# sephiroce/srf

Hardware: AMD Instinct MI355X
Metric: acoustic frames/sec through SRF (123-d fbank, 3-iter DR) at 1/2/4/8 MI355X (higher is better)
Workload: dtype fp32; 1 GPU; wsj_c4: SRF L=6 PH=CH=16 DIM=32 LPAD=RPAD=2 DR iter=3, train step (fwd+bwd+allreduce+Adam); utterances_per_gpu=28, frames_per_utterance=800, global_batch=28, parallelism=dp1, launch=hipgraph (fwd+CTC+bwd)

## Files before the change

### include/srf.h

```cpp
#ifndef SRF_H_
#define SRF_H_
#include <stddef.h>

#ifdef __cplusplus
extern "C" {
#endif

int srf_version(void);
const char* srf_last_error(void);

int srf_route_dr_auto_chunks(int B, int T, int N, int din, int lpad, int rpad, int J, int dout);
int srf_route_dr_split_table(int B, int T, int N, int din, int lpad, int rpad, int J, int dout, int n_chunks,
                             int* info, int* table, int capacity);
size_t srf_route_dr_saved_floats(int B, int T, int J, int dout, int iters);
size_t srf_route_dr_fwd_workspace(int B, int T, int N, int din, int lpad, int rpad, int J, int dout, int iters,
                                  int n_chunks);
size_t srf_route_dr_bwd_workspace(int B, int T, int N, int din, int lpad, int rpad, int J, int dout, int iters,
                                  int n_chunks);
int srf_route_dr_fwd(const float* emb, const float* W, const float* bias, int B, int T, int N, int din, int lpad,
                     int rpad, int J, int dout, int iters, int mask_first, int n_chunks, float* v_out,
                     float* saved, void* workspace, size_t workspace_bytes, void* stream);
size_t srf_route_dr_coupling_floats(int B, int T, int N, int din, int lpad, int rpad, int J, int dout, int iters);
#define SRF_DR_LAYOUT_N 17
int srf_route_dr_operand_layout(int B, int T, int N, int din, int lpad, int rpad, int J, int dout, int iters,
                                long long* out);
int srf_route_dr_fwd_ex(const float* emb, const float* W, const float* bias, int B, int T, int N, int din, int lpad,
                        int rpad, int J, int dout, int iters, int mask_first, int n_chunks, float* v_out,
                        float* saved, float* couplings, void* workspace, size_t workspace_bytes, void* stream);
int srf_route_dr_bwd_ex(const float* emb, const float* W, const float* bias, int B, int T, int N, int din, int lpad,
                        int rpad, int J, int dout, int iters, int mask_first, int n_chunks, const float* saved,
                        const float* couplings, const float* g_v, float* g_emb, float* g_W, float* g_bias,
                        void* workspace, size_t workspace_bytes, void* stream);
int srf_route_dr_bwd_weights_ex(const float* emb, int B, int T, int N, int din, int lpad, int rpad, int J, int dout,
                                int iters, int mask_first, int n_chunks, const float* saved, const float* couplings,
                                float* g_W, float* g_bias, void* workspace, size_t workspace_bytes, void* stream);
int srf_route_dr_bwd_data_ex(const float* emb, const float* W, const float* bias, int B, int T, int N, int din,
                             int lpad, int rpad, int J, int dout, int iters, int mask_first, int n_chunks,
                             const float* saved, const float* couplings, const float* g_v, float* g_emb,
                             void* workspace, size_t workspace_bytes, void* stream);
int srf_set_seed_source(const void* step_counter);
int srf_set_fault_flag(void* flag);
int srf_route_dr_bwd(const float* emb, const float* W, const float* bias, int B, int T, int N, int din, int lpad,
                     int rpad, int J, int dout, int iters, int mask_first, int n_chunks, const float* saved,
                     const float* g_v, float* g_emb, float* g_W, float* g_bias, void* workspace,
                     size_t workspace_bytes, void* stream);
int srf_route_dr_bwd_data(const float* emb, const float* W, const float* bias, int B, int T, int N, int din,
                          int lpad, int rpad, int J, int dout, int iters, int mask_first, int n_chunks,
                          const float* saved, const float* g_v, float* g_emb, void* workspace,
                          size_t workspace_bytes, void* stream);
int srf_route_dr_bwd_weights(const float* emb, int B, int T, int N, int din, int lpad, int rpad, int J, int dout,
                             int iters, int mask_first, int n_chunks, float* g_W, float* g_bias, void* workspace,
                             size_t workspace_bytes, void* stream);

size_t srf_route_sdr_saved_floats(int B, int T, int J, int dout);
size_t srf_route_sdr_fwd_workspace(int B, int T, int N, int din, int lpad, int rpad, int J, int dout);
size_t srf_route_sdr_bwd_workspace(int B, int T, int N, int din, int lpad, int rpad, int J, int dout, int iters);
int srf_route_sdr_fwd(const float* emb, const float* W, const float* bias, int B, int T, int N, int din, int lpad,
                      int rpad, int J, int dout, int iters, int mask_first, float* v_out, float* saved,
                      void* workspace, size_t workspace_bytes, void* stream);
int srf_route_sdr_bwd(const float* emb, const float* W, const float* bias, int B, int T, int N, int din, int lpad,
                      int rpad, int J, int dout, int iters, int mask_first, const float* saved, const float* g_v,
                      float* g_emb, float* g_W, float* g_bias, void* workspace, size_t workspace_bytes,
                      void* stream);

#define SRF_SDR_MAX_ITEMS 8
typedef struct {
  int t0, t1;
  const float* emb;
  const float* W;
  const float* bias;
  const float* WT;
  float* u;
  int v0, vn;
  float* v;
  float* couplings;
  void* workspace;
  size_t workspace_bytes;
  const float* g_v;
  float* carry;
  float* gu;
  int g0, gn;
  float* g_emb;
  float* g_W;
  float* g_bias;
  int accumulate;
  int u_bf16;
  int group;
  int gu_factored;
} srf_sdr_range;
int srf_route_sdr_pose_n(const srf_sdr_range* ranges, int n, int B, int T, int N, int din, int lpad, int rpad, int J,
                         int dout, int fp8, void* stream);
int srf_route_sdr_recur_fwd_n(const srf_sdr_range* ranges, int n, int B, int T, int in_n, int J, int dout, int iters,
                              int mask_first, void* stream);
int srf_route_sdr_recur_bwd_n(const srf_sdr_range* ranges, int n, int B, int T, int in_n, int J, int dout, int iters,
                              int mask_first, void* stream);
int srf_route_sdr_gx_n(const srf_sdr_range* ranges, int n, int B, int T, int N, int din, int lpad, int rpad, int J,
                       int dout, void* stream);
int srf_route_sdr_gw_n(const srf_sdr_range* ranges, int n, int B, int T, int N, int din, int lpad, int rpad, int J,
                       int dout, void* stream);
int srf_route_sdr_gx_gw_n(const srf_sdr_range* ranges, int n, int B, int T, int N, int din, int lpad, int rpad,
                          int J, int dout, void* stream);
int srf_route_sdr_gx_gw_fact_n(const srf_sdr_range* ranges, int n, int B, int T, int N, int din, int lpad, int rpad,
                               int J, int dout, int iters, void* stream);

int srf_route_sdr_pose(const float* emb, const float* W, const float* bias, int B, int T, int N, int din, int lpad,
                       int rpad, int J, int dout, int t0, int t1, float* u, int v0, int vn, void* stream);
int srf_route_sdr_pose_fp8(const float* emb, const float* W, const float* bias, int B, int T, int N, int din, int lpad,
                           int rpad, int J, int dout, int t0, int t1, float* u, int v0, int vn, void* stream);
size_t srf_route_sdr_recur_workspace(int B, int in_n, int J, int dout, int iters);
size_t srf_route_sdr_recur_zero_range(int B, int in_n, int J, int dout, int iters, size_t* offset_bytes);
size_t srf_route_sdr_coupling_floats(int in_n, int J, int dout, int iters);
int srf_route_sdr_couplings_required(int in_n, int J, int dout, int iters);
size_t srf_route_sdr_fact_floats(int in_n, int J, int dout, int iters);
int srf_route_sdr_recur_fwd(const float* u, int v0, int vn, int B, int T, int in_n, int J, int dout, int iters,
                            int mask_first, int t0, int t1, float* v_out, float* couplings, void* workspace,
                            size_t workspace_bytes, void* stream);
int srf_route_sdr_recur_bwd(const float* u, int v0, int vn, const float* v_saved, const float* couplings,
                            const float* g_v, int B, int T, int in_n, int J, int dout, int iters, int mask_first,
                            int t0, int t1, float* carry, float* gu, int g0, int gn, void* workspace,
                            size_t workspace_bytes, void* stream);
int srf_route_sdr_transpose_w(const float* W, int in_n, int J, int dout, int din, float* WT, void* stream);
int srf_route_sdr_gx(const float* gu, int g0, int gn, const float* WT, int B, int T, int N, int din, int lpad,
                     int rpad, int J, int dout, int t0, int t1, float* g_emb, void* stream);
int srf_route_sdr_gw(const float* gu, int g0, int gn, const float* emb, int B, int T, int N, int din, int lpad,
                     int rpad, int J, int dout, int t0, int t1, int accumulate, float* g_W, float* g_bias,
                     void* stream);

int srf_cnnfe_out_dims(int T, int feat_dim, int* T2, int* F2);
size_t srf_cnnfe_saved_bytes(int B, int T, int feat_dim, int nfilt);
size_t srf_cnnfe_fwd_workspace(int B, int T, int feat_dim, int nfilt);
size_t srf_cnnfe_bwd_workspace(int B, int T, int feat_dim, int nfilt);
int srf_cnnfe_fwd(const float* feats, const int* inp_len, int B, int T, int feat_dim, int nfilt,
                  const float* k0a, const float* b0a, const float* k0b, const float* b0b, const float* gamma0,
                  const float* beta0, const float* k1a, const float* b1a, const float* k1b, const float* b1b,
                  const float* gamma1, const float* beta1, float* mmean0, float* mvar0, float* mmean1, float* mvar1,
                  int training, float drop_p, unsigned long long seed, float* out, void* saved, size_t saved_bytes,
                  void* workspace, size_t workspace_bytes, void* stream);
int srf_cnnfe_bwd(const float* feats, const int* inp_len, int B, int T, int feat_dim, int nfilt, const float* gamma0,
                  const float* k1a, const float* k1b, const float* gamma1, float drop_p, unsigned long long seed,
                  const void* saved, const float* g_out, float* g_k0a, float* g_b0a, float* g_k0b, float* g_b0b,
                  float* g_gamma0, float* g_beta0, float* g_k1a, float* g_b1a, float* g_k1b, float* g_b1b,
                  float* g_gamma1, float* g_beta1, void* workspace, size_t workspace_bytes, void* stream);

#define SRF_CNNFE_BWD_PREP 1
#define SRF_CNNFE_BWD_DATA 2
#define SRF_CNNFE_BWD_WGRAD 4
#define SRF_CNNFE_BWD_ALL 7
int srf_cnnfe_bwd_parts(int parts, const float* feats, const int* inp_len, int B, int T, int feat_dim, int nfilt,
                        const float* gamma0, const float* k1a, const float* k1b, const float* gamma1, float drop_p,
                        unsigned long long seed, const void* saved, const float* g_out, float* g_k0a, float* g_b0a,
                        float* g_k0b, float* g_b0b, float* g_gamma0, float* g_beta0, float* g_k1a, float* g_b1a,
                        float* g_k1b, float* g_b1b, float* g_gamma1, float* g_beta1, void* workspace,
                        size_t workspace_bytes, void* stream);

size_t srf_primary_caps_saved_bytes(int B, int T, int PH, int PD);
size_t srf_primary_caps_bwd_workspace(int B, int T, int K, int PH, int PD);
int srf_primary_caps_fwd(const float* X, const int* inp_len, int B, int T, int K, int PH, int PD, const float* Wp,
                         const float* bp, const float* K1, const float* b1, const float* K2, const float* b2,
                         const float* gamma, const float* beta, int training, float p_caps, float p_in,
                         unsigned long long seed, float* z, void* saved, size_t saved_bytes, void* stream);
int srf_primary_caps_bwd(const float* X, const int* inp_len, int B, int T, int K, int PH, int PD, const float* Wp,
                         const float* K1, const float* K2, const float* gamma, const float* beta, int training,
                         float p_caps, float p_in, unsigned long long seed, const void* saved, const float* g_z,
                         float* g_X, float* g_Wp, float* g_bp, float* g_K1, float* g_b1, float* g_K2, float* g_b2,
                         float* g_gamma, float* g_beta, void* workspace, size_t workspace_bytes, void* stream);
int srf_primary_caps_fwd_ex(const float* X, const int* inp_len, int B, int T, int K, int PH, int PD, const float* Wp,
                            const float* bp, const float* K1, const float* b1, const float* K2, const float* b2,
                            const float* gamma, const float* beta, int training, float p_caps, float p_in,
                            unsigned long long seed, float proj_scale, int pos_enc, float* z, void* saved,
                            size_t saved_bytes, void* stream);
int srf_primary_caps_bwd_ex(const float* X, const int* inp_len, int B, int T, int K, int PH, int PD, const float* Wp,
                            const float* K1, const float* K2, const float* gamma, const float* beta, int training,
                            float p_caps, float p_in, unsigned long long seed, float proj_scale, const void* saved,
                            const float* g_z, float* g_X, float* g_Wp, float* g_bp, float* g_K1, float* g_b1,
                            float* g_K2, float* g_b2, float* g_gamma, float* g_beta, void* workspace,
                            size_t workspace_bytes, void* stream);

size_t srf_capsnorm_bwd_workspace(int F, int n, int J);
int srf_capsnorm_fwd(const float* x, int F, int n, const float* gamma, const float* beta, int training, float p,
                     unsigned long long seed, int layer, float* y, float* stat, void* stream);
int srf_capsnorm_bwd(const float* x, int F, int n, const float* gamma, const float* beta, int training, float p,
                     unsigned long long seed, int layer, const float* stat, const float* g_y, float* g_x,
                     float* g_gamma, float* g_beta, void* workspace, size_t workspace_bytes, void* stream);
int srf_capsnorm_fwd_range(const float* x, int B, int T, int t0, int t1, int n, const float* gamma, const float* beta,
                           int training, float p, unsigned long long seed, int layer, float* y, float* stat,
                           void* stream);
int srf_capsnorm_bwd_range(const float* x, int B, int T, int t0, int t1, int n, const float* gamma, const float* beta,
                           int training, float p, unsigned long long seed, int layer, const float* stat,
                           const float* g_y, float* g_x, float* gpart, void* stream);
#define SRF_CAPSNORM_MAX_ITEMS 8
typedef struct {
  int t0, t1, layer;
// ... 116 lines not shown
```

### srf_amd/_lib.py

```python
import ctypes
import os

_HERE = os.path.dirname(os.path.abspath(__file__))
LIB_PATH = os.environ.get('SRF_LIB_PATH') or os.path.join(_HERE, 'libsrf.so')

_c_int, _c_size, _vp = ctypes.c_int, ctypes.c_size_t, ctypes.c_void_p

SDR_MAX_ITEMS = 8


class SdrRange(ctypes.Structure):
    _fields_ = [('t0', _c_int), ('t1', _c_int), ('emb', _vp), ('W', _vp), ('bias', _vp), ('WT', _vp),
                ('u', _vp), ('v0', _c_int), ('vn', _c_int), ('v', _vp), ('couplings', _vp),
                ('workspace', _vp), ('workspace_bytes', _c_size), ('g_v', _vp), ('carry', _vp),
                ('gu', _vp), ('g0', _c_int), ('gn', _c_int), ('g_emb', _vp), ('g_W', _vp), ('g_bias', _vp),
                ('accumulate', _c_int), ('u_bf16', _c_int), ('group', _c_int), ('gu_factored', _c_int)]


_ranges = ctypes.POINTER(SdrRange)

CAPSNORM_MAX_ITEMS = 8


class CapsnormRange(ctypes.Structure):
    _fields_ = [('t0', _c_int), ('t1', _c_int), ('layer', _c_int), ('x', _vp), ('gamma', _vp), ('beta', _vp),
                ('y', _vp), ('stat', _vp), ('g_y', _vp), ('g_x', _vp), ('gpart', _vp)]


_cn_ranges = ctypes.POINTER(CapsnormRange)

STREAM_ADVANCE_MAX = 32


class StreamBuf(ctypes.Structure):
    _fields_ = [('ptr', _vp), ('row_bytes', _c_size), ('rows_per_stream', _c_int), ('shift', _c_int),
                ('keep', _c_int)]

_SIGNATURES = {
    'srf_version': (_c_int, []),
    'srf_last_error': (ctypes.c_char_p, []),
    'srf_set_seed_source': (_c_int, [_vp]),
    'srf_set_fault_flag': (_c_int, [_vp]),
    'srf_route_dr_auto_chunks': (_c_int, [_c_int] * 8),
    'srf_route_dr_split_table': (_c_int, [_c_int] * 9 + [_vp, _vp, _c_int]),
    'srf_route_dr_saved_floats': (_c_size, [_c_int] * 5),
    'srf_route_dr_fwd_workspace': (_c_size, [_c_int] * 10),
    'srf_route_dr_bwd_workspace': (_c_size, [_c_int] * 10),
    'srf_route_dr_fwd': (_c_int, [_vp, _vp, _vp] + [_c_int] * 11 + [_vp, _vp, _vp, _c_size, _vp]),
    'srf_route_dr_bwd': (_c_int, [_vp, _vp, _vp] + [_c_int] * 11 + [_vp, _vp, _vp, _vp, _vp, _vp, _c_size, _vp]),
    'srf_route_dr_bwd_data': (_c_int, [_vp, _vp, _vp] + [_c_int] * 11 + [_vp, _vp, _vp, _vp, _c_size, _vp]),
    'srf_route_dr_bwd_weights': (_c_int, [_vp] + [_c_int] * 11 + [_vp, _vp, _vp, _c_size, _vp]),
    'srf_route_dr_coupling_floats': (_c_size, [_c_int] * 9),
    'srf_route_dr_operand_layout': (_c_int, [_c_int] * 9 + [_vp]),
    'srf_route_dr_fwd_ex': (_c_int, [_vp, _vp, _vp] + [_c_int] * 11 + [_vp, _vp, _vp, _vp, _c_size, _vp]),
    'srf_route_dr_bwd_ex': (_c_int, [_vp, _vp, _vp] + [_c_int] * 11 + [_vp] * 7 + [_c_size, _vp]),
    'srf_route_dr_bwd_data_ex': (_c_int, [_vp, _vp, _vp] + [_c_int] * 11 + [_vp] * 5 + [_c_size, _vp]),
    'srf_route_dr_bwd_weights_ex': (_c_int, [_vp] + [_c_int] * 11 + [_vp] * 5 + [_c_size, _vp]),
    'srf_route_sdr_saved_floats': (_c_size, [_c_int] * 4),
    'srf_route_sdr_fwd_workspace': (_c_size, [_c_int] * 8),
    'srf_route_sdr_bwd_workspace': (_c_size, [_c_int] * 9),
    'srf_route_sdr_fwd': (_c_int, [_vp, _vp, _vp] + [_c_int] * 10 + [_vp, _vp, _vp, _c_size, _vp]),
    'srf_route_sdr_bwd': (_c_int, [_vp, _vp, _vp] + [_c_int] * 10 + [_vp, _vp, _vp, _vp, _vp, _vp, _c_size, _vp]),
    'srf_route_sdr_pose': (_c_int, [_vp, _vp, _vp] + [_c_int] * 10 + [_vp, _c_int, _c_int, _vp]),
    'srf_route_sdr_pose_fp8': (_c_int, [_vp, _vp, _vp] + [_c_int] * 10 + [_vp, _c_int, _c_int, _vp]),
    'srf_route_sdr_recur_workspace': (_c_size, [_c_int] * 5),
    'srf_route_sdr_recur_zero_range': (_c_size, [_c_int] * 5 + [ctypes.POINTER(_c_size)]),
    'srf_route_sdr_coupling_floats': (_c_size, [_c_int] * 4),
    'srf_route_sdr_couplings_required': (_c_int, [_c_int] * 4),
    'srf_route_sdr_fact_floats': (_c_size, [_c_int] * 4),
    'srf_route_sdr_recur_fwd': (_c_int, [_vp] + [_c_int] * 11 + [_vp, _vp, _vp, _c_size, _vp]),
    'srf_route_sdr_recur_bwd': (_c_int, [_vp, _c_int, _c_int, _vp, _vp, _vp] + [_c_int] * 9
                                + [_vp, _vp, _c_int, _c_int, _vp, _c_size, _vp]),
    'srf_route_sdr_transpose_w': (_c_int, [_vp] + [_c_int] * 4 + [_vp, _vp]),
    'srf_route_sdr_gx': (_c_int, [_vp, _c_int, _c_int, _vp] + [_c_int] * 10 + [_vp, _vp]),
    'srf_route_sdr_gw': (_c_int, [_vp, _c_int, _c_int, _vp] + [_c_int] * 11 + [_vp, _vp, _vp]),
    'srf_route_sdr_pose_n': (_c_int, [_ranges] + [_c_int] * 10 + [_vp]),
    'srf_route_sdr_recur_fwd_n': (_c_int, [_ranges] + [_c_int] * 8 + [_vp]),
    'srf_route_sdr_recur_bwd_n': (_c_int, [_ranges] + [_c_int] * 8 + [_vp]),
    'srf_route_sdr_gx_n': (_c_int, [_ranges] + [_c_int] * 9 + [_vp]),
    'srf_route_sdr_gw_n': (_c_int, [_ranges] + [_c_int] * 9 + [_vp]),
    'srf_route_sdr_gx_gw_n': (_c_int, [_ranges] + [_c_int] * 9 + [_vp]),
    'srf_route_sdr_gx_gw_fact_n': (_c_int, [_ranges] + [_c_int] * 10 + [_vp]),
    'srf_cnnfe_out_dims': (_c_int, [_c_int, _c_int, ctypes.POINTER(_c_int), ctypes.POINTER(_c_int)]),
    'srf_cnnfe_saved_bytes': (_c_size, [_c_int] * 4),
    'srf_cnnfe_fwd_workspace': (_c_size, [_c_int] * 4),
    'srf_cnnfe_bwd_workspace': (_c_size, [_c_int] * 4),
    'srf_cnnfe_fwd': (_c_int, [_vp, _vp] + [_c_int] * 4 + [_vp] * 16 + [_c_int, ctypes.c_float, ctypes.c_ulonglong,
                                                                       _vp, _vp, _c_size, _vp, _c_size, _vp]),
    'srf_cnnfe_bwd': (_c_int, [_vp, _vp] + [_c_int] * 4 + [_vp] * 4 + [ctypes.c_float, ctypes.c_ulonglong]
                      + [_vp] * 15 + [_c_size, _vp]),
    'srf_cnnfe_bwd_parts': (_c_int, [_c_int, _vp, _vp] + [_c_int] * 4 + [_vp] * 4 + [ctypes.c_float, ctypes.c_ulonglong]
                            + [_vp] * 15 + [_c_size, _vp]),
    'srf_primary_caps_saved_bytes': (_c_size, [_c_int] * 4),
    'srf_primary_caps_bwd_workspace': (_c_size, [_c_int] * 5),
    'srf_primary_caps_fwd': (_c_int, [_vp, _vp] + [_c_int] * 5 + [_vp] * 8 + [_c_int, ctypes.c_float, ctypes.c_float,
                                                                           ctypes.c_ulonglong, _vp, _vp, _c_size, _vp]),
    'srf_primary_caps_bwd': (_c_int, [_vp, _vp] + [_c_int] * 5 + [_vp] * 5 + [_c_int, ctypes.c_float, ctypes.c_float,
                                                                           ctypes.c_ulonglong] + [_vp] * 12
                             + [_c_size, _vp]),
    'srf_primary_caps_fwd_ex': (_c_int, [_vp, _vp] + [_c_int] * 5 + [_vp] * 8
                                + [_c_int, ctypes.c_float, ctypes.c_float, ctypes.c_ulonglong, ctypes.c_float, _c_int,
                                   _vp, _vp, _c_size, _vp]),
    'srf_primary_caps_bwd_ex': (_c_int, [_vp, _vp] + [_c_int] * 5 + [_vp] * 5
                                + [_c_int, ctypes.c_float, ctypes.c_float, ctypes.c_ulonglong, ctypes.c_float]
                                + [_vp] * 12 + [_c_size, _vp]),
    'srf_capsnorm_bwd_workspace': (_c_size, [_c_int] * 3),
    'srf_capsnorm_fwd': (_c_int, [_vp, _c_int, _c_int, _vp, _vp, _c_int, ctypes.c_float, ctypes.c_ulonglong, _c_int,
                                  _vp, _vp, _vp]),
    'srf_capsnorm_bwd': (_c_int, [_vp, _c_int, _c_int, _vp, _vp, _c_int, ctypes.c_float, ctypes.c_ulonglong, _c_int]
                         + [_vp] * 6 + [_c_size, _vp]),
    'srf_capsnorm_fwd_range_n': (_c_int, [_cn_ranges] + [_c_int] * 5 + [ctypes.c_float, ctypes.c_ulonglong, _vp]),
    'srf_capsnorm_bwd_range_n': (_c_int, [_cn_ranges] + [_c_int] * 5 + [ctypes.c_float, ctypes.c_ulonglong, _vp]),
    'srf_capsnorm_fwd_range': (_c_int, [_vp] + [_c_int] * 5 + [_vp, _vp, _c_int, ctypes.c_float, ctypes.c_ulonglong,
                                                             _c_int, _vp, _vp, _vp]),
    'srf_capsnorm_bwd_range': (_c_int, [_vp] + [_c_int] * 5 + [_vp, _vp, _c_int, ctypes.c_float, ctypes.c_ulonglong,
                                                             _c_int, _vp, _vp, _vp, _vp, _vp]),
    'srf_capsnorm_params_workspace': (_c_size, [_c_int] * 2),
    'srf_capsnorm_bwd_params': (_c_int, [_vp, _c_int, _c_int, _vp, _vp, _vp, _c_size, _vp]),
    'srf_caps_head_fwd': (_c_int, [_vp, _c_int, _c_int, _c_int] + [_vp] * 4 + [_c_int, ctypes.c_float,
                                                                              ctypes.c_ulonglong, _c_int]
                          + [_vp] * 4),
    'srf_caps_head_fwd_ex': (_c_int, [_vp, _c_int, _c_int, _c_int] + [_vp] * 4
                             + [_c_int, ctypes.c_float, ctypes.c_ulonglong, _c_int, ctypes.c_float] + [_vp] * 4),
    'srf_caps_head_bwd': (_c_int, [_vp, _c_int, _c_int, _c_int] + [_vp] * 3 + [_c_int, ctypes.c_float,
                                                                              ctypes.c_ulonglong, _c_int]
                          + [_vp] * 9 + [_c_size, _vp]),
    'srf_ctc_workspace': (_c_size, [_c_int] * 4),
    'srf_ctc_loss': (_c_int, [_vp] * 4 + [_c_int] * 5 + [ctypes.c_float, _vp, _vp, _vp, _c_size, _vp]),
    'srf_ctc_align_workspace': (_c_size, [_c_int] * 4),
    'srf_ctc_align': (_c_int, [_vp] * 4 + [_c_int] * 5 + [_vp] * 6 + [_c_size, _vp]),
    'srf_edit_align_workspace': (_c_size, [_c_int] * 3),
    'srf_edit_align': (_c_int, [_vp, _vp, _c_int, _vp, _vp, _c_int, _c_int, _vp, _c_int] + [_vp] * 5
                       + [_c_int, _vp, _c_size, _vp]),
    'srf_word_split_workspace': (_c_size, [_c_int] * 2),
    'srf_word_split': (_c_int, [_vp, _vp, _c_int, _c_int, _vp, _c_int, _c_int] + [_vp] * 10 + [_c_size, _vp]),
    'srf_word_align_workspace': (_c_size, [_c_int] * 3),
    'srf_word_align': (_c_int, [_vp, _vp, _c_int, _vp, _vp, _c_int, _c_int, _vp, _c_int, _c_int] + [_vp] * 11
                       + [_c_size, _vp]),
    'srf_ctc_greedy_n': (_c_int, [_vp, _vp] + [_c_int] * 4 + [_vp, _vp, _vp, _vp]),
    'srf_ctc_greedy_frames_n': (_c_int, [_vp, _vp] + [_c_int] * 5 + [_vp, _vp, _vp, _vp, _vp]),
    'srf_ctc_beam_state_bytes': (_c_size, [_c_int] * 4),
    'srf_ctc_beam_reset': (_c_int, [_vp, _c_size] + [_c_int] * 4 + [ctypes.POINTER(_c_int), _vp]),
    'srf_ctc_beam_push_n': (_c_int, [_vp, _c_size] + [_c_int] * 5 + [_vp, _vp, _c_int, ctypes.POINTER(_c_int), _vp]),
    'srf_ctc_beam_best': (_c_int, [_vp, _c_size] + [_c_int] * 4 + [_vp, _vp, _vp, _vp]),
    'srf_ctc_beam_nbest': (_c_int, [_vp, _c_size] + [_c_int] * 6 + [_vp, _vp, _vp, _vp, _vp]),
    'srf_ctc_beam_lm_state_bytes': (_c_size, [_c_int] * 4),
    'srf_ctc_beam_lm_reset': (_c_int, [_vp, _c_size] + [_c_int] * 4 + [ctypes.POINTER(_c_int), _vp]),
    'srf_ctc_beam_lm_push_n': (_c_int, [_vp, _c_size] + [_c_int] * 5 + [_vp, _vp, _c_int, _vp, _vp, _c_int,
                                                                       ctypes.POINTER(_c_int), _vp]),
    'srf_ctc_beam_lm_best': (_c_int, [_vp, _c_size] + [_c_int] * 4 + [_vp, _vp, _vp, _vp, _vp]),
    'srf_ctc_beam_lm_nbest': (_c_int, [_vp, _c_size] + [_c_int] * 6 + [_vp, _vp, _vp, _vp, _vp, _vp]),
    'srf_mwer_workspace': (_c_size, [_c_int] * 5),
    'srf_mwer_loss': (_c_int, [_vp] * 6 + [_c_int] * 6 + [ctypes.c_float] + [_vp] * 5 + [_c_size, _vp]),
    'srf_stream_advance_n': (_c_int, [ctypes.POINTER(StreamBuf), _c_int, _c_int, _vp]),
    'srf_fbank_num_frames': (_c_int, [_c_int]),
    'srf_fbank_table_floats': (_c_size, []),
    'srf_fbank_tables': (_c_int, [_vp, _c_size]),
    'srf_fbank_static': (_c_int, [_vp, _c_int, _vp, _vp] + [_c_int] * 9 + [ctypes.c_float, ctypes.c_ulonglong, _vp, _vp]),
    'srf_fbank_deltas': (_c_int, [_vp, _vp] + [_c_int] * 6 + [_vp, _vp, _c_int, _vp, _c_int, _c_int, _vp]),
    'srf_fbank_stats': (_c_int, [_vp, _vp, _c_int, _c_int, _c_int, _vp, _vp]),
    'srf_adam_step': (_c_int, [_vp, _vp, _vp, _vp, _c_size, ctypes.c_float, ctypes.c_float, ctypes.c_float,
                               ctypes.c_float, _vp]),
}

_PROF_SIGNATURES = {
    'srf_route_dr_set_timing_events': (_c_int, [_vp, _vp, _c_int]),
}


class SrfError(RuntimeError):
    pass


_lib = None


def lib():
    global _lib
    if _lib is None:
        if not os.path.exists(LIB_PATH):
            raise ImportError(f'{LIB_PATH} is missing: build it with `make -C srf_amd/csrc` '
                              '(or __graft_entry__.build()); there is no fallback path')
        import torch
        h = ctypes.CDLL(LIB_PATH)
        for name, (res, args) in list(_SIGNATURES.items()) + list(_PROF_SIGNATURES.items()):
            fn = getattr(h, name)
            fn.restype = res
            fn.argtypes = args
        _lib = h
    return _lib


def exported_symbols():
    return list(_SIGNATURES)


def prof_symbols():
    return list(_PROF_SIGNATURES)


def check(rc, what):
    if rc != 0:
        msg = lib().srf_last_error().decode(errors='replace')
        raise SrfError(f'{what} failed (rc={rc}): {msg}')
```

### srf_amd/csrc/caps.hip

```cpp
#include <algorithm>
#include <cmath>

#include "srf_common.h"
#include "srf_reduce.h"
#include "srf_rng.h"
#include "../../include/srf.h"

namespace {

constexpr float kSquashEps = 1e-7f;
constexpr float kLengthEps = 1e-7f;
constexpr float kLnEps = 1e-3f;
constexpr int kMaxVec = 4096;

__device__ __forceinline__ int ceil_div_len(int len, int div) { return (len + div - 1) / div; }

__device__ __forceinline__ void block_sum2(float& a, float& b, float* red) {
  a = wave_sum(a);
  b = wave_sum(b);
  const int w = threadIdx.x >> 6, l = threadIdx.x & 63;
  __syncthreads();
  if (l == 0) {
    red[w] = a;
    red[4 + w] = b;
  }
  __syncthreads();
  a = red[0] + red[1] + red[2] + red[3];
  b = red[4] + red[5] + red[6] + red[7];
}

__device__ __forceinline__ float drop_mult(bool on, unsigned long long seed, unsigned stream, size_t idx, float p) {
  if (!on) return 1.f;
  return srf_keep(seed, stream, idx, p) ? 1.f / (1.f - p) : 0.f;
}

__device__ __forceinline__ float pos_enc(int t, int p, int PH) {
  const int nts = PH >> 1;
  const float inc = 9.210340371976184f / (float)(nts - 1);
  const int k = p < nts ? p : p - nts;
  const float st = (float)t * expf((float)k * -inc);
  return p < nts ? sinf(st) : cosf(st);
}

__device__ __forceinline__ float proj_epilogue(float acc, int f, int T, int p, int PH, float scale, int pe) {
  const float y = acc * scale;
  return pe ? y + pos_enc(f % T, p, PH) : y;
}

__global__ __launch_bounds__(256) void proj_fwd_kernel(const float* __restrict__ X, int F, int K, int PH,
                                                       const float* __restrict__ Wp, const float* __restrict__ bp,
                                                       float* __restrict__ e, int T, float scale, int pe) {
  const int f = blockIdx.x * 4 + (threadIdx.x >> 6);
  const int l = threadIdx.x & 63;
  if (f >= F) return;
  const float* x = X + (size_t)f * K;
  for (int p0 = 0; p0 < PH; p0 += 8) {
    const int np = min(8, PH - p0);
    float acc[8];
#pragma unroll
    for (int q = 0; q < 8; ++q) acc[q] = 0.f;
#pragma unroll 4
    for (int k = l; k < K; k += 64) {
      const float xv = x[k];
      const float* w = Wp + (size_t)k * PH + p0;
#pragma unroll
      for (int q = 0; q < 8; ++q) acc[q] += xv * (q < np ? w[q < np ? q : 0] : 0.f);
    }
#pragma unroll
    for (int q = 0; q < 8; ++q) {
      const float s = wave_sum(acc[q]);
      if (l == 0 && q < np) e[(size_t)f * PH + p0 + q] = proj_epilogue(s + bp[p0 + q], f, T, p0 + q, PH, scale, pe);
    }
  }
}

template <int PH, int FW>
__global__ __launch_bounds__(256) void proj_fwd_vec_kernel(const float* __restrict__ X, int F, int K,
                                                           const float* __restrict__ Wp,
                                                           const float* __restrict__ bp, float* __restrict__ e,
                                                           int T, float scale, int pe) {
  constexpr int PQ = PH / 4;
  const int l = threadIdx.x & 63;
  const int f0 = (blockIdx.x * 4 + (threadIdx.x >> 6)) * FW;
  if (f0 >= F) return;
  float acc[FW][PH];
#pragma unroll
  for (int u = 0; u < FW; ++u)
#pragma unroll
    for (int p = 0; p < PH; ++p) acc[u][p] = 0.f;
#pragma unroll 2
  for (int k0 = 4 * l; k0 < K; k0 += 256) {
    f4 x[FW], w[4][PQ];
#pragma unroll
    for (int u = 0; u < FW; ++u) x[u] = *reinterpret_cast<const f4*>(X + (size_t)min(f0 + u, F - 1) * K + k0);
#pragma unroll
    for (int kk = 0; kk < 4; ++kk)
#pragma unroll
      for (int q = 0; q < PQ; ++q) w[kk][q] = *reinterpret_cast<const f4*>(Wp + (size_t)(k0 + kk) * PH + 4 * q);
#pragma unroll
    for (int u = 0; u < FW; ++u)
#pragma unroll
      for (int kk = 0; kk < 4; ++kk)
#pragma unroll
        for (int p = 0; p < PH; ++p) acc[u][p] += x[u][kk] * w[kk][p >> 2][p & 3];
  }
#pragma unroll
  for (int u = 0; u < FW; ++u)
#pragma unroll
    for (int p = 0; p < PH; ++p) {
      const float sum = wave_sum(acc[u][p]);
      if (l == 0 && f0 + u < F) e[(size_t)(f0 + u) * PH + p] = proj_epilogue(sum + bp[p], f0 + u, T, p, PH, scale, pe);
    }
}

constexpr int kProjWaves = 16;
template <int PH>
__global__ __launch_bounds__(64 * kProjWaves) void proj_fwd_mfma_kernel(const float* __restrict__ X, int F, int K,
                                                                       const float* __restrict__ Wp,
                                                                       const float* __restrict__ bp,
                                                                       float* __restrict__ e, int T, float scale,
                                                                       int pe, int Kq) {
  static_assert(PH <= 16, "one 16-column output tile");
  __shared__ float part[kProjWaves][16][17];
  const int lane = threadIdx.x & 63, wv = threadIdx.x >> 6;
  const int m = lane & 15, g = lane >> 4;
  const int f0 = blockIdx.x * 16;
  const int fm = min(f0 + m, F - 1);
  const bool fok = f0 + m < F;
  const int kb = wv * Kq, ke = min(K, kb + Kq);
  f4 acc = {0.f, 0.f, 0.f, 0.f};
  constexpr int U = 4;
  for (int k0 = kb; k0 < ke; k0 += 16 * U) {
    f4 xa[U];
    float wb[U][4];
#pragma unroll
    for (int u = 0; u < U; ++u) {
      const int k = k0 + 16 * u + 4 * g;
      const bool kok = k < ke;
      const f4 x = *reinterpret_cast<const f4*>(X + (size_t)fm * K + (kok ? k : kb));
      xa[u] = (fok && kok) ? x : f4{0.f, 0.f, 0.f, 0.f};
#pragma unroll
      for (int j = 0; j < 4; ++j) {
        const float w = Wp[(size_t)(kok ? k + j : kb) * PH + min(m, PH - 1)];
        wb[u][j] = (kok && m < PH) ? w : 0.f;
      }
    }
#pragma unroll
    for (int u = 0; u < U; ++u)
#pragma unroll
      for (int j = 0; j < 4; ++j) acc = mfma16x16x4(xa[u][j], wb[u][j], acc);
  }
#pragma unroll
  for (int v = 0; v < 4; ++v) part[wv][4 * g + v][m] = acc[v];
  __syncthreads();
  if (threadIdx.x < 16 * PH) {
    const int r = threadIdx.x / PH, pp = threadIdx.x % PH;
    float sum = 0.f;
#pragma unroll
    for (int w = 0; w < kProjWaves; ++w) sum += part[w][r][pp];
    if (f0 + r < F) e[(size_t)(f0 + r) * PH + pp] = proj_epilogue(sum + bp[pp], f0 + r, T, pp, PH, scale, pe);
  }
}

constexpr int kProjXF = 16;
template <int PH>
__global__ __launch_bounds__(256) void proj_bwd_x_vec_kernel(const float* __restrict__ g_e,
                                                             const float* __restrict__ Wp, int F, int K,
                                                             float* __restrict__ g_X) {
  constexpr int PQ = PH / 4;
  const size_t idx = (size_t)blockIdx.x * blockDim.x + threadIdx.x;
  const int K4 = K / 4;
  const int FG = (F + kProjXF - 1) / kProjXF;
  if (idx >= (size_t)FG * K4) return;
  const int fg = (int)(idx / K4);
  const int k0 = (int)(idx - (size_t)fg * K4) * 4;
  f4 w[4][PQ];
#pragma unroll
  for (int kk = 0; kk < 4; ++kk)
#pragma unroll
    for (int q = 0; q < PQ; ++q) w[kk][q] = *reinterpret_cast<const f4*>(Wp + (size_t)(k0 + kk) * PH + 4 * q);
#pragma unroll
  for (int u = 0; u < kProjXF; ++u) {
    const int f = fg * kProjXF + u;
    if (f >= F) break;
    f4 ge[PQ];
#pragma unroll
// ... 302 lines not shown
      const int tt = t - dt + 1;
      if (tt < 0 || tt >= cd.T) continue;
      const size_t fo = (size_t)(f - dt + 1) * E;
      for (int dp = 0; dp < 3; ++dp) {
        const int pp = p - dp + 1;
        if (pp < 0 || pp >= cd.PH) continue;
        for (int d = q; d < cd.PD; d += kEbLanes)
          s += g_v1[fo + pp * cd.PD + d] * K1[(dt * 3 + dp) * cd.PD + d] +
               g_v2[fo + pp * cd.PD + d] * K2[(dt * 3 + dp) * cd.PD + d];
      }
    }
  }
#pragma unroll
  for (int o = kEbLanes / 2; o >= 1; o >>= 1) s += __shfl_xor(s, o, 64);
  if (live && q == 0) g_e[idx] = s * scale;
}

struct RowMap {
  int T, t0, nt;
  __device__ __forceinline__ int row(int q) const {
    const int b = q / nt;
    return b * T + t0 + (q - b * nt);
  }
  static RowMap all(int F) { return RowMap{F, 0, F}; }
};

__device__ __forceinline__ void capsnorm_fwd_row(const float* __restrict__ x, int n, const float* __restrict__ gamma,
                                                 const float* __restrict__ beta, int training, float p,
                                                 unsigned long long seed, const unsigned long long* __restrict__ seed_src,
                                                 unsigned stream, float* __restrict__ y, float* __restrict__ stat,
                                                 int head, int J, int D, const float* __restrict__ gamma_o,
                                                 const float* __restrict__ beta_o, float* __restrict__ logits,
                                                 float* __restrict__ lens, float len_eps, int f) {
  seed = srf_step_seed(seed, seed_src);
  extern __shared__ __attribute__((aligned(16))) float sm[];
  float* v = sm;
  float* red = v + n;
  float s1 = 0.f, dummy = 0.f;
  for (int i = threadIdx.x; i < n; i += blockDim.x) {
    const float a = x[(size_t)f * n + i];
    v[i] = a;
    s1 += a;
  }
  block_sum2(s1, dummy, red);
  const float mean = s1 / n;
  float s2 = 0.f;
  for (int i = threadIdx.x; i < n; i += blockDim.x) {
    const float dv = v[i] - mean;
    s2 += dv * dv;
  }
  dummy = 0.f;
  block_sum2(s2, dummy, red);
  const float rstd = 1.f / sqrtf(s2 / n + kLnEps);
  for (int i = threadIdx.x; i < n; i += blockDim.x) {
    const size_t gi = (size_t)f * n + i;
    const float o = ((v[i] - mean) * rstd * gamma[i] + beta[i]) * drop_mult(training && p > 0.f, seed, stream, gi, p);
    v[i] = o;
    if (!head) y[gi] = o;
  }
  if (threadIdx.x == 0) {
    stat[4 * f] = mean;
    stat[4 * f + 1] = rstd;
  }
  if (!head) return;
  __syncthreads();
  float* L = v + n + 8;
  for (int j = threadIdx.x; j < J; j += blockDim.x) {
    float s = 0.f;
    for (int d = 0; d < D; ++d) s += v[j * D + d] * v[j * D + d];
    L[j] = sqrtf(s + len_eps);
    lens[(size_t)f * J + j] = L[j];
  }
  __syncthreads();
  float t1 = 0.f;
  dummy = 0.f;
  for (int j = threadIdx.x; j < J; j += blockDim.x) t1 += L[j];
  block_sum2(t1, dummy, red);
  const float mo = t1 / J;
  float t2 = 0.f;
  for (int j = threadIdx.x; j < J; j += blockDim.x) t2 += (L[j] - mo) * (L[j] - mo);
  dummy = 0.f;
  block_sum2(t2, dummy, red);
  const float ro = 1.f / sqrtf(t2 / J + kLnEps);
  for (int j = threadIdx.x; j < J; j += blockDim.x)
    logits[(size_t)f * J + j] = (L[j] - mo) * ro * gamma_o[j] + beta_o[j];
  if (threadIdx.x == 0) {
    stat[4 * f + 2] = mo;
    stat[4 * f + 3] = ro;
  }
}

__device__ __forceinline__ void capsnorm_bwd_row(
    const float* __restrict__ x, int n, const float* __restrict__ gamma, const float* __restrict__ beta,
    int training, float p, unsigned long long seed, const unsigned long long* __restrict__ seed_src, unsigned stream,
    const float* __restrict__ stat, const float* __restrict__ g_in, int head, int J, int D,
    const float* __restrict__ gamma_o, const float* __restrict__ lens, float* __restrict__ g_x,
    float* __restrict__ gpart, int f) {
  seed = srf_step_seed(seed, seed_src);
  extern __shared__ __attribute__((aligned(16))) float sm[];
  float* gy = sm;
  float* red = gy + n;
  float* gl = red + 8;
  const float mean = stat[4 * f], rstd = stat[4 * f + 1];
  const size_t stride = head ? (size_t)2 * n + 2 * J : (size_t)2 * n;
  if (head) {
    const float mo = stat[4 * f + 2], ro = stat[4 * f + 3];
    float a1 = 0.f, a2 = 0.f;
    for (int j = threadIdx.x; j < J; j += blockDim.x) {
      const float go = g_in[(size_t)f * J + j];
      const float xh = (lens[(size_t)f * J + j] - mo) * ro;
      gpart[(size_t)f * stride + 2 * n + j] = go * xh;
      gpart[(size_t)f * stride + 2 * n + J + j] = go;
      const float gx = go * gamma_o[j];
      gl[j] = gx;
      a1 += gx;
      a2 += gx * xh;
    }
    block_sum2(a1, a2, red);
    for (int j = threadIdx.x; j < J; j += blockDim.x) {
      const float xh = (lens[(size_t)f * J + j] - mo) * ro;
      gl[j] = ro * (gl[j] - a1 / J - xh * a2 / J) / lens[(size_t)f * J + j];
    }
    __syncthreads();
  }
  float a1 = 0.f, a2 = 0.f;
  for (int i = threadIdx.x; i < n; i += blockDim.x) {
    const size_t gi = (size_t)f * n + i;
    const float xh = (x[gi] - mean) * rstd;
    const float dm = drop_mult(training && p > 0.f, seed, stream, gi, p);
    float go;
    if (head) {
      const float o = (xh * gamma[i] + beta[i]) * dm;
      go = gl[i / D] * o;
    } else {
      go = g_in[gi];
    }
    const float g = go * dm;
    gpart[(size_t)f * stride + i] = g * xh;
    gpart[(size_t)f * stride + n + i] = g;
    const float t = g * gamma[i];
    gy[i] = t;
    a1 += t;
    a2 += t * xh;
  }
  block_sum2(a1, a2, red);
  for (int i = threadIdx.x; i < n; i += blockDim.x) {
    const size_t gi = (size_t)f * n + i;
    const float xh = (x[gi] - mean) * rstd;
    g_x[gi] = rstd * (gy[i] - a1 / n - xh * a2 / n);
  }
}

template <int NPL>
__device__ __forceinline__ void capsnorm_fwd_wave(const float* __restrict__ x, const float* __restrict__ gamma,
                                                  const float* __restrict__ beta, bool drop, float p,
                                                  unsigned long long seed, unsigned stream, float* __restrict__ y,
                                                  float* __restrict__ stat, int f, int lane) {
  constexpr int n = 64 * NPL, NV = NPL / 4;
  const f4* xr = reinterpret_cast<const f4*>(x + (size_t)f * n);
  f4 v[NV];
  float s1 = 0.f;
#pragma unroll
  for (int k = 0; k < NV; ++k) {
    v[k] = xr[k * 64 + lane];
    s1 += (v[k].x + v[k].y) + (v[k].z + v[k].w);
  }
  const float mean = wave_sum(s1) / n;
  float s2 = 0.f;
#pragma unroll
  for (int k = 0; k < NV; ++k) {
    const f4 d = v[k] - mean;
    s2 += (d.x * d.x + d.y * d.y) + (d.z * d.z + d.w * d.w);
  }
  const float rstd = 1.f / sqrtf(wave_sum(s2) / n + kLnEps);
  f4* yr = reinterpret_cast<f4*>(y + (size_t)f * n);
#pragma unroll
  for (int k = 0; k < NV; ++k) {
    const int q = k * 64 + lane;
    const f4 g = reinterpret_cast<const f4*>(gamma)[q], b = reinterpret_cast<const f4*>(beta)[q];
    const size_t gi = (size_t)f * n + 4 * q;
    f4 o;
#pragma unroll
    for (int c = 0; c < 4; ++c) o[c] = ((v[k][c] - mean) * rstd * g[c] + b[c]) * drop_mult(drop, seed, stream, gi + c, p);
    yr[q] = o;
  }
  if (lane == 0) {
    stat[4 * f] = mean;
    stat[4 * f + 1] = rstd;
  }
}

template <int NPL>
__device__ __forceinline__ void caps_head_fwd_wave(const float* __restrict__ x, const float* __restrict__ gamma,
                                                   const float* __restrict__ beta, bool drop, float p,
                                                   unsigned long long seed, unsigned stream,
                                                   float* __restrict__ stat, int D, const float* __restrict__ gamma_o,
                                                   const float* __restrict__ beta_o, float* __restrict__ logits,
                                                   float* __restrict__ lens, float len_eps, int f, int lane) {
  constexpr int n = 64 * NPL, NV = NPL / 4;
  const int LPC = D / 4, J = n / D;
  const f4* xr = reinterpret_cast<const f4*>(x + (size_t)f * n);
  f4 v[NV];
  float s1 = 0.f;
#pragma unroll
  for (int k = 0; k < NV; ++k) {
    v[k] = xr[k * 64 + lane];
    s1 += (v[k].x + v[k].y) + (v[k].z + v[k].w);
  }
  const float mean = wave_sum(s1) / n;
  float s2 = 0.f;
#pragma unroll
  for (int k = 0; k < NV; ++k) {
    const f4 d = v[k] - mean;
    s2 += (d.x * d.x + d.y * d.y) + (d.z * d.z + d.w * d.w);
  }
  const float rstd = 1.f / sqrtf(wave_sum(s2) / n + kLnEps);
  float L[NV];
  float t1 = 0.f;
#pragma unroll
  for (int k = 0; k < NV; ++k) {
    const int q = k * 64 + lane;
    const f4 g = reinterpret_cast<const f4*>(gamma)[q], b = reinterpret_cast<const f4*>(beta)[q];
    const size_t gi = (size_t)f * n + 4 * q;
    float ss = 0.f;
#pragma unroll
    for (int c = 0; c < 4; ++c) {
      const float o = ((v[k][c] - mean) * rstd * g[c] + b[c]) * drop_mult(drop, seed, stream, gi + c, p);
      ss += o * o;
    }
    for (int m = 1; m < LPC; m <<= 1) ss += __shfl_xor(ss, m, 64);
    L[k] = sqrtf(ss + len_eps);
    t1 += L[k];
  }
  const float mo = wave_sum(t1) / (float)LPC / J;
  float t2 = 0.f;
#pragma unroll
  for (int k = 0; k < NV; ++k) t2 += (L[k] - mo) * (L[k] - mo);
  const float ro = 1.f / sqrtf(wave_sum(t2) / (float)LPC / J + kLnEps);
  if (lane % LPC == 0) {
#pragma unroll
    for (int k = 0; k < NV; ++k) {
      const int j = (k * 64 + lane) / LPC;
      lens[(size_t)f * J + j] = L[k];
      logits[(size_t)f * J + j] = (L[k] - mo) * ro * gamma_o[j] + beta_o[j];
    }
  }
  if (lane == 0) {
    stat[4 * f] = mean;
    stat[4 * f + 1] = rstd;
    stat[4 * f + 2] = mo;
    stat[4 * f + 3] = ro;
  }
}

template <int NPL>
__global__ __launch_bounds__(256) void caps_head_fwd_wave_kernel(const float* __restrict__ x,
                                                                 const float* __restrict__ gamma,
                                                                 const float* __restrict__ beta, int training, float p,
                                                                 unsigned long long seed,
                                                                 const unsigned long long* __restrict__ seed_src,
                                                                 unsigned stream, float* __restrict__ stat, int D,
                                                                 const float* __restrict__ gamma_o,
                                                                 const float* __restrict__ beta_o,
                                                                 float* __restrict__ logits, float* __restrict__ lens,
                                                                 float len_eps, int rows) {
  const int w = blockIdx.x * 4 + (threadIdx.x >> 6);
  if (w >= rows) return;
  caps_head_fwd_wave<NPL>(x, gamma, beta, training && p > 0.f, p, srf_step_seed(seed, seed_src), stream, stat, D,
                          gamma_o, beta_o, logits, lens, len_eps, w, threadIdx.x & 63);
}

template <int NPL>
__device__ __forceinline__ void capsnorm_bwd_wave(const float* __restrict__ x, const float* __restrict__ gamma,
                                                  bool drop, float p, unsigned long long seed, unsigned stream,
                                                  const float* __restrict__ stat, const float* __restrict__ g_in,
                                                  float* __restrict__ g_x, f4 (&pgxh)[NPL / 4], f4 (&pgg)[NPL / 4],
                                                  int f, int lane) {
  constexpr int n = 64 * NPL, NV = NPL / 4;
  const float mean = stat[4 * f], rstd = stat[4 * f + 1];
  const f4* xr = reinterpret_cast<const f4*>(x + (size_t)f * n);
  const f4* gr = reinterpret_cast<const f4*>(g_in + (size_t)f * n);
  f4 xh[NV], t[NV];
  float a1 = 0.f, a2 = 0.f;
#pragma unroll
  for (int k = 0; k < NV; ++k) {
    const int q = k * 64 + lane;
    const f4 xv = xr[q], go = gr[q], gam = reinterpret_cast<const f4*>(gamma)[q];
    const size_t gi = (size_t)f * n + 4 * q;
    f4 gxh, gg;
#pragma unroll
    for (int c = 0; c < 4; ++c) {
      xh[k][c] = (xv[c] - mean) * rstd;
      const float g = go[c] * drop_mult(drop, seed, stream, gi + c, p);
      gxh[c] = g * xh[k][c];
      gg[c] = g;
      t[k][c] = g * gam[c];
      a1 += t[k][c];
      a2 += t[k][c] * xh[k][c];
    }
    pgxh[k] += gxh;
    pgg[k] += gg;
  }
  a1 = wave_sum(a1);
  a2 = wave_sum(a2);
  f4* ox = reinterpret_cast<f4*>(g_x + (size_t)f * n);
#pragma unroll
  for (int k = 0; k < NV; ++k) {
    f4 o;
#pragma unroll
    for (int c = 0; c < 4; ++c) o[c] = rstd * (t[k][c] - a1 / n - xh[k][c] * a2 / n);
    ox[k * 64 + lane] = o;
  }
}

template <int NPL>
__device__ __forceinline__ void store_gpart(float* __restrict__ gpart, size_t row, const f4 (&pgxh)[NPL / 4],
                                            const f4 (&pgg)[NPL / 4], int lane) {
  constexpr int n = 64 * NPL;
  f4* pg = reinterpret_cast<f4*>(gpart + row * 2 * n);
#pragma unroll
  for (int k = 0; k < NPL / 4; ++k) {
    pg[k * 64 + lane] = pgxh[k];
    pg[n / 4 + k * 64 + lane] = pgg[k];
  }
}

template <int NPL, bool BWD>
__global__ __launch_bounds__(256) void capsnorm_wave_kernel(const float* __restrict__ x, const float* __restrict__ gamma,
                                                            const float* __restrict__ beta, int training, float p,
                                                            unsigned long long seed,
                                                            const unsigned long long* __restrict__ seed_src,
                                                            unsigned stream, float* __restrict__ y,
                                                            float* __restrict__ stat, const float* __restrict__ g_in,
                                                            float* __restrict__ gpart, RowMap rmap, int rows, int rpw) {
  const int w = blockIdx.x * 4 + (threadIdx.x >> 6);
  const int lane = threadIdx.x & 63;
  const unsigned long long sd = srf_step_seed(seed, seed_src);
  const bool drop = training && p > 0.f;
  if constexpr (BWD) {
    const int r0 = w * rpw;
    if (r0 >= rows) return;
    f4 pgxh[NPL / 4], pgg[NPL / 4];
#pragma unroll
    for (int k = 0; k < NPL / 4; ++k) pgxh[k] = pgg[k] = f4{0.f, 0.f, 0.f, 0.f};
    const int r1 = min(rows, r0 + rpw);
    for (int r = r0; r < r1; ++r)
      capsnorm_bwd_wave<NPL>(x, gamma, drop, p, sd, stream, stat, g_in, y, pgxh, pgg, rmap.row(r), lane);
    store_gpart<NPL>(gpart, rpw == 1 ? (size_t)rmap.row(r0) : (size_t)w, pgxh, pgg, lane);
  } else {
    if (w >= rows) return;
    capsnorm_fwd_wave<NPL>(x, gamma, beta, drop, p, sd, stream, y, stat, rmap.row(w), lane);
  }
}

__global__ __launch_bounds__(256) void capsnorm_fwd_kernel(
    const float* __restrict__ x, int n, const float* __restrict__ gamma, const float* __restrict__ beta, int training,
    float p, unsigned long long seed, const unsigned long long* __restrict__ seed_src, unsigned stream,
    float* __restrict__ y, float* __restrict__ stat, int head, int J, int D, const float* __restrict__ gamma_o,
    const float* __restrict__ beta_o, float* __restrict__ logits, float* __restrict__ lens, float len_eps,
    RowMap rmap) {
  capsnorm_fwd_row(x, n, gamma, beta, training, p, seed, seed_src, stream, y, stat, head, J, D, gamma_o, beta_o,
                   logits, lens, len_eps, rmap.row(blockIdx.x));
}

__global__ __launch_bounds__(256) void capsnorm_bwd_kernel(
    const float* __restrict__ x, int n, const float* __restrict__ gamma, const float* __restrict__ beta, int training,
    float p, unsigned long long seed, const unsigned long long* __restrict__ seed_src, unsigned stream,
    const float* __restrict__ stat, const float* __restrict__ g_in, int head, int J, int D,
    const float* __restrict__ gamma_o, const float* __restrict__ lens, float* __restrict__ g_x,
    float* __restrict__ gpart, RowMap rmap) {
  capsnorm_bwd_row(x, n, gamma, beta, training, p, seed, seed_src, stream, stat, g_in, head, J, D, gamma_o, lens, g_x,
                   gpart, rmap.row(blockIdx.x));
}

struct CnItems {
  srf_capsnorm_range it[SRF_CAPSNORM_MAX_ITEMS];
  int B, T, n_items;
};

template <int NPL, bool BWD>
__global__ __launch_bounds__(256) void capsnorm_range_n_wave_kernel(CnItems items, int training, float p,
                                                                    unsigned long long seed,
                                                                    const unsigned long long* __restrict__ seed_src) {
  const srf_capsnorm_range& r = items.it[blockIdx.y];
  const int nt = r.t1 - r.t0;
  const int w = blockIdx.x * 4 + (threadIdx.x >> 6);
  if (w >= items.B * nt) return;
  const int f = RowMap{items.T, r.t0, nt}.row(w);
  const unsigned stream = (unsigned)(kStreamMid0 + r.layer);
  const unsigned long long sd = srf_step_seed(seed, seed_src);
  const bool drop = training && p > 0.f;
  if constexpr (BWD) {
    f4 pgxh[NPL / 4], pgg[NPL / 4];
#pragma unroll
    for (int k = 0; k < NPL / 4; ++k) pgxh[k] = pgg[k] = f4{0.f, 0.f, 0.f, 0.f};
    capsnorm_bwd_wave<NPL>(r.x, r.gamma, drop, p, sd, stream, r.stat, r.g_y, r.g_x, pgxh, pgg, f, threadIdx.x & 63);
    store_gpart<NPL>(r.gpart, (size_t)f, pgxh, pgg, threadIdx.x & 63);
  } else
    capsnorm_fwd_wave<NPL>(r.x, r.gamma, r.beta, drop, p, sd, stream, r.y, r.stat, f, threadIdx.x & 63);
}

template <bool BWD>
__global__ __launch_bounds__(256) void capsnorm_range_n_kernel(CnItems items, int n, int training, float p,
                                                               unsigned long long seed,
                                                               const unsigned long long* __restrict__ seed_src) {
  const srf_capsnorm_range& r = items.it[blockIdx.y];
  const int nt = r.t1 - r.t0;
  if ((int)blockIdx.x >= items.B * nt) return;
  const int f = RowMap{items.T, r.t0, nt}.row(blockIdx.x);
  const unsigned stream = (unsigned)(kStreamMid0 + r.layer);
  if constexpr (BWD)
    capsnorm_bwd_row(r.x, n, r.gamma, r.beta, training, p, seed, seed_src, stream, r.stat, r.g_y, 0, 0, 0, nullptr,
                     nullptr, r.g_x, r.gpart, f);
  else
    capsnorm_fwd_row(r.x, n, r.gamma, r.beta, training, p, seed, seed_src, stream, r.y, r.stat, 0, 0, 0, nullptr,
                     nullptr, nullptr, nullptr, kLengthEps, f);
}

struct CapsSaved {
  float *e, *m, *lnstat;
  unsigned char* sel;
  size_t bytes;
};

CapsSaved caps_saved_layout(int F, int PH, int PD, void* base) {
  const size_t E = (size_t)PH * PD;
  size_t off = 0;
  auto take = [&](size_t bytes) {
    size_t o = off;
    off += srf::align_up(bytes, 256);
    return o;
  };
  const size_t oe = take((size_t)F * PH * 4), om = take((size_t)F * E * 4), os = take((size_t)F * 2 * 4),
               osel = take((size_t)F * E);
  char* b = static_cast<char*>(base);
  CapsSaved c;
  c.e = (float*)(b + oe);
  c.m = (float*)(b + om);
  c.lnstat = (float*)(b + os);
  c.sel = (unsigned char*)(b + osel);
  c.bytes = off;
  return c;
}

struct CapsBwdWs {
  float *gv1, *gv2, *wpart, *wsum, *g_e, *ppart, *psum, *scratch;
  size_t bytes;
};

constexpr int kProjChunks = 64;

CapsBwdWs caps_bwd_layout(int F, int K, int PH, int PD, void* base) {
  const size_t E = (size_t)PH * PD;
  const size_t wcols = 2 * E + 20 * PD, pcols = (size_t)K * PH + PH;
  size_t off = 0;
  auto take = [&](size_t bytes) {
    size_t o = off;
    off += srf::align_up(bytes, 256);
    return o;
  };
  const size_t o1 = take((size_t)F * E * 4), o2 = take((size_t)F * E * 4), ow = take((size_t)F * wcols * 4),
               owsum = take(wcols * 4), oge = take((size_t)F * PH * 4), opp = take(kProjChunks * pcols * 4),
               ops = take(pcols * 4),
               osc = take(std::max(srf::colsum_scratch_floats(F, (int)wcols), srf::colsum_scratch_floats(kProjChunks, (int)pcols)) * 4);
  char* b = static_cast<char*>(base);
  CapsBwdWs w;
  w.gv1 = (float*)(b + o1);
  w.gv2 = (float*)(b + o2);
  w.wpart = (float*)(b + ow);
  w.wsum = (float*)(b + owsum);
  w.g_e = (float*)(b + oge);
  w.ppart = (float*)(b + opp);
  w.psum = (float*)(b + ops);
  w.scratch = (float*)(b + osc);
  w.bytes = off;
  return w;
}

int check_caps(int B, int T, int PH, int PD) {
  SRF_REQUIRE(B > 0 && T > 0 && PH > 0 && PD > 0, "bad primary capsule shape");
  SRF_REQUIRE((size_t)PH * PD <= kMaxVec, "PH*PD = %d exceeds %d", PH * PD, kMaxVec);
  return SRF_OK;
}

}

constexpr int kCnRowsPerWave = 4;

template <bool BWD>
static bool capsnorm_wave(int n, int rows, RowMap rm, const float* x, const float* gamma, const float* beta,
                          int training, float p, unsigned long long seed, unsigned stream, float* y, float* stat,
                          const float* g_in, float* gpart, hipStream_t st, int rpw = 1) {
  const dim3 grid(((rows + rpw - 1) / rpw + 3) / 4);
#define SRF_CN_WAVE(NPL)                                                                                             \
  hipLaunchKernelGGL((capsnorm_wave_kernel<NPL, BWD>), grid, dim3(256), 0, st, x, gamma, beta, training, p, seed,   \
                     srf::seed_source(), stream, y, stat, g_in, gpart, rm, rows, rpw)
  if (n == 256) SRF_CN_WAVE(4);
  else if (n == 512) SRF_CN_WAVE(8);
  else if (n == 1024) SRF_CN_WAVE(16);
  else return false;
#undef SRF_CN_WAVE
  return true;
}

extern "C" {

size_t srf_primary_caps_saved_bytes(int B, int T, int PH, int PD) {
  return caps_saved_layout(B * T, PH, PD, nullptr).bytes;
}

size_t srf_primary_caps_bwd_workspace(int B, int T, int K, int PH, int PD) {
  return caps_bwd_layout(B * T, K, PH, PD, nullptr).bytes;
}

int srf_primary_caps_fwd(const float* X, const int* inp_len, int B, int T, int K, int PH, int PD, const float* Wp,
                         const float* bp, const float* K1, const float* b1, const float* K2, const float* b2,
                         const float* gamma, const float* beta, int training, float p_caps, float p_in,
                         unsigned long long seed, float* z, void* saved, size_t saved_bytes, void* stream) {
  return srf_primary_caps_fwd_ex(X, inp_len, B, T, K, PH, PD, Wp, bp, K1, b1, K2, b2, gamma, beta, training, p_caps,
                                 p_in, seed, 1.f, 0, z, saved, saved_bytes, stream);
}

int srf_primary_caps_fwd_ex(const float* X, const int* inp_len, int B, int T, int K, int PH, int PD, const float* Wp,
                            const float* bp, const float* K1, const float* b1, const float* K2, const float* b2,
                            const float* gamma, const float* beta, int training, float p_caps, float p_in,
                            unsigned long long seed, float proj_scale, int pos_enc, float* z, void* saved,
                            size_t saved_bytes, void* stream) {
  int rc = check_caps(B, T, PH, PD);
  if (rc) return rc;
  SRF_REQUIRE(!pos_enc || (PH >= 4 && PH % 2 == 0), "positional encoding needs an even PH >= 4, got %d", PH);
  SRF_REQUIRE(X && inp_len && Wp && bp && K1 && b1 && K2 && b2 && gamma && beta && z && saved, "null pointer");
  const int F = B * T;
  CapsSaved sv = caps_saved_layout(F, PH, PD, saved);
  if (saved_bytes < sv.bytes) {
    srf::set_error("primary caps saved buffer too small: %zu < %zu", saved_bytes, sv.bytes);
    return SRF_EWORKSPACE;
  }
  hipStream_t st = static_cast<hipStream_t>(stream);
  constexpr int FW = 2;
  const dim3 gvec((F + 4 * FW - 1) / (4 * FW));
  const int Kq = ((K + kProjWaves - 1) / kProjWaves + 15) / 16 * 16;
  if (K % 4 == 0 && (PH == 4 || PH == 8 || PH == 16)) {
    const dim3 gm((F + 15) / 16), bm(64 * kProjWaves);
    if (PH == 4)
      hipLaunchKernelGGL((proj_fwd_mfma_kernel<4>), gm, bm, 0, st, X, F, K, Wp, bp, sv.e, T, proj_scale, pos_enc, Kq);
    else if (PH == 8)
      hipLaunchKernelGGL((proj_fwd_mfma_kernel<8>), gm, bm, 0, st, X, F, K, Wp, bp, sv.e, T, proj_scale, pos_enc, Kq);
    else
      hipLaunchKernelGGL((proj_fwd_mfma_kernel<16>), gm, bm, 0, st, X, F, K, Wp, bp, sv.e, T, proj_scale, pos_enc,
                         Kq);
  } else if (K % 4 == 0 && PH == 4)
    hipLaunchKernelGGL((proj_fwd_vec_kernel<4, FW>), gvec, dim3(256), 0, st, X, F, K, Wp, bp, sv.e, T,
                       proj_scale, pos_enc);
  else if (K % 4 == 0 && PH == 8)
    hipLaunchKernelGGL((proj_fwd_vec_kernel<8, FW>), gvec, dim3(256), 0, st, X, F, K, Wp, bp, sv.e, T,
                       proj_scale, pos_enc);
  else if (K % 4 == 0 && PH == 16)
    hipLaunchKernelGGL((proj_fwd_vec_kernel<16, FW>), gvec, dim3(256), 0, st, X, F, K, Wp, bp, sv.e, T,
                       proj_scale, pos_enc);
  else
    hipLaunchKernelGGL(proj_fwd_kernel, dim3((F + 3) / 4), dim3(256), 0, st, X, F, K, PH, Wp, bp, sv.e, T, proj_scale,
                       pos_enc);
  SRF_LAUNCH_CHECK("proj_fwd");
  CapsDims cd{B, T, PH, PD};
  const size_t sh = (size_t)(PH * PD + 5 * PH + 8) * sizeof(float);
  hipLaunchKernelGGL(encaps_fwd_kernel, dim3(F), dim3(256), sh, st, sv.e, inp_len, cd, K1, b1, K2, b2, gamma, beta,
                     training, p_caps, p_in, seed, srf::seed_source(), sv.m, sv.sel, sv.lnstat, z);
  SRF_LAUNCH_CHECK("encaps_fwd");
  return SRF_OK;
}

int srf_primary_caps_bwd(const float* X, const int* inp_len, int B, int T, int K, int PH, int PD, const float* Wp,
                         const float* K1, const float* K2, const float* gamma, const float* beta, int training,
                         float p_caps, float p_in, unsigned long long seed, const void* saved, const float* g_z,
                         float* g_X, float* g_Wp, float* g_bp, float* g_K1, float* g_b1, float* g_K2, float* g_b2,
                         float* g_gamma, float* g_beta, void* workspace, size_t workspace_bytes, void* stream) {
  return srf_primary_caps_bwd_ex(X, inp_len, B, T, K, PH, PD, Wp, K1, K2, gamma, beta, training, p_caps, p_in, seed,
                                 1.f, saved, g_z, g_X, g_Wp, g_bp, g_K1, g_b1, g_K2, g_b2, g_gamma, g_beta, workspace,
                                 workspace_bytes, stream);
}

int srf_primary_caps_bwd_ex(const float* X, const int* inp_len, int B, int T, int K, int PH, int PD, const float* Wp,
                            const float* K1, const float* K2, const float* gamma, const float* beta, int training,
                            float p_caps, float p_in, unsigned long long seed, float proj_scale, const void* saved,
                            const float* g_z, float* g_X, float* g_Wp, float* g_bp, float* g_K1, float* g_b1,
                            float* g_K2, float* g_b2, float* g_gamma, float* g_beta, void* workspace,
                            size_t workspace_bytes, void* stream) {
  int rc = check_caps(B, T, PH, PD);
  if (rc) return rc;
  SRF_REQUIRE(X && inp_len && Wp && K1 && K2 && gamma && beta && saved && g_z && g_X && g_Wp && g_bp && g_K1 &&
                  g_b1 && g_K2 && g_b2 && g_gamma && g_beta && workspace,
              "null pointer");
  const int F = B * T, E = PH * PD;
  CapsSaved sv = caps_saved_layout(F, PH, PD, const_cast<void*>(saved));
  CapsBwdWs w = caps_bwd_layout(F, K, PH, PD, workspace);
  if (workspace_bytes < w.bytes) {
    srf::set_error("primary caps workspace too small: %zu < %zu", workspace_bytes, w.bytes);
    return SRF_EWORKSPACE;
  }
  hipStream_t st = static_cast<hipStream_t>(stream);
  CapsDims cd{B, T, PH, PD};
  const size_t sh = (size_t)(4 * E + 6 * PH + 8) * sizeof(float);
  hipLaunchKernelGGL(encaps_bwd_a_kernel, dim3(F), dim3(256), sh, st, g_z, sv.e, sv.m, sv.sel, sv.lnstat, inp_len, cd,
                     gamma, beta, training, p_caps, p_in, seed, srf::seed_source(), w.gv1, w.gv2, w.wpart);
  SRF_LAUNCH_CHECK("encaps_bwd_a");
  const int wcols = 2 * E + 20 * PD;
  if ((rc = srf::colsum(w.wpart, F, wcols, nullptr, w.scratch, st,
                        srf::ColSplit{{g_gamma, g_beta, g_K1, g_b1, g_K2, g_b2}, {E, E, 9 * PD, PD, 9 * PD, PD}})))
    return rc;
  hipLaunchKernelGGL(encaps_bwd_b_kernel, dim3(((size_t)F * PH * kEbLanes + 255) / 256), dim3(256), 0, st, w.gv1,
                     w.gv2, cd, K1, K2, w.g_e, proj_scale);
  SRF_LAUNCH_CHECK("encaps_bwd_b");
  const dim3 gx4(((size_t)((F + kProjXF - 1) / kProjXF) * (K / 4) + 255) / 256);
  if (K % 4 == 0 && PH == 4)
    hipLaunchKernelGGL(proj_bwd_x_vec_kernel<4>, gx4, dim3(256), 0, st, w.g_e, Wp, F, K, g_X);
  else if (K % 4 == 0 && PH == 8)
    hipLaunchKernelGGL(proj_bwd_x_vec_kernel<8>, gx4, dim3(256), 0, st, w.g_e, Wp, F, K, g_X);
  else if (K % 4 == 0 && PH == 16)
    hipLaunchKernelGGL(proj_bwd_x_vec_kernel<16>, gx4, dim3(256), 0, st, w.g_e, Wp, F, K, g_X);
  else
    hipLaunchKernelGGL(proj_bwd_x_kernel, dim3(((size_t)F * K + 255) / 256), dim3(256), 0, st, w.g_e, Wp, F, K, PH,
                       g_X);
  SRF_LAUNCH_CHECK("proj_bwd_x");
  const int fchunk = (F + kProjChunks - 1) / kProjChunks;
  if (PH <= 16)
    hipLaunchKernelGGL(proj_bwd_w_mfma_kernel, dim3((K + 63) / 64, kProjChunks), dim3(256), 0, st, X, w.g_e, F, K, PH,
                       fchunk, w.ppart);
  else
    hipLaunchKernelGGL(proj_bwd_w_kernel, dim3((K + 255) / 256, kProjChunks), dim3(256), 0, st, X, w.g_e, F, K, PH,
                       fchunk, w.ppart);
  SRF_LAUNCH_CHECK("proj_bwd_w");
  const int pcols = K * PH + PH;
  if ((rc = srf::colsum(w.ppart, kProjChunks, pcols, nullptr, w.scratch, st,
                        srf::ColSplit{{g_Wp, g_bp, nullptr, nullptr}, {K * PH, PH, 0, 0}})))
    return rc;
  return SRF_OK;
}

size_t srf_capsnorm_bwd_workspace(int F, int n, int J) {
  const int cols = 2 * n + 2 * J;
// ... 229 lines not shown
```

### srf_amd/csrc/route_dr.hip

```cpp
#include <algorithm>
#include <cmath>
#include <type_traits>

#include "srf_common.h"
#include "route_fwd32.h"
#include "../../include/srf.h"
#include "../../include/srf_prof.h"

namespace {

constexpr float kSquashEps = 1e-7f;

thread_local hipEvent_t* t_ev_start = nullptr;
thread_local hipEvent_t* t_ev_stop = nullptr;
thread_local int t_ev_n = 0;
constexpr int MODE_FWD = 0;
constexpr int MODE_BWD = 1;

using srf::DrGeom;

template <int KS>
__device__ __forceinline__ void load_vec(const float* __restrict__ p, float (&v)[KS]) {
  if constexpr (KS % 4 == 0) {
#pragma unroll
    for (int q = 0; q < KS / 4; ++q) {
      f4 t = *reinterpret_cast<const f4*>(p + 4 * q);
      v[4 * q] = t.x; v[4 * q + 1] = t.y; v[4 * q + 2] = t.z; v[4 * q + 3] = t.w;
    }
  } else {
    static_assert(KS == 2, "din must be 8, 16, 32 or 64");
    f2 t = *reinterpret_cast<const f2*>(p);
    v[0] = t.x; v[1] = t.y;
  }
}

__device__ __forceinline__ f4 ld4(const float* p) { return *reinterpret_cast<const f4*>(p); }
__device__ __forceinline__ void st4(float* p, f4 v) { *reinterpret_cast<f4*>(p) = v; }

struct FrameLoc {
  int b, t;
  bool valid;
};

__device__ __forceinline__ FrameLoc frame_loc(int f, int F, int T) {
  const int fc = min(f, F - 1);
  FrameLoc r;
  r.b = fc / T;
  r.t = fc - r.b * T;
  r.valid = f < F;
  return r;
}

template <int DIN>
__device__ __forceinline__ void load_x(const float* __restrict__ emb, const FrameLoc& fl, int T, int N, int lpad,
                                       int i, int g, float (&x)[DIN / 4]) {
  constexpr int KS = DIN / 4;
  const int w = i / N, n = i - w * N;
  const int ts = fl.t + w - lpad;
  const bool ok = fl.valid && ts >= 0 && ts < T;
  const int tsc = min(max(ts, 0), T - 1);
  load_vec<KS>(emb + ((size_t)(fl.b * T + tsc) * N + n) * DIN + g * KS, x);
#pragma unroll
  for (int k = 0; k < KS; ++k) x[k] = ok ? x[k] : 0.f;
}

template <int DIN>
__device__ __forceinline__ f4 pose_tile(const float* __restrict__ W, const float* __restrict__ bias, int i,
                                        int JD, int NT, int tg, int lane, const float (&x)[DIN / 4]) {
  constexpr int KS = DIN / 4;
  const int tc = min(tg, NT - 1);
  const int arow = min(tc * 16 + (lane & 15), JD - 1);
  const int g = lane >> 4;
  float a[KS];
  load_vec<KS>(W + ((size_t)i * JD + arow) * DIN + g * KS, a);
  const int crow = min(tc * 16 + 4 * g, JD - 4);
  f4 acc = ld4(bias + (size_t)i * JD + crow);
#pragma unroll
  for (int k = 0; k < KS; ++k) acc = mfma16x16x4(a[k], x[k], acc);
  return acc;
}

template <int DOUT, int TW>
__device__ __forceinline__ void jreduce(float (&p)[TW]) {
#pragma unroll
  for (int t = 0; t < TW; ++t) {
    p[t] = xor16_sum(p[t]);
    if constexpr (DOUT >= 16) p[t] = xor32_sum(p[t]);
  }
  if constexpr (DOUT > 16) {
    constexpr int TPJ = DOUT / 16;
#pragma unroll
    for (int t0 = 0; t0 < TW; t0 += TPJ) {
      float s = 0.f;
#pragma unroll
      for (int q = 0; q < TPJ; ++q) s += p[t0 + q];
#pragma unroll
      for (int q = 0; q < TPJ; ++q) p[t0 + q] = s;
    }
  }
}

template <int DOUT>
__device__ __forceinline__ int tile_j(int tg, int g) { return (tg * 16 + 4 * g) / DOUT; }

template <int DOUT>
__device__ __forceinline__ bool tile_primary(int tg) {
  if constexpr (DOUT > 16) return (tg % (DOUT / 16)) == 0;
  return true;
}

__device__ __forceinline__ void load_rows(const float* __restrict__ v, int f, bool fvalid, int JD, int tg, int g,
                                          float (&o)[4]) {
  const int row = tg * 16 + 4 * g;
  const bool ok = fvalid && row < JD;
  const f4 a = ld4(v + (size_t)(fvalid ? f : 0) * JD + min(row, JD - 4));
  o[0] = ok ? a.x : 0.f; o[1] = ok ? a.y : 0.f; o[2] = ok ? a.z : 0.f; o[3] = ok ? a.w : 0.f;
}

template <int DIN, int TW>
struct Frags {
  float x[DIN / 4];
  float w[TW][DIN / 4];
  f4 b[TW];
};

template <int DIN, int TW, bool NOBIAS = false>
__device__ __forceinline__ void fetch_frags(const float* __restrict__ emb, const float* __restrict__ W,
                                            const float* __restrict__ bias, const FrameLoc& loc, int T, int N,
                                            int lpad, int i, int JD, int NT, int tbase, int lane,
                                            Frags<DIN, TW>& fr) {
  constexpr int KS = DIN / 4;
  const int g = lane >> 4;
  load_x<DIN>(emb, loc, T, N, lpad, i, g, fr.x);
  const float* Wi = W + (size_t)i * JD * DIN;
  const float* bi = bias + (size_t)i * JD;
  int lrow = lane & 15, brow = 4 * g;
#pragma unroll
  for (int t = 0; t < TW; ++t) {
    const int tc = __builtin_amdgcn_readfirstlane(min(tbase + t, NT - 1));
    if constexpr (DIN < 16) {
      lrow = min(tc * 16 + (lane & 15), JD - 1) - tc * 16;
      brow = min(tc * 16 + 4 * g, JD - 4) - tc * 16;
    }
    load_vec<KS>(Wi + (size_t)tc * 16 * DIN + lrow * DIN + g * KS, fr.w[t]);
    if constexpr (NOBIAS) {
      fr.b[t] = f4{0.f, 0.f, 0.f, 0.f};
    } else {
      fr.b[t] = ld4(bi + tc * 16 + brow);
    }
  }
}

template <int DIN, int TW>
__device__ __forceinline__ void pose_tiles(const Frags<DIN, TW>& fr, float (&u)[TW][4]) {
#pragma unroll
  for (int t = 0; t < TW; ++t) {
    f4 acc = fr.b[t];
#pragma unroll
// ... 1379 lines not shown
      if (r > 0) vst[R + r - 1] = __builtin_bit_cast(f4, __builtin_amdgcn_raw_buffer_load_b128(rs_v[r - 1], wo0, so, 0));
    }
  };
  const int iwo = 4 * rq * 16 + 4 * ((2 * wg + (fm >> 2)) ^ (rq & 3)) + (fm & 3);
  const int iro = n * 16 + 4 * ((2 * h) ^ ((n >> 2) & 3));
  auto img_store = [&](float* im, int v) {
#pragma unroll
    for (int c = 0; c < 4; ++c) im[v * (D * 16) + iwo + c * 16] = vst[v][c];
  };
  auto img_read = [&](const float* im, f2 (&nx)[NV][4]) {
#pragma unroll
    for (int v = 0; v < NV; ++v) {
      const f4 a = ld4(im + v * (D * 16) + iro), b = ld4(im + v * (D * 16) + (iro ^ 4));
      nx[v][0] = f2{a[0], a[1]}, nx[v][1] = f2{a[2], a[3]}, nx[v][2] = f2{b[0], b[1]}, nx[v][3] = f2{b[2], b[3]};
    }
  };

  f16v acc[CAP];
  float gb[CAP];
#pragma unroll
  for (int k = 0; k < CAP; ++k) {
    gb[k] = 0.f;
    acc[k] = f16v{};
  }
  float* const imw = vimg + wv * IMG;
  if (ft0 < ft1) {
    stage_load(ft0);
    if constexpr (VW == 0) vec_load(nxa, ft0);
    else img_load(ft0);
    stage_store(0);
    if (ft0 + 1 < ft1) stage_load(ft0 + 1);
    if constexpr (VW == 2) {
#pragma unroll
      for (int v = 0; v < NV; ++v) img_store(imw, v);
      img_load(min(ft0 + 1, ft1 - 1));
    }
  }
  const int xoff = CG * 4 + (n * 16 + ((h ^ ((n >> 3) & 1)) * 8)) * 2;
  const float s0 = c0 * sg;
  auto caps = [&](int buf, const f2 (&g0)[4], const f2 (&cur)[NV][4], bool img_next) {
    const unsigned char* sb = stg[buf] + k0 * PCB;
#pragma unroll
    for (int k = 0; k < CAP; ++k) {
      const unsigned char* ck = sb + k * PCB;
      const float* ckf = reinterpret_cast<const float*>(ck);
      f2 gu[4];
#pragma unroll
      for (int v = 0; v < 4; ++v) gu[v] = g0[v];
#pragma unroll
      for (int r = 0; r < RV; ++r) {
        const float* cp = ckf + ((r * 2 + 0) * 4 + wv) * 16 + 8 * h;
        const float* gp = ckf + ((r * 2 + 1) * 4 + wv) * 16 + 8 * h;
        const f4 ca = ld4(cp), cb = ld4(cp + 4), ga = ld4(gp), gbv = ld4(gp + 4);
        const f2 c2[4] = {f2{ca[0], ca[1]}, f2{ca[2], ca[3]}, f2{cb[0], cb[1]}, f2{cb[2], cb[3]}};
        const f2 g2[4] = {f2{ga[0], ga[1]}, f2{ga[2], ga[3]}, f2{gbv[0], gbv[1]}, f2{gbv[2], gbv[3]}};
#pragma unroll
        for (int v = 0; v < 4; ++v) {
          gu[v] = __builtin_elementwise_fma(c2[v], cur[r + 1][v], gu[v]);
          gu[v] = __builtin_elementwise_fma(g2[v], cur[R + r][v], gu[v]);
        }
      }
      const f2 gq = (gu[0] + gu[1]) + (gu[2] + gu[3]);
      gb[k] += gq[0] + gq[1];
      h8 bh, bl;
      split8h(gu, bh, bl);
      const h8 xh = *reinterpret_cast<const h8*>(ck + xoff);
      const h8 xl = *reinterpret_cast<const h8*>(ck + xoff + D * 16 * 2);
      acc[k] = mfma32h(xh, bh, acc[k]);
      acc[k] = mfma32h(xh, bl, acc[k]);
      acc[k] = mfma32h(xl, bh, acc[k]);
      if constexpr (VW == 2) {
        if (img_next) {
#pragma unroll
          for (int v = 0; v < NV; ++v)
            if (v * CAP / NV == k) img_store(imw + (buf ^ 1) * (4 * IMG), v);
        }
      }
    }
  };
  auto tile = [&](auto bufc, const f2 (&cur)[NV][4], f2 (&nxt)[NV][4], int ft) {
    constexpr int buf = decltype(bufc)::value;
    f2 g0[4];
#pragma unroll
    for (int v = 0; v < 4; ++v) g0[v] = cur[0][v] * s0;
    __syncthreads();
    if (ft + 1 < ft1) {
      stage_store(buf ^ 1);
      if (ft + 2 < ft1) stage_load(ft + 2);
    }
    vec_load(nxt, ft + 1 < ft1 ? ft + 1 : ft);
    caps(buf, g0, cur, false);
  };
  auto tile_img = [&](auto bufc, int ft) {
    constexpr int buf = decltype(bufc)::value;
    f2 cur[NV][4], g0[4];
    __syncthreads();
    img_read(imw + buf * (4 * IMG), cur);
    if (ft + 1 < ft1) {
      stage_store(buf ^ 1);
      if (ft + 2 < ft1) stage_load(ft + 2);
    }
#pragma unroll
    for (int v = 0; v < 4; ++v) g0[v] = cur[0][v] * s0;
    caps(buf, g0, cur, ft + 1 < ft1);
    __builtin_amdgcn_sched_barrier(0);
    img_load(min(ft + 2, ft1 - 1));
  };
  using S0 = std::integral_constant<int, 0>;
  using S1 = std::integral_constant<int, 1>;
  for (int ft = ft0; ft < ft1; ft += 2) {
    if constexpr (VW == 0) tile(S0{}, nxa, nxb, ft);
    else tile_img(S0{}, ft);
    if (ft + 1 >= ft1) break;
    if constexpr (VW == 0) tile(S1{}, nxb, nxa, ft + 1);
    else tile_img(S1{}, ft + 1);
  }
  float* gw = gwp + (size_t)s * pstride;
  float* gbo = gbp + (size_t)s * pstride;
  const float un = srf_exp2i(-(bx + eg)), ug = srf_exp2i(-eg);
#pragma unroll
  for (int k = 0; k < CAP; ++k) {
    const float a = gb[k];
    float pa, pb;
    xpair32(a, pa, pb);
    if (k0 + k >= ncap || !wave_on) continue;
    const int i = i0 + k0 + k;
    if (h == 0) gbo[(size_t)i * JD + row] = (pa + pb) * ug;
#pragma unroll
    for (int q = 0; q < 4; ++q)
      st4(gw + ((size_t)i * JD + row) * D + 8 * q + 4 * h,
          f4{acc[k][4 * q] * un, acc[k][4 * q + 1] * un, acc[k][4 * q + 2] * un, acc[k][4 * q + 3] * un});
  }
}

__global__ void gw_reduce_kernel(const float* __restrict__ part, int S, size_t n4, size_t stride, float* __restrict__ gW,
                                 size_t nw4, float* __restrict__ gb) {
  const size_t idx = (size_t)blockIdx.x * blockDim.x + threadIdx.x;
  if (idx >= n4) return;
  f4 a = ld4(part + idx * 4);
  for (int s = 1; s < S; ++s) a += ld4(part + (size_t)s * stride + idx * 4);
  if (idx < nw4)
    st4(gW + idx * 4, a);
  else
    st4(gb + (idx - nw4) * 4, a);
}

template <int Q>
__device__ __forceinline__ float qsum(float v) {
#pragma unroll
  for (int o = 1; o < Q; o <<= 1) v += __shfl_xor(v, o, 64);
  return v;
}

struct SlabSplit {
  int n;
  int G, U, in_n, JD;
};

__device__ __forceinline__ int slab_count(const SlabSplit& sp, size_t FJD, size_t off) {
  if (sp.G <= 0) return sp.n;
  const uint32_t f = FJD <= 0xffffffffu ? (uint32_t)off / (uint32_t)sp.JD : (uint32_t)(off / (size_t)sp.JD);
  return srf::bal_tile_slots((int)(f >> 5), sp.in_n, sp.U, sp.G);
}

__device__ __forceinline__ f4 sum_slab4(const float* __restrict__ slab, const SlabSplit& sp, size_t FJD, size_t off) {
  const int n = slab_count(sp, FJD, off);
  f4 a = ld4(slab + off);
#pragma unroll 4
  for (int c = 1; c < n; ++c) a += ld4(slab + (size_t)c * FJD + off);
  return a;
}

template <int DOUT>
__global__ void fwd_finish_kernel(const float* __restrict__ slab, SlabSplit sp, size_t FJD,
                                  const float* __restrict__ vc_in, float* __restrict__ s_out,
                                  float* __restrict__ vc_out, float* __restrict__ v_out) {
  constexpr int Q = DOUT / 4;
  const size_t idx = (size_t)blockIdx.x * blockDim.x + threadIdx.x;
  const bool ok = idx < FJD / 4;
  const size_t off = (ok ? idx : 0) * 4;
  const f4 sv = sum_slab4(slab, sp, FJD, off);
  const float n2 = qsum<Q>((sv.x * sv.x + sv.y * sv.y) + (sv.z * sv.z + sv.w * sv.w));
  if (!ok) return;
  const float fac = n2 / (1.f + n2) / sqrtf(n2 + kSquashEps);
  const f4 v = sv * fac;
  st4(s_out + off, sv);
  if (vc_out) st4(vc_out + off, vc_in ? v + ld4(vc_in + off) : v);
  if (v_out) st4(v_out + off, v);
}

template <int DOUT>
__global__ void bwd_finish_kernel(const float* __restrict__ slab, SlabSplit sp, size_t FJD,
                                  const float* __restrict__ a_init, float* __restrict__ A,
                                  const float* __restrict__ s, float* __restrict__ gs, float* __restrict__ zero4,
                                  size_t nz4, float* __restrict__ zero1) {
  constexpr int Q = DOUT / 4;
  const size_t idx = (size_t)blockIdx.x * blockDim.x + threadIdx.x;
  if (idx < nz4) st4(zero4 + idx * 4, f4{0.f, 0.f, 0.f, 0.f});
  if (zero1 != nullptr && idx == 0) *zero1 = 0.f;
  const bool ok = idx < FJD / 4;
  const size_t off = (ok ? idx : 0) * 4;
  f4 a;
  if (a_init) {
    a = ld4(a_init + off);
    if (ok) st4(A + off, f4{0.f, 0.f, 0.f, 0.f});
  } else {
    a = ld4(A + off) + sum_slab4(slab, sp, FJD, off);
    if (ok) st4(A + off, a);
  }
  const f4 sv = ld4(s + off);
  const float n2 = qsum<Q>((sv.x * sv.x + sv.y * sv.y) + (sv.z * sv.z + sv.w * sv.w));
  const float sa = qsum<Q>((sv.x * a.x + sv.y * a.y) + (sv.z * a.z + sv.w * a.w));
  if (!ok) return;
  const float rs = 1.f / sqrtf(n2 + kSquashEps);
  const float ip = 1.f / (1.f + n2);
  const float gfac = n2 * ip * rs;
  const float dg2 = 2.f * rs * ip * (ip - 0.5f * n2 / (n2 + kSquashEps)) * sa;
  st4(gs + off, a * gfac + sv * dg2);
}

struct PassCfg {
  int TW, NW;
};

PassCfg pass_cfg(const DrGeom& g) {
  const int NT = g.NT();
  int TW = 8;
  int NW = (NT + TW - 1) / TW;
  if (NW > 8) {
    TW = 16;
    NW = (NT + TW - 1) / TW;
  }
  return {TW, NW};
}

int auto_chunks(const DrGeom& g, int NW) {
  const int n_ftiles = (g.F() + 15) / 16;
  const int wg_per_cu = std::max(1, 8 / NW);
  const int slots = 256 * wg_per_cu;
  int best = 1;
  double best_cost = 1e30;
  for (int c = 1; c <= std::min(g.in_n(), 96); ++c) {
    const int rounds = (n_ftiles * c + slots - 1) / slots;
    const int len = (g.in_n() + c - 1) / c;
    double cost = (double)rounds * (len + 2);
    if (8 % c != 0 && c % 8 != 0) cost *= 1.05;
    cost *= 1.0 + 0.002 * c;
    if (cost < best_cost) {
      best_cost = cost;
      best = c;
    }
  }
  return best;
}

template <int D, int TW, int MODE>
void launch_pass(const DrGeom& g, int NW, int n_chunks, const float* emb, const float* W, const float* bias, int r,
                 const float* vc, const float* gsv, float* slab, float* stats, int want_acc, hipStream_t st) {
  const int n_ftiles = (g.F() + 15) / 16;
  const int chunk_len = (g.in_n() + n_chunks - 1) / n_chunks;
  const size_t shmem = (NW > 1) ? (size_t)2 * NW * 48 * sizeof(float) : 16;
  auto kern = r == 0 ? route_pass_kernel<D, D, TW, MODE, true> : route_pass_kernel<D, D, TW, MODE, false>;
  hipLaunchKernelGGL(kern, dim3(n_ftiles * n_chunks), dim3(64 * NW), shmem, st,
                     emb, W, bias, g.F(), g.T, g.N, g.lpad, g.in_n(), g.J, n_chunks, chunk_len, g.mask_first, r,
                     vc, gsv, slab, stats, want_acc);
}

template <int D, int MODE>
void dispatch_pass(const DrGeom& g, const PassCfg& pc, int n_chunks, const float* emb, const float* W,
                   const float* bias, int r, const float* vc, const float* gsv, float* slab, float* stats,
                   int want_acc, hipStream_t st) {
  if (pc.TW == 8)
    launch_pass<D, 8, MODE>(g, pc.NW, n_chunks, emb, W, bias, r, vc, gsv, slab, stats, want_acc, st);
  else
    launch_pass<D, 16, MODE>(g, pc.NW, n_chunks, emb, W, bias, r, vc, gsv, slab, stats, want_acc, st);
}

template <int D>
void launch_fwd_finish(const DrGeom& g, const float* slab, const SlabSplit& sp, const float* vc_in, float* s_out,
                       float* vc_out, float* v_out, hipStream_t st) {
  const size_t FJD = (size_t)g.F() * g.JD();
  hipLaunchKernelGGL((fwd_finish_kernel<D>), dim3((FJD / 4 + 255) / 256), dim3(256), 0, st, slab, sp, FJD,
                     vc_in, s_out, vc_out, v_out);
}

template <int D>
void launch_bwd_finish(const DrGeom& g, const float* slab, const SlabSplit& sp, const float* a_init, float* A,
                       const float* s, float* gs, hipStream_t st, float* zero = nullptr, size_t n_zero = 0,
                       float* zero1 = nullptr) {
  const size_t FJD = (size_t)g.F() * g.JD();
  const size_t nz4 = zero ? n_zero / 4 : 0;
  const size_t n = std::max(FJD / 4, nz4);
  hipLaunchKernelGGL((bwd_finish_kernel<D>), dim3((n + 255) / 256), dim3(256), 0, st, slab, sp, FJD, a_init,
                     A, s, gs, zero, nz4, zero1);
}

constexpr int gu_tw(int d) { return d >= 64 ? 4 : 2; }
constexpr int kGuNW = 4;

inline int gu_wgroups(const DrGeom& g) { return (g.NT() + kGuNW * gu_tw(g.dout) - 1) / (kGuNW * gu_tw(g.dout)); }
inline int padded_frames(const DrGeom& g) { return (g.F() + 15) / 16 * 16; }
inline int gu_window(const DrGeom& g) { return g.lpad + g.rpad + 1; }
inline size_t gu_lds_bytes(const DrGeom& g, int nw, int n_per) {
  return (size_t)nw * (15 + gu_window(g)) * gu_row_stride(n_per, g.din) * sizeof(float);
}
constexpr size_t kGuLdsMax = 64 * 1024;

int gu_n_per(const DrGeom& g, int nw) {
  const int base = (g.F() + 15) / 16 * gu_wgroups(g);
  const int slots = 256 * 4;
  int best = 1;
  double best_cost = 1e30;
  for (int n_per = 1; n_per <= g.N; ++n_per) {
    if (n_per > 1 && gu_lds_bytes(g, nw, n_per) > kGuLdsMax) break;
    const int chunks = (g.N + n_per - 1) / n_per;
    const int rounds = (base * chunks + slots - 1) / slots;
    const double cost = (double)rounds * (gu_window(g) * n_per + 4);
    if (cost < best_cost) {
      best_cost = cost;
      best = n_per;
    }
  }
  return best;
}

inline size_t gux16_lds_bytes(const DrGeom& g, int n_per) {
  return (size_t)kGux16NW * (31 + gu_window(g)) * (n_per * 32 + 4) * sizeof(float);
}
constexpr size_t kGux16LdsMax = (160 / kGux16Occ - 4) * 1024;
int gux16_n_per(const DrGeom& g, int jgpw) {
  const int base = (g.F() + 31) / 32 * ((g.J + kGux16NW - 1) / kGux16NW / jgpw);
  const int slots = 256 * kGux16Occ;
  int best = 1;
  double best_cost = 1e30;
  for (int n_per = 1; n_per <= g.N; ++n_per) {
    if (n_per > 1 && gux16_lds_bytes(g, n_per) > kGux16LdsMax) break;
    const int chunks = (g.N + n_per - 1) / n_per;
    const int rounds = (base * chunks + slots - 1) / slots;
    const double cost = (double)rounds * (gu_window(g) * n_per * jgpw + 4);
    if (cost < best_cost) {
      best_cost = cost;
      best = n_per;
    }
  }
  return best;
}

struct Gw2Plan {
  int cap, n_rt, n_cc, S, ft_per;
  size_t pstride;
};
constexpr int gw3_capsules(int d) { return d <= 16 ? 8 : 4; }

enum class GxPass {
  kRecompute,
  kStored,
  kStored16,
};
enum class GwPass {
  kFromGu,
  kGw2,
  kGw3,
  kGw16s,
};

struct BwdWs {
  size_t A, gs, slab, stats, gu_t, xT, WT;
  size_t gumax;
  size_t p32;
  size_t gl;
  size_t gwpart;
  size_t bytes;
};

struct DrPlan {
  DrGeom g;
  bool fwd32;
  srf::Fwd32Plan p32;
  srf::Fwd32Cpl cpl;
  Gw2Plan gw2;
  bool can_store;
  bool couplings;
  PassCfg pc;
  int chunks;
  int plan_arg;
  GxPass gx;
  GwPass gw;
  size_t fwd_bytes;
  BwdWs ws;
  int JP() const { return p32.JDp / g.dout; }
  const float* hdr(const float* cpl_base) const { return srf::fwd32_hdr(p32, cpl_base + cpl.planes); }
};

#ifndef SRF_GUX16_JGPW
#define SRF_GUX16_JGPW 2
#endif
template <int R>
void launch_gux16(const DrGeom& g, const float* WT, const float* hdr, const float* saved, const float* gs,
                  float* g_emb, const float* cst, const float* glst, int JP, float* gumax, hipStream_t st) {
  const int n_all = (g.J + kGux16NW - 1) / kGux16NW;
  const int jgpw = n_all % SRF_GUX16_JGPW == 0 ? SRF_GUX16_JGPW : 1;
  const int n_wgroups = n_all / jgpw;
  const int n_per = gux16_n_per(g, jgpw);
  const int n_chunks = (g.N + n_per - 1) / n_per;
  int grid = (g.F() + 31) / 32 * n_wgroups * n_chunks;
  if (SRF_GUX16_XCD) grid = (grid + 7) / 8 * 8;
  hipLaunchKernelGGL((route_gux16_kernel<R>), dim3(grid), dim3(64 * kGux16NW), gux16_lds_bytes(g, n_per), st, WT, hdr,
                     g.F(), g.T, g.N, g.lpad, g.in_n(), g.J, g.mask_first, n_wgroups, n_chunks, n_per, saved, gs, g_emb,
                     cst, glst, JP, gumax, jgpw);
}

template <int D, int R>
void launch_gu(const DrPlan& p, const float* emb, const float* W, const float* WT, const float* bias,
               const float* saved, const float* gs, const float* stats, float* gu_t, float* g_emb, hipStream_t st,
               const float* cst, const float* glst, const float* hdr, float* gumax) {
  const DrGeom& g = p.g;
  if constexpr (D == 32 && R >= 2 && R <= 4) {
    if (p.gx == GxPass::kStored16) {
      launch_gux16<R>(g, WT, hdr, saved, gs, g_emb, cst, glst, p.JP(), gumax, st);
      return;
    }
  }
  const int n_ftiles = (g.F() + 15) / 16;
  const int n_wgroups = gu_wgroups(g);
  constexpr int TW = gu_tw(D);
  const int nw = std::min(kGuNW, (g.NT() + TW - 1) / TW);
  const int n_per = gu_n_per(g, nw);
  const int n_chunks = (g.N + n_per - 1) / n_per;
  const int nslots = 15 + gu_window(g);
  const size_t lds = gu_lds_bytes(g, nw, n_per);
  if constexpr (R >= 2 && D <= 32) {
    if (p.gx == GxPass::kStored) {
      hipLaunchKernelGGL((route_gux_kernel<D, TW, R>), dim3(n_ftiles * n_wgroups * n_chunks), dim3(64 * nw), lds, st,
                         WT, g.F(), g.T, g.N, g.lpad, g.in_n(), g.J, g.mask_first, n_wgroups, n_chunks, n_per, saved,
                         gs, g_emb, nslots, cst, glst, p.JP());
      return;
    }
  }
  const bool ldsacc = lds <= kGuLdsMax;
  hipLaunchKernelGGL((ldsacc ? route_gu_kernel<D, D, TW, R, true> : route_gu_kernel<D, D, TW, R, false>),
                     dim3(n_ftiles * n_wgroups * n_chunks), dim3(64 * nw), ldsacc ? lds : 0, st, emb, W, WT, bias, g.F(),
                     padded_frames(g), g.T, g.N, g.lpad, g.rpad, g.in_n(), g.J, g.mask_first, n_wgroups, n_chunks, n_per,
                     saved, gs, stats, gu_t, g_emb, nslots, nullptr, nullptr, 0);
}

template <int V>
using Int = std::integral_constant<int, V>;
// ... 19 lines not shown
}

template <int D>
int launch_gw2(const DrPlan& pl, const float* xT, const float* saved, const float* gs, const float* cst,
               const float* glst, float* gwp, float* gbp, hipStream_t st, const float* hdr, const float* gumax) {
  static_assert(D <= 32, "couplings are stored by the 32x32 forward");
  const DrGeom& g = pl.g;
  const Gw2Plan& p = pl.gw2;
  const int JP = pl.JP(), Fp = padded_frames(g);
  const int grid = p.n_rt * p.n_cc * p.S;
  if constexpr (D == 32) {
    if (pl.gw == GwPass::kGw16s) {
      constexpr int VW = SRF_GW16S_LDSVEC, NG = VW == 2 ? 2 : 1;
      const int tasks = p.n_rt * ((p.n_cc + NG - 1) / NG) * p.S;
      const int grid16 = SRF_GW16S_XCD ? (tasks + 7) / 8 * 8 : tasks;
      const _Float16* x16 = reinterpret_cast<const _Float16*>(xT);
      hipLaunchKernelGGL((g.iters == 2 ? route_gw16s_kernel<2, kGw16Cap, VW> : route_gw16s_kernel<3, kGw16Cap, VW>),
                         dim3(grid16), dim3(256 * NG), 0, st, x16, hdr, gumax, saved, gs, cst, glst, g.F(), Fp, g.in_n(),
                         g.J, g.mask_first, JP, p.n_rt, p.S, p.ft_per, gwp, gbp, p.pstride);
      SRF_LAUNCH_CHECK("route_gw16s");
      return SRF_OK;
    }
  }
  if (pl.gw == GwPass::kGw3) {
    constexpr int CAP = gw3_capsules(D);
    hipLaunchKernelGGL((g.iters == 2 ? route_gw3_kernel<D, 2, CAP> : route_gw3_kernel<D, 3, CAP>), dim3(grid), dim3(256),
                       0, st, xT, saved, gs, cst, glst, g.F(), Fp, g.in_n(), g.J, g.mask_first, JP, p.n_rt, p.S, p.ft_per,
                       gwp, gbp, p.pstride);
    SRF_LAUNCH_CHECK("route_gw3");
    return SRF_OK;
  }
  hipLaunchKernelGGL((g.iters == 4 ? route_gw2_kernel<D, 4> : route_gw2_kernel<D, 5>), dim3(grid), dim3(256), 0, st, xT,
                     saved, gs, cst, glst, g.F(), Fp, g.in_n(), g.J, g.mask_first, JP, p.n_rt, p.n_cc, p.S, p.ft_per, gwp,
                     gbp, p.pstride);
  SRF_LAUNCH_CHECK("route_gw2");
  return SRF_OK;
}


inline bool use_fwd32(const DrGeom& g) { return srf::fwd32_supported(g.din, g.dout, g.J); }

inline bool use_gux16(const DrGeom& g) {
  return g.din == 32 && g.dout == 32 && g.iters >= 2 && g.iters <= 4 &&
         gux16_lds_bytes(g, 1) <= kGux16LdsMax;
}
inline bool use_gw16s(const DrGeom& g) { return use_gux16(g) && g.iters <= 3; }

inline int gw3_cap(const DrGeom& g) { return g.iters <= 3 && g.din <= 32 ? gw3_capsules(g.din) : 0; }

Gw2Plan gw2_plan(const DrGeom& g, GwPass kind) {
  const bool g16 = kind == GwPass::kGw16s, g3 = kind == GwPass::kGw3;
  Gw2Plan p{};
  const int NT = g.NT();
  const int NCT = g16 ? 2 : (g.din + 15) / 16;
  p.n_rt = g16 ? (g.J + 3) / 4 : (NT + 3) / 4;
  p.cap = g16 ? kGw16Cap : g3 ? gw3_capsules(g.din) : (g.din <= 16 ? 8 : 4);
  const int slots = g16 ? 512 : g3 ? 2 * 768 : 512;
  const double per_tile = g16 ? 120.0 : 200.0;
  p.n_cc = (g.in_n() + p.cap - 1) / p.cap;
  const int NFT = padded_frames(g) / 16;
  p.pstride = (size_t)g.in_n() * g.JD() * (g.din + 1);
  const int base = p.n_rt * p.n_cc;
  double best = 1e30;
  for (int S0 = 1; S0 <= NFT; ++S0) {
    const int ft_per = (NFT + S0 - 1) / S0;
    const int S = (NFT + ft_per - 1) / ft_per;
    const int rounds = (base * S + slots - 1) / slots;
    const double work = (double)rounds * ft_per * p.cap * NCT * per_tile / 2.4e9;
    const double slab = S > 1 ? 2.0 * S * p.pstride * 4 / 4e12 : 0.0;
    if (work + slab < best) {
      best = work + slab;
      p.S = S;
      p.ft_per = ft_per;
    }
  }
  return p;
}

inline bool couplings_ok(const DrGeom& g, const srf::Fwd32Cpl& cpl) {
  if (!use_fwd32(g) || g.iters < 2 || g.din > 32) return false;
  constexpr size_t kLim = size_t(1) << 31;
  const int TW = gu_tw(g.dout);
  const int nw = std::min(kGuNW, (g.NT() + TW - 1) / TW);
  return gu_lds_bytes(g, nw, 1) <= kGuLdsMax && cpl.total * 4 < kLim && (size_t)g.F() * g.JD() * 4 * g.iters < kLim;
}

inline bool plan_balanced(int n_chunks) { return n_chunks > 0 && (n_chunks & srf::kBalFlag) != 0; }
inline bool plan_arg_ok(const DrPlan& p, int n_chunks) {
  return plan_balanced(n_chunks) ? p.fwd32 : (n_chunks >= 1 && n_chunks <= p.g.in_n());
}

void resolve(DrPlan& p, const DrGeom& g, int n_chunks, bool have_couplings) {
  p = DrPlan{};
  p.g = g;
  p.fwd32 = use_fwd32(g);
  p.pc = pass_cfg(g);
  p.chunks = plan_balanced(n_chunks) ? auto_chunks(g, p.pc.NW) : n_chunks;
  p.fwd_bytes = plan_balanced(n_chunks) ? 0 : (size_t)n_chunks * ((size_t)g.B * g.T + 1) * g.J * g.dout * sizeof(float);
  GwPass stored_gw = GwPass::kGw2;
  if (p.fwd32) {
    p.p32 = srf::fwd32_plan(g, n_chunks);
    p.fwd_bytes = std::max(p.fwd_bytes, srf::fwd32_workspace(p.p32));
    p.cpl = srf::fwd32_cpl_layout(p.p32, g);
    stored_gw = use_gw16s(g) ? GwPass::kGw16s : gw3_cap(g) ? GwPass::kGw3 : GwPass::kGw2;
    p.gw2 = gw2_plan(g, stored_gw);
  }
  p.plan_arg = p.fwd32 ? p.p32.plan_arg : n_chunks == 0 ? auto_chunks(g, p.pc.NW) : p.chunks;
  p.can_store = couplings_ok(g, p.cpl);
  p.couplings = have_couplings && p.can_store;
  p.gx = !p.couplings ? GxPass::kRecompute : use_gux16(g) ? GxPass::kStored16 : GxPass::kStored;
  p.gw = p.couplings ? stored_gw : GwPass::kFromGu;

  const size_t F = g.F(), JD = g.JD(), in_n = g.in_n(), Fp = padded_frames(g);
  size_t off = 0;
  auto take = [&](size_t nfloat) {
    const size_t o = off;
    off += srf::align_up(nfloat * sizeof(float), 256);
    return o / sizeof(float);
  };
  BwdWs& w = p.ws;
  w.A = take(F * JD);
  w.gs = take((size_t)g.iters * F * JD);
  w.slab = take((size_t)p.chunks * F * JD);
  w.stats = take((size_t)(g.iters - 1) * F * in_n * 2);
  w.gu_t = take(in_n * (size_t)g.NT() * 16 * Fp);
  w.xT = take(in_n * g.din * Fp);
  w.WT = take(in_n * JD * g.din);
  w.gumax = take(64);
  if (p.fwd32) {
    w.p32 = take((srf::fwd32_scratch_bytes(p.p32) + 3) / 4);
    w.gl = take((size_t)std::max(g.iters - 1, 1) * srf::fwd32_frame_stride(g.F()) * in_n * p.JP());
    w.gwpart = take((size_t)p.gw2.S * p.gw2.pstride);
  }
  w.bytes = off;
}

int check_geom(const DrGeom& g) {
  SRF_REQUIRE(g.B > 0 && g.T > 0 && g.N > 0 && g.J > 1, "bad shape B=%d T=%d N=%d J=%d", g.B, g.T, g.N, g.J);
  SRF_REQUIRE(g.lpad >= 0 && g.rpad >= 0, "negative window pad");
  SRF_REQUIRE(g.iters >= 1 && g.iters <= 5, "routing iterations must be in [1,5], got %d", g.iters);
  SRF_REQUIRE(g.din == 8 || g.din == 16 || g.din == 32 || g.din == 64, "unsupported in_d %d", g.din);
  SRF_REQUIRE(g.dout == g.din, "in_d (%d) != out_d (%d) is not supported", g.din, g.dout);
  SRF_REQUIRE((long long)g.F() * g.in_n() * g.JD() < (1LL << 40), "problem too large");
  return SRF_OK;
}

inline SlabSplit uniform_split(int n) { return SlabSplit{n, 0, 0, 0, 0}; }
inline SlabSplit pass_split(const DrGeom& g, const srf::Fwd32Plan& p) {
  return p.bal_G > 0 ? SlabSplit{p.n_slots, p.bal_G, p.bal_U, g.in_n(), g.JD()} : uniform_split(p.n_chunks);
}

template <int D>
int fwd_impl(const DrPlan& p, const float* emb, const float* W, const float* bias, float* v_out, float* saved,
             float* couplings, float* slab, hipStream_t st) {
  const DrGeom& g = p.g;
  const srf::Fwd32Plan& plan = p.p32;
  const srf::Fwd32Cpl& cl = p.cpl;
  const size_t FJD = (size_t)g.F() * g.JD();
  hipEvent_t* ev0 = t_ev_start;
  hipEvent_t* ev1 = t_ev_stop;
  const int nev = t_ev_n;
  t_ev_start = t_ev_stop = nullptr;
  t_ev_n = 0;
  float* bsum = nullptr;
  void* planes = slab;
  void* scratch = slab;
  if (p.fwd32) {
    float *WT = nullptr, *xT = nullptr;
    if (p.couplings) {
      planes = couplings + cl.planes;
      WT = couplings + cl.WT;
      xT = couplings + cl.xT;
    } else {
      scratch = static_cast<char*>(static_cast<void*>(slab)) + srf::fwd32_planes_bytes(plan);
    }
    const int rc = srf::fwd32_prepare(plan, g, emb, W, bias, planes, scratch, WT, xT, st,
                                      p.gx == GxPass::kStored16, p.gw == GwPass::kGw16s);
    if (rc) return rc;
  } else {
    bsum = slab + (size_t)p.chunks * FJD;
    const int chunk_len = (g.in_n() + p.chunks - 1) / p.chunks;
    hipLaunchKernelGGL(bias_chunk_sum_kernel, dim3((p.chunks * g.JD() + 255) / 256), dim3(256), 0, st, bias,
                       g.in_n(), g.JD(), p.chunks, chunk_len, bsum);
    SRF_LAUNCH_CHECK("bias_chunk_sum");
  }
  for (int r = 0; r < g.iters; ++r) {
    const float* vc = r > 0 ? saved + (size_t)(2 * (r - 1) + 1) * FJD : nullptr;
    if (r < nev) SRF_HIP_TRY(hipEventRecord(ev0[r], st));
    if (p.fwd32 && r == 0 && srf::fwd32_first_full_supported(plan, g)) {
      const int rc = srf::fwd32_first_full(plan, g, planes, scratch, saved, saved + FJD,
                                           g.iters == 1 ? v_out : nullptr, st);
      if (rc) return rc;
      if (r < nev) SRF_HIP_TRY(hipEventRecord(ev1[r], st));
      continue;
    }
    if (p.fwd32) {
      float *cst = nullptr, *lzst = nullptr;
      if (p.couplings && r > 0) {
        const size_t blk = (size_t)srf::fwd32_frame_stride(g.F()) * g.in_n();
        cst = couplings + cl.c + (size_t)(r - 1) * blk * p.JP();
        lzst = couplings + cl.lz + (size_t)(r - 1) * blk;
      }
      const int rc = srf::fwd32_pass(plan, g, r == 0, planes, scratch, vc, cst, lzst, st);
      if (rc) return rc;
    } else {
      dispatch_pass<D, MODE_FWD>(g, p.pc, p.chunks, emb, W, bias, r, vc, r == 0 ? bsum : nullptr, slab, nullptr, 1, st);
    }
    SRF_LAUNCH_CHECK("route_pass(fwd)");
    if (r < nev) SRF_HIP_TRY(hipEventRecord(ev1[r], st));
    const bool last = r == g.iters - 1;
    launch_fwd_finish<D>(g, p.fwd32 ? srf::fwd32_slab(plan, scratch) : slab,
                         !p.fwd32 ? uniform_split(p.chunks) : r == 0 ? uniform_split(plan.n_chunks) : pass_split(g, plan),
                         vc, saved + (size_t)(2 * r) * FJD, last ? nullptr : saved + (size_t)(2 * r + 1) * FJD,
                         last ? v_out : nullptr, st);
    SRF_LAUNCH_CHECK("fwd_finish");
  }
  return SRF_OK;
}

template <int D>
int bwd_weights_impl(const DrPlan& p, const float* emb, float* g_W, float* g_bias, float* ws, hipStream_t st,
                     const float* saved, const float* couplings) {
  const DrGeom& g = p.g;
  const BwdWs& w = p.ws;
  const int Fp = padded_frames(g);
  if constexpr (D <= 32) {
    if (p.gw != GwPass::kFromGu) {
      const Gw2Plan& gp = p.gw2;
      const bool direct = gp.S == 1;
      float* gwp = direct ? g_W : ws + w.gwpart;
      float* gbp = direct ? g_bias : ws + w.gwpart + (size_t)g.in_n() * g.JD() * g.din;
      const int rc = launch_gw2<D>(p, couplings + p.cpl.xT, saved, ws + w.gs, couplings + p.cpl.c, ws + w.gl, gwp, gbp,
                                   st, p.hdr(couplings), ws + w.gumax);
      if (rc || direct) return rc;
      const size_t nw4 = (size_t)g.in_n() * g.JD() * g.din / 4, n4 = gp.pstride / 4;
      hipLaunchKernelGGL(gw_reduce_kernel, dim3((n4 + 255) / 256), dim3(256), 0, st, ws + w.gwpart, gp.S, n4,
                         gp.pstride, g_W, nw4, g_bias);
      SRF_LAUNCH_CHECK("gw_reduce");
      return SRF_OK;
    }
  }
  {
    SRF_REQUIRE(g.din <= 64, "window_xt tile holds din <= 64, got %d", g.din);
    const int tiles = (Fp + kXtFrames - 1) / kXtFrames;
    hipLaunchKernelGGL(window_xt_kernel, dim3(g.in_n() * tiles), dim3(256), 0, st, emb, g.F(), Fp, g.T, g.N, g.din,
                       g.lpad, g.in_n(), ws + w.xT);
    SRF_LAUNCH_CHECK("window_xt");
  }
  {
    const int tasks = g.in_n() * g.NT();
    hipLaunchKernelGGL((route_gw_kernel<D>), dim3((tasks + 3) / 4), dim3(256), 0, st, ws + w.gu_t, ws + w.xT, Fp,
                       g.in_n(), g.JD(), g_W, g_bias);
    SRF_LAUNCH_CHECK("route_gw");
  }
  return SRF_OK;
}

template <int D>
int bwd_impl(const DrPlan& p, const float* emb, const float* W, const float* bias, const float* saved,
             const float* couplings, const float* g_v, float* g_emb, float* g_W, float* g_bias, float* ws,
             hipStream_t st, bool with_weights) {
  const DrGeom& g = p.g;
  const BwdWs& w = p.ws;
  const srf::Fwd32Plan& plan = p.p32;
  const srf::Fwd32Cpl& cl = p.cpl;
  const size_t FJD = (size_t)g.F() * g.JD();
  const int R = g.iters;
  const bool p32 = p.couplings;
  float* const gsv = ws + w.gs;
  const size_t n_emb = (size_t)g.F() * g.N * g.din;
  launch_bwd_finish<D>(g, nullptr, uniform_split(1), g_v, ws + w.A, saved + (size_t)(2 * (R - 1)) * FJD,
                       gsv + (size_t)(R - 1) * FJD, st, p32 ? g_emb : nullptr, n_emb, p32 ? ws + w.gumax : nullptr);
  SRF_LAUNCH_CHECK("bwd_finish");
  for (int r = R - 1; r >= 1; --r) {
    const float* vc = saved + (size_t)(2 * (r - 1) + 1) * FJD;
    float* stats_r = ws + w.stats + (size_t)(r - 1) * g.F() * g.in_n() * 2;
    if (p32) {
      const size_t blk = (size_t)srf::fwd32_frame_stride(g.F()) * g.in_n();
      const int JP = p.JP();
      const int rc = srf::bwd32_pass(plan, g, couplings + cl.planes, ws + w.p32,
                                     couplings + cl.c + (size_t)(r - 1) * blk * JP,
                                     couplings + cl.lz + (size_t)(r - 1) * blk, gsv + (size_t)r * FJD, stats_r,
                                     ws + w.gl + (size_t)(r - 1) * blk * JP, st);
      if (rc) return rc;
      launch_bwd_finish<D>(g, srf::fwd32_slab(plan, ws + w.p32), pass_split(g, plan), nullptr, ws + w.A,
                           saved + (size_t)(2 * (r - 1)) * FJD, gsv + (size_t)(r - 1) * FJD, st);
    } else {
      dispatch_pass<D, MODE_BWD>(g, p.pc, p.chunks, emb, W, bias, r, vc, gsv + (size_t)r * FJD, ws + w.slab, stats_r, 1,
                                 st);
      SRF_LAUNCH_CHECK("route_pass(bwd)");
      launch_bwd_finish<D>(g, ws + w.slab, uniform_split(p.chunks), nullptr, ws + w.A,
                           saved + (size_t)(2 * (r - 1)) * FJD, gsv + (size_t)(r - 1) * FJD, st);
    }
    SRF_LAUNCH_CHECK("bwd_finish");
  }
  if (!p32) {
    const size_t total = (size_t)g.in_n() * g.JD() * g.din + n_emb;
    hipLaunchKernelGGL(transpose_w_kernel, dim3((total + 255) / 256), dim3(256), 0, st, W, g.in_n(), g.JD(), g.din,
                       ws + w.WT, g_emb, n_emb);
    SRF_LAUNCH_CHECK("transpose_w");
  }
  dispatch_iters(R, [&](auto r) {
    launch_gu<D, r>(p, emb, W, p32 ? couplings + cl.WT : ws + w.WT, bias, saved, gsv, ws + w.stats, ws + w.gu_t, g_emb,
                    st, p32 ? couplings + cl.c : nullptr, p32 ? ws + w.gl : nullptr,
                    p32 ? p.hdr(couplings) : nullptr, ws + w.gumax);
  });
  SRF_LAUNCH_CHECK("route_gu");
  return with_weights ? bwd_weights_impl<D>(p, emb, g_W, g_bias, ws, st, saved, couplings) : SRF_OK;
}

int enter(DrPlan& p, const DrGeom& g, int n_chunks, bool pointers, bool have_couplings, bool forward,
          size_t workspace_bytes) {
  if (const int rc = check_geom(g)) return rc;
  SRF_REQUIRE(pointers, "null pointer argument");
  resolve(p, g, n_chunks, have_couplings);
  SRF_REQUIRE(plan_arg_ok(p, n_chunks), "n_chunks %d: neither in [1, %d] nor a balanced plan of the 32x32 passes",
              n_chunks, g.in_n());
  const size_t need = forward ? p.fwd_bytes : p.ws.bytes;
  if (workspace_bytes < need) {
    srf::set_error("%s workspace too small: %zu < %zu", forward ? "forward" : "backward", workspace_bytes, need);
    return SRF_EWORKSPACE;
  }
  return SRF_OK;
}

int route_dr_bwd_entry(const float* emb, const float* W, const float* bias, int B, int T, int N, int din, int lpad,
                       int rpad, int J, int dout, int iters, int mask_first, int n_chunks, const float* saved,
                       const float* couplings, const float* g_v, float* g_emb, float* g_W, float* g_bias,
                       void* workspace, size_t workspace_bytes, void* stream, bool with_weights) {
  DrPlan p;
  const int rc = enter(p, DrGeom{B, T, N, din, lpad, rpad, J, dout, iters, mask_first ? 1 : 0}, n_chunks,
                       emb && W && bias && saved && g_v && g_emb && g_W && g_bias && workspace, couplings != nullptr,
                       false, workspace_bytes);
  if (rc) return rc;
  return dispatch_din(din, [&](auto D) {
    return bwd_impl<D>(p, emb, W, bias, saved, couplings, g_v, g_emb, g_W, g_bias, static_cast<float*>(workspace),
                       static_cast<hipStream_t>(stream), with_weights);
  });
}

DrPlan query(int B, int T, int N, int din, int lpad, int rpad, int J, int dout, int iters, int n_chunks) {
  DrPlan p;
  resolve(p, DrGeom{B, T, N, din, lpad, rpad, J, dout, iters, 0}, n_chunks, false);
  return p;
}

}

extern "C" {

int srf_route_dr_set_timing_events(void* const* starts, void* const* stops, int n) {
  SRF_REQUIRE(n >= 0 && (n == 0 || (starts && stops)), "bad timing event arrays");
  t_ev_start = (hipEvent_t*)starts;
  t_ev_stop = (hipEvent_t*)stops;
  t_ev_n = n;
  return SRF_OK;
}

int srf_route_dr_auto_chunks(int B, int T, int N, int din, int lpad, int rpad, int J, int dout) {
  return query(B, T, N, din, lpad, rpad, J, dout, 1, 0).plan_arg;
}

int srf_route_dr_split_table(int B, int T, int N, int din, int lpad, int rpad, int J, int dout, int n_chunks,
                             int* info, int* table, int capacity) {
  const bool shape_ok = B > 0 && T > 0 && N > 0 && lpad >= 0 && rpad >= 0;
  const DrPlan plan = shape_ok ? query(B, T, N, din, lpad, rpad, J, dout, 1, n_chunks) : DrPlan{};
  SRF_REQUIRE(shape_ok && plan.fwd32, "split_table: not a 32x32-pass shape");
  SRF_REQUIRE(n_chunks == 0 || plan_arg_ok(plan, n_chunks), "split_table: bad plan argument %d", n_chunks);
  SRF_REQUIRE(info != nullptr && capacity >= 0 && (table != nullptr || capacity == 0), "split_table: null argument");
  const srf::Fwd32Plan& p = plan.p32;
  const int in_n = plan.g.in_n();
  const bool bal = p.bal_G > 0;
  const int n_wg = bal ? p.bal_G : p.n_ftiles * p.n_chunks;
  info[0] = bal ? 1 : 0;
  info[1] = n_wg;
  info[2] = p.n_ftiles * in_n;
  info[3] = p.n_slots;
  info[4] = p.plan_arg;
  int n = 0;
  auto emit = [&](int w, int ft, int i0, int i1, int slot) {
    if (n < capacity) {
      int* row = table + (size_t)n * 5;
      row[0] = w, row[1] = ft, row[2] = i0, row[3] = i1, row[4] = slot;
    }
    ++n;
  };
  for (int w = 0; w < n_wg; ++w) {
    if (!bal) {
      const int ft = w / p.n_chunks, slot = w - ft * p.n_chunks;
      const int i0 = slot * p.chunk_len;
      emit(w, ft, std::min(i0, in_n), std::min(in_n, i0 + p.chunk_len), slot);
      continue;
    }
    int u = srf::bal_first(w, p.bal_U, p.bal_G);
    const int u1 = srf::bal_first(w + 1, p.bal_U, p.bal_G);
    while (u < u1) {
      const int ft = u / in_n, i0 = u - ft * in_n, i1 = std::min(in_n, i0 + (u1 - u));
      emit(w, ft, i0, i1, w - srf::bal_owner(ft * in_n, p.bal_U, p.bal_G));
      u += i1 - i0;
    }
  }
  return n;
}

size_t srf_route_dr_saved_floats(int B, int T, int J, int dout, int iters) {
  return (size_t)2 * iters * B * T * J * dout;
}

size_t srf_route_dr_fwd_workspace(int B, int T, int N, int din, int lpad, int rpad, int J, int dout, int iters,
                                  int n_chunks) {
  (void)iters;
  return query(B, T, N, din, lpad, rpad, J, dout, 1, n_chunks).fwd_bytes;
}

size_t srf_route_dr_bwd_workspace(int B, int T, int N, int din, int lpad, int rpad, int J, int dout, int iters,
                                  int n_chunks) {
  return query(B, T, N, din, lpad, rpad, J, dout, iters, n_chunks).ws.bytes;
}

size_t srf_route_dr_coupling_floats(int B, int T, int N, int din, int lpad, int rpad, int J, int dout, int iters) {
  const DrPlan p = query(B, T, N, din, lpad, rpad, J, dout, iters, 0);
  return p.can_store ? p.cpl.total : 0;
}

int srf_route_dr_operand_layout(int B, int T, int N, int din, int lpad, int rpad, int J, int dout, int iters,
                                long long* out) {
  SRF_REQUIRE(out != nullptr, "operand_layout: null argument");
  DrPlan p;
  const DrGeom g{B, T, N, din, lpad, rpad, J, dout, iters, 0};
  if (const int rc = check_geom(g)) return rc;
  resolve(p, g, 0, true);
  if (!p.couplings) {
    srf::set_error("operand_layout: no coupling storage for this shape");
    return SRF_EUNSUPPORTED;
  }
  const srf::Fwd32Shape& s = p.p32;
  const size_t in_n = g.in_n(), Fp = padded_frames(g);
  const size_t pl = p.cpl.planes;
  const size_t v[SRF_DR_LAYOUT_N] = {pl,
                                     2 * in_n * s.JDp * g.din * 2,
                                     pl + s.ws_w / 4,
                                     in_n * s.JDp * 8,
                                     pl + (s.ws_w + s.ws_b) / 4,
                                     2 * s.xplane * 2,
                                     pl + (s.ws_w + s.ws_b + s.ws_x) / 4,
                                     3 * sizeof(float),
                                     p.cpl.WT,
                                     in_n * g.din * ((size_t)g.NT() * 16) * 4,
                                     p.cpl.xT,
                                     in_n * g.din * Fp * 4,
                                     (size_t)s.JDp,
                                     s.xplane,
                                     Fp,
                                     p.gx == GxPass::kStored16 ? 1u : 0u,
                                     p.gw == GwPass::kGw16s ? 1u : 0u};
  for (int k = 0; k < SRF_DR_LAYOUT_N; ++k) out[k] = (long long)v[k];
  return SRF_OK;
}

int srf_route_dr_fwd(const float* emb, const float* W, const float* bias, int B, int T, int N, int din, int lpad,
                     int rpad, int J, int dout, int iters, int mask_first, int n_chunks, float* v_out, float* saved,
                     void* workspace, size_t workspace_bytes, void* stream) {
  return srf_route_dr_fwd_ex(emb, W, bias, B, T, N, din, lpad, rpad, J, dout, iters, mask_first, n_chunks, v_out,
                             saved, nullptr, workspace, workspace_bytes, stream);
}

int srf_route_dr_fwd_ex(const float* emb, const float* W, const float* bias, int B, int T, int N, int din, int lpad,
                        int rpad, int J, int dout, int iters, int mask_first, int n_chunks, float* v_out,
                        float* saved, float* couplings, void* workspace, size_t workspace_bytes, void* stream) {
  DrPlan p;
  const int rc = enter(p, DrGeom{B, T, N, din, lpad, rpad, J, dout, iters, mask_first ? 1 : 0}, n_chunks,
                       emb && W && bias && v_out && saved && workspace, couplings != nullptr, true, workspace_bytes);
  if (rc) return rc;
  return dispatch_din(din, [&](auto D) {
    return fwd_impl<D>(p, emb, W, bias, v_out, saved, couplings, static_cast<float*>(workspace),
                       static_cast<hipStream_t>(stream));
  });
}

int srf_route_dr_bwd(const float* emb, const float* W, const float* bias, int B, int T, int N, int din, int lpad,
                     int rpad, int J, int dout, int iters, int mask_first, int n_chunks, const float* saved,
                     const float* g_v, float* g_emb, float* g_W, float* g_bias, void* workspace,
                     size_t workspace_bytes, void* stream) {
  return route_dr_bwd_entry(emb, W, bias, B, T, N, din, lpad, rpad, J, dout, iters, mask_first, n_chunks, saved,
                            nullptr, g_v, g_emb, g_W, g_bias, workspace, workspace_bytes, stream, true);
}

int srf_route_dr_bwd_ex(const float* emb, const float* W, const float* bias, int B, int T, int N, int din, int lpad,
                        int rpad, int J, int dout, int iters, int mask_first, int n_chunks, const float* saved,
                        const float* couplings, const float* g_v, float* g_emb, float* g_W, float* g_bias,
                        void* workspace, size_t workspace_bytes, void* stream) {
  return route_dr_bwd_entry(emb, W, bias, B, T, N, din, lpad, rpad, J, dout, iters, mask_first, n_chunks, saved,
                            couplings, g_v, g_emb, g_W, g_bias, workspace, workspace_bytes, stream, true);
}

int srf_route_dr_bwd_data(const float* emb, const float* W, const float* bias, int B, int T, int N, int din,
                          int lpad, int rpad, int J, int dout, int iters, int mask_first, int n_chunks,
                          const float* saved, const float* g_v, float* g_emb, void* workspace,
                          size_t workspace_bytes, void* stream) {
  return srf_route_dr_bwd_data_ex(emb, W, bias, B, T, N, din, lpad, rpad, J, dout, iters, mask_first, n_chunks, saved,
                                  nullptr, g_v, g_emb, workspace, workspace_bytes, stream);
}

int srf_route_dr_bwd_data_ex(const float* emb, const float* W, const float* bias, int B, int T, int N, int din,
                             int lpad, int rpad, int J, int dout, int iters, int mask_first, int n_chunks,
                             const float* saved, const float* couplings, const float* g_v, float* g_emb,
                             void* workspace, size_t workspace_bytes, void* stream) {
  float* unused = reinterpret_cast<float*>(workspace);
  return route_dr_bwd_entry(emb, W, bias, B, T, N, din, lpad, rpad, J, dout, iters, mask_first, n_chunks, saved,
                            couplings, g_v, g_emb, unused, unused, workspace, workspace_bytes, stream, false);
}

int srf_route_dr_bwd_weights(const float* emb, int B, int T, int N, int din, int lpad, int rpad, int J, int dout,
                             int iters, int mask_first, int n_chunks, float* g_W, float* g_bias, void* workspace,
                             size_t workspace_bytes, void* stream) {
  return srf_route_dr_bwd_weights_ex(emb, B, T, N, din, lpad, rpad, J, dout, iters, mask_first, n_chunks, nullptr,
                                     nullptr, g_W, g_bias, workspace, workspace_bytes, stream);
}

int srf_route_dr_bwd_weights_ex(const float* emb, int B, int T, int N, int din, int lpad, int rpad, int J, int dout,
                                int iters, int mask_first, int n_chunks, const float* saved, const float* couplings,
                                float* g_W, float* g_bias, void* workspace, size_t workspace_bytes, void* stream) {
  DrPlan p;
  const int rc = enter(p, DrGeom{B, T, N, din, lpad, rpad, J, dout, iters, mask_first ? 1 : 0}, n_chunks,
                       emb && g_W && g_bias && workspace, couplings != nullptr && saved != nullptr, false,
                       workspace_bytes);
  if (rc) return rc;
  return dispatch_din(din, [&](auto D) {
    return bwd_weights_impl<D>(p, emb, g_W, g_bias, static_cast<float*>(workspace),
                               static_cast<hipStream_t>(stream), saved, couplings);
  });
}

}
```

### srf_amd/ops.py

```python
import ctypes
import os

import torch

from . import _lib


def _ptr(t):
    return ctypes_void(t.data_ptr())


def ctypes_void(addr):
    return ctypes.c_void_p(addr)


def _stream():
    return ctypes_void(torch.cuda.current_stream().cuda_stream)


def _check_dev(name, t, shape):
    if not t.is_cuda:
        raise ValueError(f'{name} must be a HIP device tensor (no CPU path exists)')
    if t.dtype != torch.float32:
        raise ValueError(f'{name} must be float32, got {t.dtype}')
    if tuple(t.shape) != tuple(shape):
        raise ValueError(f'{name} has shape {tuple(t.shape)}, expected {tuple(shape)}')
    if not t.is_contiguous():
        raise ValueError(f'{name} must be contiguous')


def _grad_target(p):
    if getattr(p, '_srf_flat', False) and p.grad is not None:
        return p.grad, True
    return torch.empty_like(p), False


def _returned(target_flags):
    return [None if inplace else t for t, inplace in target_flags]


class RouteGeom:

    def __init__(self, B, T, N, din, lpad, rpad, J, dout, iters, mask_first, n_chunks=0):
        self.B, self.T, self.N, self.din = B, T, N, din
        self.lpad, self.rpad, self.J, self.dout = lpad, rpad, J, dout
        self.iters, self.mask_first = iters, int(bool(mask_first))
        self.in_n = N * (lpad + rpad + 1)
        self.timing = None
        self.store_couplings = True
        L = _lib.lib()
        if n_chunks <= 0:
            n_chunks = L.srf_route_dr_auto_chunks(B, T, N, din, lpad, rpad, J, dout)
        self.n_chunks = n_chunks

    def args(self):
        return (self.B, self.T, self.N, self.din, self.lpad, self.rpad, self.J, self.dout, self.iters,
                self.mask_first, self.n_chunks)

    def ws_args(self):
        return (self.B, self.T, self.N, self.din, self.lpad, self.rpad, self.J, self.dout, self.iters,
                self.n_chunks)


DR_GW_SIDE = False
_dr_side = {}
_dr_pending = []
_dr_keep = []
_SIDE_KEEP = os.environ.get('SRF_SIDE_KEEP', '1') != '0'
_SIDE_WAIT = os.environ.get('SRF_SIDE_WAIT', 'event')


def _dr_side_stream(dev):
    s = _dr_side.get(dev.index)
    if s is None:
        s = _dr_side[dev.index] = torch.cuda.Stream(device=dev)
    return s


def _dr_issue_pending():
    while _dr_pending:
        dev, ev, launch, keep = _dr_pending.pop(0)
        side = _dr_side_stream(dev)
        if _SIDE_WAIT == 'tail':
            side.wait_stream(torch.cuda.current_stream(dev))
        else:
            side.wait_event(ev)
        launch(ctypes_void(side.cuda_stream))
        for t in keep:
            if t is not None:
                t.record_stream(side)
        if _SIDE_KEEP:
            _dr_keep.append(keep)


def dr_side_join():
    _dr_issue_pending()
    for s in _dr_side.values():
        torch.cuda.current_stream(s.device).wait_stream(s)
    _dr_keep.clear()


_dr_state = {'queued': False, 'main': None}


def _dr_backward_done():
    _dr_state['queued'] = False
    main, _dr_state['main'] = _dr_state['main'], None
    _dr_issue_pending()
    if main is not None:
        s = _dr_side.get(main.device.index)
        if s is not None:
            main.wait_stream(s)
            _dr_keep.clear()


def dr_reset():
    _dr_pending.clear()
    _dr_keep.clear()
    _dr_state['queued'] = False
    _dr_state['main'] = None


def _defer_side(dev, ev, launch, keep):
    _dr_pending.append((dev, ev, launch, keep))
    _dr_state['main'] = torch.cuda.current_stream(dev)
    if not _dr_state['queued']:
        torch.autograd.Variable._execution_engine.queue_callback(_dr_backward_done)
        _dr_state['queued'] = True


class DynamicRouting(torch.autograd.Function):

    @staticmethod
    def forward(ctx, emb, W, bias, geom, need_bwd=True):
        g = geom
        _check_dev('emb', emb, (g.B, g.T, g.N, g.din))
        _check_dev('W', W, (g.in_n, g.J, g.dout, g.din))
        _check_dev('bias', bias, (g.in_n, g.J, g.dout))
        L = _lib.lib()
        dev = emb.device
        v = torch.empty((g.B, g.T, g.J, g.dout), device=dev, dtype=torch.float32)
        saved = torch.empty(L.srf_route_dr_saved_floats(g.B, g.T, g.J, g.dout, g.iters), device=dev,
                            dtype=torch.float32)
        ws_bytes = L.srf_route_dr_fwd_workspace(*g.ws_args())
        ws = torch.empty(max(ws_bytes, 16), device=dev, dtype=torch.uint8)
        if g.timing is not None:
            starts, stops, n = g.timing.pop(0)
            _lib.check(L.srf_route_dr_set_timing_events(starts, stops, n), 'set_timing_events')
            if not g.timing:
                g.timing = None
        nc = L.srf_route_dr_coupling_floats(g.B, g.T, g.N, g.din, g.lpad, g.rpad, g.J, g.dout, g.iters) \
            if need_bwd and g.store_couplings else 0
        cpl = torch.empty(nc, device=dev, dtype=torch.float32) if nc else None
        rc = L.srf_route_dr_fwd_ex(_ptr(emb), _ptr(W), _ptr(bias), *g.args(), _ptr(v), _ptr(saved),
                                   _ptr(cpl) if cpl is not None else None, _ptr(ws), ws_bytes, _stream())
        _lib.check(rc, 'srf_route_dr_fwd_ex')
        ctx.geom = g
        ctx.params = (W, bias)
        ctx.couplings = cpl
        ctx.save_for_backward(emb, W, bias, saved)
        return v

    @staticmethod
    def backward(ctx, g_v):
        emb, W, bias, saved = ctx.saved_tensors
        g = ctx.geom
        g_v = g_v.contiguous()
        L = _lib.lib()
        g_emb = torch.empty_like(emb)
        tW, tb = _grad_target(ctx.params[0]), _grad_target(ctx.params[1])
        g_W, g_b = tW[0], tb[0]
        ws_bytes = L.srf_route_dr_bwd_workspace(*g.ws_args())
        ws = torch.empty(ws_bytes, device=emb.device, dtype=torch.uint8)
        cpl = ctx.couplings
        ctx.couplings = None
        cp = _ptr(cpl) if cpl is not None else None
        _dr_issue_pending()
        if DR_GW_SIDE and cpl is not None and tW[1] and tb[1]:
            rc = L.srf_route_dr_bwd_data_ex(_ptr(emb), _ptr(W), _ptr(bias), *g.args(), _ptr(saved), cp, _ptr(g_v),
                                            _ptr(g_emb), _ptr(ws), ws_bytes, _stream())
            _lib.check(rc, 'srf_route_dr_bwd_data_ex')
            ev = getattr(g, '_gw_event', None)
            if ev is None:
                ev = g._gw_event = torch.cuda.Event()
            ev.record()

            def launch(st, emb=emb, saved=saved, cpl=cpl, g_W=g_W, g_b=g_b, ws=ws):
                _lib.check(L.srf_route_dr_bwd_weights_ex(_ptr(emb), *g.args(), _ptr(saved), _ptr(cpl), _ptr(g_W),
                                                         _ptr(g_b), _ptr(ws), ws_bytes, st),
                           'srf_route_dr_bwd_weights_ex')
            _defer_side(emb.device, ev, launch, (emb, saved, cpl, ws))
        else:
            rc = L.srf_route_dr_bwd_ex(_ptr(emb), _ptr(W), _ptr(bias), *g.args(), _ptr(saved), cp, _ptr(g_v),
                                       _ptr(g_emb), _ptr(g_W), _ptr(g_b), _ptr(ws), ws_bytes, _stream())
            _lib.check(rc, 'srf_route_dr_bwd_ex')
        return (g_emb, *_returned([tW, tb]), None, None)


def dynamic_routing(emb, W, bias, geom):
    need_bwd = torch.is_grad_enabled() and (emb.requires_grad or W.requires_grad or bias.requires_grad)
    return DynamicRouting.apply(emb, W, bias, geom, need_bwd)


class SequentialRouting(torch.autograd.Function):

    @staticmethod
    def forward(ctx, emb, W, bias, geom):
        g = geom
        _check_dev('emb', emb, (g.B, g.T, g.N, g.din))
        _check_dev('W', W, (g.in_n, g.J, g.dout, g.din))
        _check_dev('bias', bias, (g.in_n, g.J, g.dout))
        L = _lib.lib()
        dev = emb.device
        v = torch.empty((g.B, g.T, g.J, g.dout), device=dev, dtype=torch.float32)
        saved = torch.empty(L.srf_route_sdr_saved_floats(g.B, g.T, g.J, g.dout), device=dev, dtype=torch.float32)
        geo = (g.B, g.T, g.N, g.din, g.lpad, g.rpad, g.J, g.dout)
        ws_bytes = L.srf_route_sdr_fwd_workspace(*geo)
        ws = torch.empty(ws_bytes, device=dev, dtype=torch.uint8)
        rc = L.srf_route_sdr_fwd(_ptr(emb), _ptr(W), _ptr(bias), *geo, g.iters, g.mask_first, _ptr(v), _ptr(saved),
                                 _ptr(ws), ws_bytes, _stream())
        _lib.check(rc, 'srf_route_sdr_fwd')
        ctx.geom = g
        ctx.params = (W, bias)
        ctx.save_for_backward(emb, W, bias, saved)
        return v

    @staticmethod
    def backward(ctx, g_v):
        emb, W, bias, saved = ctx.saved_tensors
        g = ctx.geom
        g_v = g_v.contiguous()
        L = _lib.lib()
        g_emb = torch.empty_like(emb)
        tW, tb = _grad_target(ctx.params[0]), _grad_target(ctx.params[1])
        geo = (g.B, g.T, g.N, g.din, g.lpad, g.rpad, g.J, g.dout)
        ws_bytes = L.srf_route_sdr_bwd_workspace(*geo, g.iters)
        ws = torch.empty(ws_bytes, device=emb.device, dtype=torch.uint8)
        rc = L.srf_route_sdr_bwd(_ptr(emb), _ptr(W), _ptr(bias), *geo, g.iters, g.mask_first, _ptr(saved),
                                 _ptr(g_v), _ptr(g_emb), _ptr(tW[0]), _ptr(tb[0]), _ptr(ws), ws_bytes, _stream())
        _lib.check(rc, 'srf_route_sdr_bwd')
        return (g_emb, *_returned([tW, tb]), None)


def sequential_routing(emb, W, bias, geom):
    return SequentialRouting.apply(emb, W, bias, geom)


CNNFE_PARAMS = ('conv0a_kernel', 'conv0a_bias', 'conv0b_kernel', 'conv0b_bias', 'bn0_gamma', 'bn0_beta',
                'conv1a_kernel', 'conv1a_bias', 'conv1b_kernel', 'conv1b_bias', 'bn1_gamma', 'bn1_beta')


CNNFE_WGRAD_SIDE = False
_cnnfe_events = {}


def cnnfe_out_dims(T, feat_dim):
    import ctypes
    t2, f2 = ctypes.c_int(), ctypes.c_int()
    _lib.check(_lib.lib().srf_cnnfe_out_dims(T, feat_dim, ctypes.byref(t2), ctypes.byref(f2)), 'srf_cnnfe_out_dims')
    return t2.value, f2.value


class CnnFe(torch.autograd.Function):

    @staticmethod
    def forward(ctx, feats, inp_len_i32, moving, training, drop_p, seed, *params):
        B, T, Fd = feats.shape
        _check_dev('feats', feats, (B, T, Fd))
        L = _lib.lib()
        T2, F2 = cnnfe_out_dims(T, Fd)
        dev = feats.device
        out = torch.empty((B, T2, F2, 64), device=dev, dtype=torch.float32)
        sb = L.srf_cnnfe_saved_bytes(B, T, Fd, 64)
        saved = torch.empty(sb, device=dev, dtype=torch.uint8)
        wb = L.srf_cnnfe_fwd_workspace(B, T, Fd, 64)
        ws = torch.empty(wb, device=dev, dtype=torch.uint8)
        rc = L.srf_cnnfe_fwd(_ptr(feats), _ptr(inp_len_i32), B, T, Fd, 64, *[_ptr(p) for p in params],
                             *[_ptr(m) for m in moving], int(bool(training)), float(drop_p), int(seed), _ptr(out),
                             _ptr(saved), sb, _ptr(ws), wb, _stream())
        _lib.check(rc, 'srf_cnnfe_fwd')
        ctx.meta = (B, T, Fd, float(drop_p) if training else 0.0, int(seed))
        ctx.params = params
        ctx.save_for_backward(feats, inp_len_i32, saved, *params)
        return out

    @staticmethod
    def backward(ctx, g_out):
        feats, inp_len, saved, *params = ctx.saved_tensors
        B, T, Fd, drop_p, seed = ctx.meta
        P = dict(zip(CNNFE_PARAMS, params))
        targets = [_grad_target(p) for p in ctx.params]
        G = dict(zip(CNNFE_PARAMS, [t for t, _ in targets]))
        L = _lib.lib()
        wb = L.srf_cnnfe_bwd_workspace(B, T, Fd, 64)
        ws = torch.empty(wb, device=feats.device, dtype=torch.uint8)
        g_out = g_out.contiguous()
        args = (_ptr(feats), _ptr(inp_len), B, T, Fd, 64, _ptr(P['bn0_gamma']), _ptr(P['conv1a_kernel']),
                _ptr(P['conv1b_kernel']), _ptr(P['bn1_gamma']), drop_p, seed, _ptr(saved), _ptr(g_out),
                *[_ptr(G[k]) for k in CNNFE_PARAMS], _ptr(ws), wb)
        inplace = dict(zip(CNNFE_PARAMS, [t[1] for t in targets]))
        if CNNFE_WGRAD_SIDE and inplace['conv1a_kernel'] and inplace['conv1b_kernel']:
            _dr_issue_pending()
            _lib.check(L.srf_cnnfe_bwd_parts(1, *args, _stream()), 'srf_cnnfe_bwd_parts(prep)')
            dev = feats.device
            ev = _cnnfe_events.get(dev.index)
            if ev is None:
                ev = _cnnfe_events[dev.index] = torch.cuda.Event()
            ev.record()
            _lib.check(L.srf_cnnfe_bwd_parts(2, *args, _stream()), 'srf_cnnfe_bwd_parts(data)')

            def launch(st):
                _lib.check(L.srf_cnnfe_bwd_parts(4, *args, st), 'srf_cnnfe_bwd_parts(wgrad)')
            _defer_side(dev, ev, launch, (feats, inp_len, saved, g_out, ws))
        else:
            _lib.check(L.srf_cnnfe_bwd(*args, _stream()), 'srf_cnnfe_bwd')
        return (None, None, None, None, None, None, *_returned(targets))


def cnnfe(feats, inp_len_i32, params, moving, training, drop_p, seed):
    return CnnFe.apply(feats, inp_len_i32, moving, training, drop_p, seed, *params)


CAPS_PARAMS = ('proj_kernel', 'proj_bias', 'encaps1_kernel', 'encaps1_bias', 'encaps2_kernel', 'encaps2_bias',
               'ln_input_gamma', 'ln_input_beta')


class PrimaryCaps(torch.autograd.Function):

    @staticmethod
    def forward(ctx, X, inp_len_i32, PH, PD, training, p_caps, p_in, seed, variant, *params):
        proj_scale, pos_enc = variant
        B, T = X.shape[:2]
        K = X.shape[2] * X.shape[3]
        _check_dev('X', X, tuple(X.shape))
        L = _lib.lib()
        z = torch.empty((B, T, PH, PD), device=X.device, dtype=torch.float32)
        sb = L.srf_primary_caps_saved_bytes(B, T, PH, PD)
        saved = torch.empty(sb, device=X.device, dtype=torch.uint8)
        tr = int(bool(training))
        rc = L.srf_primary_caps_fwd_ex(_ptr(X), _ptr(inp_len_i32), B, T, K, PH, PD, *[_ptr(p) for p in params], tr,
                                       float(p_caps), float(p_in), int(seed), float(proj_scale), int(bool(pos_enc)),
                                       _ptr(z), _ptr(saved), sb, _stream())
        _lib.check(rc, 'srf_primary_caps_fwd_ex')
        ctx.meta = (B, T, K, PH, PD, tr, float(p_caps), float(p_in), int(seed), float(proj_scale))
        ctx.params = params
        ctx.save_for_backward(X, inp_len_i32, saved, *params)
        return z

    @staticmethod
    def backward(ctx, g_z):
        X, inp_len, saved, *params = ctx.saved_tensors
        B, T, K, PH, PD, tr, p_caps, p_in, seed, proj_scale = ctx.meta
        P = dict(zip(CAPS_PARAMS, params))
        L = _lib.lib()
# ... 883 lines not shown
```

### srf_amd/sequence_router.py

```python
import math

import numpy as np
import torch

from . import ops

SQUASH_EPS = 1e-7
LENGTH_EPS = 1e-7
LENGTH_EPS_EINSUM = 1e-9
CAPS_TYPES = ('lowmemory', 'einsum', 'naive')
LN_EPS = 1e-3
BN_EPS = 1e-3
BN_MOMENTUM = 0.99
CNN_DROPOUT = 0.2


def _replica_id():
    import torch.distributed as dist
    return dist.get_rank() if dist.is_available() and dist.is_initialized() else 0


class SequenceRouter(torch.nn.Module):

    iter = -1
# ... 72 lines not shown
            spec.append((f'b{l}', (in_n, out_n, out_d), 'normal0.1'))
            spec.append((f'ln_mid{l + 1}_gamma', (out_n * out_d,), 'ones'))
            spec.append((f'ln_mid{l + 1}_beta', (out_n * out_d,), 'zeros'))
        spec.append(('ln_output_gamma', (class_n,), 'ones'))
        spec.append(('ln_output_beta', (class_n,), 'zeros'))
        self._spec = spec

        offsets, off = {}, 0
        for name, shape, _ in spec:
            offsets[name] = off
            off += (int(np.prod(shape)) + 63) // 64 * 64
        self.n_flat = off
        self.flat_params = torch.zeros(off, device=dev, dtype=torch.float32)
        self.flat_grad = torch.zeros(off, device=dev, dtype=torch.float32)
        self.params = torch.nn.ParameterDict()
        rng = np.random.default_rng(seed)
        for name, shape, init in spec:
            n = int(np.prod(shape))
            view = self.flat_params[offsets[name]:offsets[name] + n].view(shape)
            with torch.no_grad():
                view.copy_(torch.from_numpy(self._init_value(rng, shape, init)))
            p = torch.nn.Parameter(view)
            p.grad = self.flat_grad[offsets[name]:offsets[name] + n].view(shape)
            p._srf_flat = True
            self.params[name] = p
        self.offsets = offsets
        for k in range(self.cnn_n):
            self.register_buffer(f'bn{k}_moving_mean', torch.zeros(self.nfilt, device=dev))
            self.register_buffer(f'bn{k}_moving_var', torch.ones(self.nfilt, device=dev))
        self._geoms = {}
        self._identity = {}
        if self.caps_type == 'lowmemory' and not self.is_context:
            for l, (in_n, out_n, out_d, in_d) in enumerate(shapes):
                if out_d != in_d:
                    raise ValueError(f'lowmemory DR needs equal capsule dims, layer {l}: {in_d} -> {out_d}')
                eye = torch.eye(in_d, device=dev, dtype=torch.float32).expand(in_n, out_n, in_d, in_d)
                self._identity[l] = (eye.contiguous(), torch.zeros((in_n, out_n, out_d), device=dev))
        if logger is not None:
            logger.info('Layer x %d, Iter x %d, Init %s, Win %d (l:%d, r:%d), ' % (
                self.enc_num, SequenceRouter.iter, 'SDR' if self.is_context else 'DR', self.window, self.lpad,
                self.rpad))

    def _init_value(self, rng, shape, init):
        if init == 'zeros':
            return np.zeros(shape, np.float32)
        if init == 'ones':
            return np.ones(shape, np.float32)
        if init == 'normal0.1':
            return (0.1 * rng.standard_normal(shape)).astype(np.float32)
        if self.init == 'uniform':
            return rng.uniform(-0.05, 0.05, size=shape).astype(np.float32)
        rf = int(np.prod(shape[:-2])) if len(shape) > 2 else 1
        fan_in, fan_out = shape[-2] * rf, shape[-1] * rf
        lim = math.sqrt(6.0 / (fan_in + fan_out))
        return rng.uniform(-lim, lim, size=shape).astype(np.float32)

    def P(self, name):
        return self.params[name]

    def zero_grad(self, set_to_none=False):
        self.flat_grad.zero_()

    def load_params(self, named):
        with torch.no_grad():
            for k, v in named.items():
                key = k.replace('.', '_')
                if key.endswith('moving_mean') or key.endswith('moving_var'):
                    getattr(self, key).copy_(torch.as_tensor(v, dtype=torch.float32))
                else:
                    self.params[key].copy_(torch.as_tensor(v, dtype=torch.float32))

    def export_params(self):
        out = {}
        for k, v in self.params.items():
            head, _, tail = k.rpartition('_')
            key = f'{head}.{tail}' if tail in ('kernel', 'bias', 'gamma', 'beta') else k
            out[key] = v.detach().cpu().numpy()
        for k in range(self.cnn_n):
            out[f'bn{k}.moving_mean'] = getattr(self, f'bn{k}_moving_mean').cpu().numpy()
            out[f'bn{k}.moving_var'] = getattr(self, f'bn{k}_moving_var').cpu().numpy()
        return out

    def _geom(self, l, B, T):
        key = (l, B, T)
        g = self._geoms.get(key)
        if g is None:
            in_n, out_n, out_d, in_d = self.layer_shapes[l]
            N = in_n // self.window
            g = ops.RouteGeom(B, T, N, in_d, self.lpad, self.rpad, out_n, out_d, self.route_iters,
                              l == self.enc_num - 1, self.n_chunks_override.get(l, 0))
            self._geoms[key] = g
        return g

    def _stack_plan(self, B, T):
        key = ('sdr_stack', B, T)
        p = self._geoms.get(key)
        if p is None:
            layers = []
            for l, (in_n, out_n, out_d, in_d) in enumerate(self.layer_shapes):
                layers.append((in_n // self.window, in_d, out_n, out_d, int(l == self.enc_num - 1)))
            p = ops.SdrStackPlan(B, T, layers, self.lpad, self.rpad, self.route_iters, pose_fp8=self.pose_fp8,
                                 **self.sdr_options)
            self._geoms[key] = p
        return p

    def _on_grad(self, t, names):
        hook = self.grad_hook
        if hook is not None and t.requires_grad and torch.is_grad_enabled():
            def fire(g, names=tuple(names)):
                hook(names)
            t.register_hook(fire)

    def _next_seed(self):
        self._calls += 1
        return (self._seed_base * 0x9E3779B1 + self._calls) % (1 << 63)

    def forward(self, feats, input_lengths=None, training=False, **kwargs):
        inp_len = input_lengths
        if not torch.is_tensor(inp_len):
            inp_len = torch.as_tensor(inp_len)
        il32 = inp_len.to(device=feats.device, dtype=torch.int32).contiguous()
        drop = bool(training) and self.dropout_enabled
        seed = self._next_seed() if drop else 0
        moving = [getattr(self, n) for n in ('bn0_moving_mean', 'bn0_moving_var', 'bn1_moving_mean',
                                             'bn1_moving_var')]
        x = ops.cnnfe(feats.contiguous(), il32, [self.P(k) for k in ops.CNNFE_PARAMS], moving, training,
                      CNN_DROPOUT if drop else 0.0, seed)
        self._on_grad(x, ops.CAPS_PARAMS)
        emb = ops.primary_caps(x, il32, self.caps_inp_n, self.caps_inp_d, training, CNN_DROPOUT if drop else 0.0,
                               self.inp_dropout if drop else 0.0, seed, [self.P(k) for k in ops.CAPS_PARAMS],
                               self.proj_scale, self.caps_type == 'einsum')
        B, T2 = emb.shape[:2]
        p_mid = self.inn_dropout if drop else 0.0
        if self.is_context and self.enc_num > 1 and self.sdr_stack:
            last = self.enc_num - 1
            params = [self.P(f'{w}{l}') for l in range(self.enc_num) for w in ('W', 'b')]
            params += [self.P(f'ln_mid{l + 1}_{t}') for l in range(last) for t in ('gamma', 'beta')]
            self._on_grad(emb, [f'{w}{l}' for l in range(self.enc_num) for w in ('W', 'b')]
                          + [f'ln_mid{l + 1}_{t}' for l in range(last) for t in ('gamma', 'beta')])
            plan = self._stack_plan(B, T2)
            plan.collectives_overlap = self.grad_buckets is not None and self.grad_buckets.active()
            v = ops.sdr_stack(emb, plan, training, p_mid, seed, params)
            self._on_grad(v, [f'ln_mid{last + 1}_gamma', f'ln_mid{last + 1}_beta', 'ln_output_gamma',
                              'ln_output_beta'])
            return ops.CapsHead.apply(v, self.P(f'ln_mid{last + 1}_gamma'), self.P(f'ln_mid{last + 1}_beta'),
                                      self.P('ln_output_gamma'), self.P('ln_output_beta'), training, p_mid, seed,
                                      last, self.length_eps)
        for l in range(self.enc_num):
            route = ops.sequential_routing if self.is_context else ops.dynamic_routing
            W, bias = self._identity.get(l, (self.P(f'W{l}'), self.P(f'b{l}')))
            if l in self._identity and torch.is_grad_enabled():
                self.P(f'W{l}').grad.zero_()
                self.P(f'b{l}').grad.zero_()
            self._on_grad(emb, [f'W{l}', f'b{l}'])
            v = route(emb, W, bias, self._geom(l, B, T2))
            norms = [f'ln_mid{l + 1}_gamma', f'ln_mid{l + 1}_beta']
            self._on_grad(v, norms if l < self.enc_num - 1 else norms + ['ln_output_gamma', 'ln_output_beta'])
            if l < self.enc_num - 1:
                emb = ops.CapsNorm.apply(v, self.P(f'ln_mid{l + 1}_gamma'), self.P(f'ln_mid{l + 1}_beta'), training,
                                         p_mid, seed, l)
            else:
                return ops.CapsHead.apply(v, self.P(f'ln_mid{l + 1}_gamma'), self.P(f'ln_mid{l + 1}_beta'),
                                          self.P('ln_output_gamma'), self.P('ln_output_beta'), training, p_mid,
                                          seed, l, self.length_eps)
```

Baseline: 3.049 million frames/s.

## Fuse capsule layer norm and head into dynamic routing kernels

```diff
diff --git a/include/srf.h b/include/srf.h
--- a/include/srf.h
+++ b/include/srf.h
@@ -38,6 +38,32 @@
                              int lpad, int rpad, int J, int dout, int iters, int mask_first, int n_chunks,
                              const float* saved, const float* couplings, const float* g_v, float* g_emb,
                              void* workspace, size_t workspace_bytes, void* stream);
+int srf_route_dr_norm_supported(int B, int T, int N, int din, int lpad, int rpad, int J, int dout, int iters);
+int srf_route_dr_fwd_norm_ex(const float* emb, const float* W, const float* bias, int B, int T, int N, int din,
+                             int lpad, int rpad, int J, int dout, int iters, int mask_first, int n_chunks,
+                             float* saved, float* couplings, void* workspace, size_t workspace_bytes,
+                             const float* gamma, const float* beta, int training, float p, unsigned long long seed,
+                             int layer, float* y, float* stat, void* stream);
+int srf_route_dr_fwd_head_ex(const float* emb, const float* W, const float* bias, int B, int T, int N, int din,
+                             int lpad, int rpad, int J, int dout, int iters, int mask_first, int n_chunks,
+                             float* v_out, float* saved, float* couplings, void* workspace, size_t workspace_bytes,
+                             const float* gamma_mid, const float* beta_mid, const float* gamma_out,
+                             const float* beta_out, int training, float p, unsigned long long seed, int layer,
+                             float length_eps, float* logits, float* stat, float* lens, void* stream);
+int srf_route_dr_bwd_norm_ex(const float* emb, const float* W, const float* bias, int B, int T, int N, int din,
+                             int lpad, int rpad, int J, int dout, int iters, int mask_first, int n_chunks,
+                             const float* saved, const float* couplings, const float* g_y, const float* gamma,
+                             const float* stat, int training, float p, unsigned long long seed, int layer,
+                             float* g_emb, float* g_W, float* g_bias, float* g_gamma, float* g_beta,
+                             void* workspace, size_t workspace_bytes, void* norm_workspace,
+                             size_t norm_workspace_bytes, void* stream);
+int srf_route_dr_bwd_norm_data_ex(const float* emb, const float* W, const float* bias, int B, int T, int N, int din,
+                                  int lpad, int rpad, int J, int dout, int iters, int mask_first, int n_chunks,
+                                  const float* saved, const float* couplings, const float* g_y, const float* gamma,
+                                  const float* stat, int training, float p, unsigned long long seed, int layer,
+                                  float* g_emb, float* g_gamma, float* g_beta, void* workspace,
+                                  size_t workspace_bytes, void* norm_workspace, size_t norm_workspace_bytes,
+                                  void* stream);
 int srf_set_seed_source(const void* step_counter);
 int srf_set_fault_flag(void* flag);
 int srf_route_dr_bwd(const float* emb, const float* W, const float* bias, int B, int T, int N, int din, int lpad,
diff --git a/srf_amd/_lib.py b/srf_amd/_lib.py
--- a/srf_amd/_lib.py
+++ b/srf_amd/_lib.py
@@ -56,6 +56,18 @@
     'srf_route_dr_bwd_ex': (_c_int, [_vp, _vp, _vp] + [_c_int] * 11 + [_vp] * 7 + [_c_size, _vp]),
     'srf_route_dr_bwd_data_ex': (_c_int, [_vp, _vp, _vp] + [_c_int] * 11 + [_vp] * 5 + [_c_size, _vp]),
     'srf_route_dr_bwd_weights_ex': (_c_int, [_vp] + [_c_int] * 11 + [_vp] * 5 + [_c_size, _vp]),
+    'srf_route_dr_norm_supported': (_c_int, [_c_int] * 9),
+    'srf_route_dr_fwd_norm_ex': (_c_int, [_vp, _vp, _vp] + [_c_int] * 11 + [_vp, _vp, _vp, _c_size, _vp, _vp, _c_int,
+                                                                           ctypes.c_float, ctypes.c_ulonglong, _c_int,
+                                                                           _vp, _vp, _vp]),
+    'srf_route_dr_fwd_head_ex': (_c_int, [_vp, _vp, _vp] + [_c_int] * 11 + [_vp, _vp, _vp, _vp, _c_size] + [_vp] * 4
+                                 + [_c_int, ctypes.c_float, ctypes.c_ulonglong, _c_int, ctypes.c_float] + [_vp] * 4),
+    'srf_route_dr_bwd_norm_ex': (_c_int, [_vp, _vp, _vp] + [_c_int] * 11 + [_vp] * 5
+                                 + [_c_int, ctypes.c_float, ctypes.c_ulonglong, _c_int] + [_vp] * 6
+                                 + [_c_size, _vp, _c_size, _vp]),
+    'srf_route_dr_bwd_norm_data_ex': (_c_int, [_vp, _vp, _vp] + [_c_int] * 11 + [_vp] * 5
+                                      + [_c_int, ctypes.c_float, ctypes.c_ulonglong, _c_int] + [_vp] * 4
+                                      + [_c_size, _vp, _c_size, _vp]),
     'srf_route_sdr_saved_floats': (_c_size, [_c_int] * 4),
     'srf_route_sdr_fwd_workspace': (_c_size, [_c_int] * 8),
     'srf_route_sdr_bwd_workspace': (_c_size, [_c_int] * 9),
diff --git a/srf_amd/csrc/caps.hip b/srf_amd/csrc/caps.hip
--- a/srf_amd/csrc/caps.hip
+++ b/srf_amd/csrc/caps.hip
@@ -4,13 +4,13 @@
 #include "srf_common.h"
 #include "srf_reduce.h"
 #include "srf_rng.h"
+#include "caps_norm_dev.h"
 #include "../../include/srf.h"
 
 namespace {
 
 constexpr float kSquashEps = 1e-7f;
 constexpr float kLengthEps = 1e-7f;
-constexpr float kLnEps = 1e-3f;
 constexpr int kMaxVec = 4096;
 
 __device__ __forceinline__ int ceil_div_len(int len, int div) { return (len + div - 1) / div; }
@@ -27,11 +27,6 @@
   __syncthreads();
   a = red[0] + red[1] + red[2] + red[3];
   b = red[4] + red[5] + red[6] + red[7];
-}
-
-__device__ __forceinline__ float drop_mult(bool on, unsigned long long seed, unsigned stream, size_t idx, float p) {
-  if (!on) return 1.f;
-  return srf_keep(seed, stream, idx, p) ? 1.f / (1.f - p) : 0.f;
 }
 
 __device__ __forceinline__ float pos_enc(int t, int p, int PH) {
@@ -640,108 +635,6 @@
 }
 
 template <int NPL>
-__device__ __forceinline__ void capsnorm_fwd_wave(const float* __restrict__ x, const float* __restrict__ gamma,
-                                                  const float* __restrict__ beta, bool drop, float p,
-                                                  unsigned long long seed, unsigned stream, float* __restrict__ y,
-                                                  float* __restrict__ stat, int f, int lane) {
-  constexpr int n = 64 * NPL, NV = NPL / 4;
-  const f4* xr = reinterpret_cast<const f4*>(x + (size_t)f * n);
-  f4 v[NV];
-  float s1 = 0.f;
-#pragma unroll
-  for (int k = 0; k < NV; ++k) {
-    v[k] = xr[k * 64 + lane];
-    s1 += (v[k].x + v[k].y) + (v[k].z + v[k].w);
-  }
-  const float mean = wave_sum(s1) / n;
-  float s2 = 0.f;
-#pragma unroll
-  for (int k = 0; k < NV; ++k) {
-    const f4 d = v[k] - mean;
-    s2 += (d.x * d.x + d.y * d.y) + (d.z * d.z + d.w * d.w);
-  }
-  const float rstd = 1.f / sqrtf(wave_sum(s2) / n + kLnEps);
-  f4* yr = reinterpret_cast<f4*>(y + (size_t)f * n);
-#pragma unroll
-  for (int k = 0; k < NV; ++k) {
-    const int q = k * 64 + lane;
-    const f4 g = reinterpret_cast<const f4*>(gamma)[q], b = reinterpret_cast<const f4*>(beta)[q];
-    const size_t gi = (size_t)f * n + 4 * q;
-    f4 o;
-#pragma unroll
-    for (int c = 0; c < 4; ++c) o[c] = ((v[k][c] - mean) * rstd * g[c] + b[c]) * drop_mult(drop, seed, stream, gi + c, p);
-    yr[q] = o;
-  }
-  if (lane == 0) {
-    stat[4 * f] = mean;
-    stat[4 * f + 1] = rstd;
-  }
-}
-
-template <int NPL>
-__device__ __forceinline__ void caps_head_fwd_wave(const float* __restrict__ x, const float* __restrict__ gamma,
-                                                   const float* __restrict__ beta, bool drop, float p,
-                                                   unsigned long long seed, unsigned stream,
-                                                   float* __restrict__ stat, int D, const float* __restrict__ gamma_o,
-                                                   const float* __restrict__ beta_o, float* __restrict__ logits,
-                                                   float* __restrict__ lens, float len_eps, int f, int lane) {
-  constexpr int n = 64 * NPL, NV = NPL / 4;
-  const int LPC = D / 4, J = n / D;
-  const f4* xr = reinterpret_cast<const f4*>(x + (size_t)f * n);
-  f4 v[NV];
-  float s1 = 0.f;
-#pragma unroll
-  for (int k = 0; k < NV; ++k) {
-    v[k] = xr[k * 64 + lane];
-    s1 += (v[k].x + v[k].y) + (v[k].z + v[k].w);
-  }
-  const float mean = wave_sum(s1) / n;
-  float s2 = 0.f;
-#pragma unroll
-  for (int k = 0; k < NV; ++k) {
-    const f4 d = v[k] - mean;
-    s2 += (d.x * d.x + d.y * d.y) + (d.z * d.z + d.w * d.w);
-  }
-  const float rstd = 1.f / sqrtf(wave_sum(s2) / n + kLnEps);
-  float L[NV];
-  float t1 = 0.f;
-#pragma unroll
-  for (int k = 0; k < NV; ++k) {
-    const int q = k * 64 + lane;
-    const f4 g = reinterpret_cast<const f4*>(gamma)[q], b = reinterpret_cast<const f4*>(beta)[q];
-    const size_t gi = (size_t)f * n + 4 * q;
-    float ss = 0.f;
-#pragma unroll
-    for (int c = 0; c < 4; ++c) {
-      const float o = ((v[k][c] - mean) * rstd * g[c] + b[c]) * drop_mult(drop, seed, stream, gi + c, p);
-      ss += o * o;
-    }
-    for (int m = 1; m < LPC; m <<= 1) ss += __shfl_xor(ss, m, 64);
-    L[k] = sqrtf(ss + len_eps);
-    t1 += L[k];
-  }
-  const float mo = wave_sum(t1) / (float)LPC / J;
-  float t2 = 0.f;
-#pragma unroll
-  for (int k = 0; k < NV; ++k) t2 += (L[k] - mo) * (L[k] - mo);
-  const float ro = 1.f / sqrtf(wave_sum(t2) / (float)LPC / J + kLnEps);
-  if (lane % LPC == 0) {
-#pragma unroll
-    for (int k = 0; k < NV; ++k) {
-      const int j = (k * 64 + lane) / LPC;
-      lens[(size_t)f * J + j] = L[k];
-      logits[(size_t)f * J + j] = (L[k] - mo) * ro * gamma_o[j] + beta_o[j];
-    }
-  }
-  if (lane == 0) {
-    stat[4 * f] = mean;
-    stat[4 * f + 1] = rstd;
-    stat[4 * f + 2] = mo;
-    stat[4 * f + 3] = ro;
-  }
-}
-
-template <int NPL>
 __global__ __launch_bounds__(256) void caps_head_fwd_wave_kernel(const float* __restrict__ x,
                                                                  const float* __restrict__ gamma,
                                                                  const float* __restrict__ beta, int training, float p,
@@ -756,61 +649,6 @@
   if (w >= rows) return;
   caps_head_fwd_wave<NPL>(x, gamma, beta, training && p > 0.f, p, srf_step_seed(seed, seed_src), stream, stat, D,
                           gamma_o, beta_o, logits, lens, len_eps, w, threadIdx.x & 63);
-}
-
-template <int NPL>
-__device__ __forceinline__ void capsnorm_bwd_wave(const float* __restrict__ x, const float* __restrict__ gamma,
-                                                  bool drop, float p, unsigned long long seed, unsigned stream,
-                                                  const float* __restrict__ stat, const float* __restrict__ g_in,
-                                                  float* __restrict__ g_x, f4 (&pgxh)[NPL / 4], f4 (&pgg)[NPL / 4],
-                                                  int f, int lane) {
-  constexpr int n = 64 * NPL, NV = NPL / 4;
-  const float mean = stat[4 * f], rstd = stat[4 * f + 1];
-  const f4* xr = reinterpret_cast<const f4*>(x + (size_t)f * n);
-  const f4* gr = reinterpret_cast<const f4*>(g_in + (size_t)f * n);
-  f4 xh[NV], t[NV];
-  float a1 = 0.f, a2 = 0.f;
-#pragma unroll
-  for (int k = 0; k < NV; ++k) {
-    const int q = k * 64 + lane;
-    const f4 xv = xr[q], go = gr[q], gam = reinterpret_cast<const f4*>(gamma)[q];
-    const size_t gi = (size_t)f * n + 4 * q;
-    f4 gxh, gg;
-#pragma unroll
-    for (int c = 0; c < 4; ++c) {
-      xh[k][c] = (xv[c] - mean) * rstd;
-      const float g = go[c] * drop_mult(drop, seed, stream, gi + c, p);
-      gxh[c] = g * xh[k][c];
-      gg[c] = g;
-      t[k][c] = g * gam[c];
-      a1 += t[k][c];
-      a2 += t[k][c] * xh[k][c];
-    }
-    pgxh[k] += gxh;
-    pgg[k] += gg;
-  }
-  a1 = wave_sum(a1);
-  a2 = wave_sum(a2);
-  f4* ox = reinterpret_cast<f4*>(g_x + (size_t)f * n);
-#pragma unroll
-  for (int k = 0; k < NV; ++k) {
-    f4 o;
-#pragma unroll
-    for (int c = 0; c < 4; ++c) o[c] = rstd * (t[k][c] - a1 / n - xh[k][c] * a2 / n);
-    ox[k * 64 + lane] = o;
-  }
-}
-
-template <int NPL>
-__device__ __forceinline__ void store_gpart(float* __restrict__ gpart, size_t row, const f4 (&pgxh)[NPL / 4],
-                                            const f4 (&pgg)[NPL / 4], int lane) {
-  constexpr int n = 64 * NPL;
-  f4* pg = reinterpret_cast<f4*>(gpart + row * 2 * n);
-#pragma unroll
-  for (int k = 0; k < NPL / 4; ++k) {
-    pg[k * 64 + lane] = pgxh[k];
-    pg[n / 4 + k * 64 + lane] = pgg[k];
-  }
 }
 
 template <int NPL, bool BWD>
@@ -972,8 +810,6 @@
 }
 
 }
-
-constexpr int kCnRowsPerWave = 4;
 
 template <bool BWD>
 static bool capsnorm_wave(int n, int rows, RowMap rm, const float* x, const float* gamma, const float* beta,
diff --git a/srf_amd/csrc/caps_norm_dev.h b/srf_amd/csrc/caps_norm_dev.h
--- /dev/null
+++ b/srf_amd/csrc/caps_norm_dev.h
@@ -0,0 +1,205 @@
+#pragma once
+#include "srf_common.h"
+#include "srf_rng.h"
+
+namespace {
+
+constexpr float kLnEps = 1e-3f;
+constexpr int kCnRowsPerWave = 4;
+
+__device__ __forceinline__ float drop_mult(bool on, unsigned long long seed, unsigned stream, size_t idx, float p) {
+  if (!on) return 1.f;
+  return srf_keep(seed, stream, idx, p) ? 1.f / (1.f - p) : 0.f;
+}
+
+template <int NPL>
+__device__ __forceinline__ void capsnorm_fwd_wave_regs(const f4 (&v)[NPL / 4], const float* __restrict__ gamma,
+                                                       const float* __restrict__ beta, bool drop, float p,
+                                                       unsigned long long seed, unsigned stream,
+                                                       float* __restrict__ y, float* __restrict__ stat, int f,
+                                                       int lane) {
+  constexpr int n = 64 * NPL, NV = NPL / 4;
+  float s1 = 0.f;
+#pragma unroll
+  for (int k = 0; k < NV; ++k) s1 += (v[k].x + v[k].y) + (v[k].z + v[k].w);
+  const float mean = wave_sum(s1) / n;
+  float s2 = 0.f;
+#pragma unroll
+  for (int k = 0; k < NV; ++k) {
+    const f4 d = v[k] - mean;
+    s2 += (d.x * d.x + d.y * d.y) + (d.z * d.z + d.w * d.w);
+  }
+  const float rstd = 1.f / sqrtf(wave_sum(s2) / n + kLnEps);
+  f4* yr = reinterpret_cast<f4*>(y + (size_t)f * n);
+#pragma unroll
+  for (int k = 0; k < NV; ++k) {
+    const int q = k * 64 + lane;
+    const f4 g = reinterpret_cast<const f4*>(gamma)[q], b = reinterpret_cast<const f4*>(beta)[q];
+    const size_t gi = (size_t)f * n + 4 * q;
+    f4 o;
+#pragma unroll
+    for (int c = 0; c < 4; ++c) o[c] = ((v[k][c] - mean) * rstd * g[c] + b[c]) * drop_mult(drop, seed, stream, gi + c, p);
+    yr[q] = o;
+  }
+  if (lane == 0) {
+    stat[4 * f] = mean;
+    stat[4 * f + 1] = rstd;
+  }
+}
+
+template <int NPL>
+__device__ __forceinline__ void capsnorm_fwd_wave(const float* __restrict__ x, const float* __restrict__ gamma,
+                                                  const float* __restrict__ beta, bool drop, float p,
+                                                  unsigned long long seed, unsigned stream, float* __restrict__ y,
+                                                  float* __restrict__ stat, int f, int lane) {
+  constexpr int n = 64 * NPL, NV = NPL / 4;
+  const f4* xr = reinterpret_cast<const f4*>(x + (size_t)f * n);
+  f4 v[NV];
+#pragma unroll
+  for (int k = 0; k < NV; ++k) v[k] = xr[k * 64 + lane];
+  capsnorm_fwd_wave_regs<NPL>(v, gamma, beta, drop, p, seed, stream, y, stat, f, lane);
+}
+
+template <int NPL>
+__device__ __forceinline__ void caps_head_fwd_wave_regs(const f4 (&v)[NPL / 4], const float* __restrict__ gamma,
+                                                        const float* __restrict__ beta, bool drop, float p,
+                                                        unsigned long long seed, unsigned stream,
+                                                        float* __restrict__ stat, int D,
+                                                        const float* __restrict__ gamma_o,
+                                                        const float* __restrict__ beta_o, float* __restrict__ logits,
+                                                        float* __restrict__ lens, float len_eps, int f, int lane) {
+  constexpr int n = 64 * NPL, NV = NPL / 4;
+  const int LPC = D / 4, J = n / D;
+  float s1 = 0.f;
+#pragma unroll
+  for (int k = 0; k < NV; ++k) s1 += (v[k].x + v[k].y) + (v[k].z + v[k].w);
+  const float mean = wave_sum(s1) / n;
+  float s2 = 0.f;
+#pragma unroll
+  for (int k = 0; k < NV; ++k) {
+    const f4 d = v[k] - mean;
+    s2 += (d.x * d.x + d.y * d.y) + (d.z * d.z + d.w * d.w);
+  }
+  const float rstd = 1.f / sqrtf(wave_sum(s2) / n + kLnEps);
+  float L[NV];
+  float t1 = 0.f;
+#pragma unroll
+  for (int k = 0; k < NV; ++k) {
+    const int q = k * 64 + lane;
+    const f4 g = reinterpret_cast<const f4*>(gamma)[q], b = reinterpret_cast<const f4*>(beta)[q];
+    const size_t gi = (size_t)f * n + 4 * q;
+    float ss = 0.f;
+#pragma unroll
+    for (int c = 0; c < 4; ++c) {
+      const float o = ((v[k][c] - mean) * rstd * g[c] + b[c]) * drop_mult(drop, seed, stream, gi + c, p);
+      ss += o * o;
+    }
+    for (int m = 1; m < LPC; m <<= 1) ss += __shfl_xor(ss, m, 64);
+    L[k] = sqrtf(ss + len_eps);
+    t1 += L[k];
+  }
+  const float mo = wave_sum(t1) / (float)LPC / J;
+  float t2 = 0.f;
+#pragma unroll
+  for (int k = 0; k < NV; ++k) t2 += (L[k] - mo) * (L[k] - mo);
+  const float ro = 1.f / sqrtf(wave_sum(t2) / (float)LPC / J + kLnEps);
+  if (lane % LPC == 0) {
+#pragma unroll
+    for (int k = 0; k < NV; ++k) {
+      const int j = (k * 64 + lane) / LPC;
+      lens[(size_t)f * J + j] = L[k];
+      logits[(size_t)f * J + j] = (L[k] - mo) * ro * gamma_o[j] + beta_o[j];
+    }
+  }
+  if (lane == 0) {
+    stat[4 * f] = mean;
+    stat[4 * f + 1] = rstd;
+    stat[4 * f + 2] = mo;
+    stat[4 * f + 3] = ro;
+  }
+}
+
+template <int NPL>
+__device__ __forceinline__ void caps_head_fwd_wave(const float* __restrict__ x, const float* __restrict__ gamma,
+                                                   const float* __restrict__ beta, bool drop, float p,
+                                                   unsigned long long seed, unsigned stream,
+                                                   float* __restrict__ stat, int D, const float* __restrict__ gamma_o,
+                                                   const float* __restrict__ beta_o, float* __restrict__ logits,
+                                                   float* __restrict__ lens, float len_eps, int f, int lane) {
+  constexpr int n = 64 * NPL, NV = NPL / 4;
+  const f4* xr = reinterpret_cast<const f4*>(x + (size_t)f * n);
+  f4 v[NV];
+#pragma unroll
+  for (int k = 0; k < NV; ++k) v[k] = xr[k * 64 + lane];
+  caps_head_fwd_wave_regs<NPL>(v, gamma, beta, drop, p, seed, stream, stat, D, gamma_o, beta_o, logits, lens, len_eps,
+                               f, lane);
+}
+
+template <int NPL, class XRow, class GxOut>
+__device__ __forceinline__ void capsnorm_bwd_wave_regs(XRow&& xrow, const float* __restrict__ gamma,
+                                                       bool drop, float p, unsigned long long seed, unsigned stream,
+                                                       const float* __restrict__ stat,
+                                                       const float* __restrict__ g_in, GxOut&& gx,
+                                                       f4 (&pgxh)[NPL / 4], f4 (&pgg)[NPL / 4], int f, int lane) {
+#pragma clang fp contract(off)
+  constexpr int n = 64 * NPL, NV = NPL / 4;
+  const float mean = stat[4 * f], rstd = stat[4 * f + 1];
+  const f4* gr = reinterpret_cast<const f4*>(g_in + (size_t)f * n);
+  f4 xh[NV], t[NV];
+  float a1 = 0.f, a2 = 0.f;
+#pragma unroll
+  for (int k = 0; k < NV; ++k) {
+    const int q = k * 64 + lane;
+    const f4 xv = xrow(k), go = gr[q], gam = reinterpret_cast<const f4*>(gamma)[q];
+    const size_t gi = (size_t)f * n + 4 * q;
+    f4 gxh, gg;
+#pragma unroll
+    for (int c = 0; c < 4; ++c) {
+      xh[k][c] = (xv[c] - mean) * rstd;
+      const float g = go[c] * drop_mult(drop, seed, stream, gi + c, p);
+      gxh[c] = g * xh[k][c];
+      gg[c] = g;
+      t[k][c] = g * gam[c];
+      a1 += t[k][c];
+      a2 += t[k][c] * xh[k][c];
+    }
+    pgxh[k] += gxh;
+    pgg[k] += gg;
+  }
+  a1 = wave_sum(a1);
+  a2 = wave_sum(a2);
+#pragma unroll
+  for (int k = 0; k < NV; ++k) {
+    f4 o;
+#pragma unroll
+    for (int c = 0; c < 4; ++c) o[c] = rstd * (t[k][c] - a1 / n - xh[k][c] * a2 / n);
+    gx(k, o);
+  }
+}
+
+template <int NPL>
+__device__ __forceinline__ void capsnorm_bwd_wave(const float* __restrict__ x, const float* __restrict__ gamma,
+                                                  bool drop, float p, unsigned long long seed, unsigned stream,
+                                                  const float* __restrict__ stat, const float* __restrict__ g_in,
+                                                  float* __restrict__ g_x, f4 (&pgxh)[NPL / 4], f4 (&pgg)[NPL / 4],
+                                                  int f, int lane) {
+  constexpr int n = 64 * NPL;
+  const f4* xr = reinterpret_cast<const f4*>(x + (size_t)f * n);
+  f4* ox = reinterpret_cast<f4*>(g_x + (size_t)f * n);
+  capsnorm_bwd_wave_regs<NPL>([&](int k) { return xr[k * 64 + lane]; }, gamma, drop, p, seed, stream, stat, g_in,
+                              [&](int k, const f4& o) { ox[k * 64 + lane] = o; }, pgxh, pgg, f, lane);
+}
+
+template <int NPL>
+__device__ __forceinline__ void store_gpart(float* __restrict__ gpart, size_t row, const f4 (&pgxh)[NPL / 4],
+                                            const f4 (&pgg)[NPL / 4], int lane) {
+  constexpr int n = 64 * NPL;
+  f4* pg = reinterpret_cast<f4*>(gpart + row * 2 * n);
+#pragma unroll
+  for (int k = 0; k < NPL / 4; ++k) {
+    pg[k * 64 + lane] = pgxh[k];
+    pg[n / 4 + k * 64 + lane] = pgg[k];
+  }
+}
+
+}
diff --git a/srf_amd/csrc/route_dr.hip b/srf_amd/csrc/route_dr.hip
--- a/srf_amd/csrc/route_dr.hip
+++ b/srf_amd/csrc/route_dr.hip
@@ -4,6 +4,8 @@
 
 #include "srf_common.h"
 #include "route_fwd32.h"
+#include "caps_norm_dev.h"
+#include "srf_reduce.h"
 #include "../../include/srf.h"
 #include "../../include/srf_prof.h"
 
@@ -1689,6 +1691,13 @@
   return v;
 }
 
+__device__ __forceinline__ float dot4(const f4& a, const f4& b) {
+  return fmaf(a.x, b.x, a.y * b.y) + fmaf(a.z, b.z, a.w * b.w);
+}
+__device__ __forceinline__ f4 axpby4(const f4& a, float f, const f4& s, float g) {
+  return f4{fmaf(a.x, f, s.x * g), fmaf(a.y, f, s.y * g), fmaf(a.z, f, s.z * g), fmaf(a.w, f, s.w * g)};
+}
+
 struct SlabSplit {
   int n;
   int G, U, in_n, JD;
@@ -1717,7 +1726,7 @@
   const bool ok = idx < FJD / 4;
   const size_t off = (ok ? idx : 0) * 4;
   const f4 sv = sum_slab4(slab, sp, FJD, off);
-  const float n2 = qsum<Q>((sv.x * sv.x + sv.y * sv.y) + (sv.z * sv.z + sv.w * sv.w));
+  const float n2 = qsum<Q>(dot4(sv, sv));
   if (!ok) return;
   const float fac = n2 / (1.f + n2) / sqrtf(n2 + kSquashEps);
   const f4 v = sv * fac;
@@ -1728,7 +1737,7 @@
 
 template <int DOUT>
 __global__ void bwd_finish_kernel(const float* __restrict__ slab, SlabSplit sp, size_t FJD,
-                                  const float* __restrict__ a_init, float* __restrict__ A,
+                                  const float* __restrict__ a_init, float* __restrict__ A, int a_load, int a_store,
                                   const float* __restrict__ s, float* __restrict__ gs, float* __restrict__ zero4,
                                   size_t nz4, float* __restrict__ zero1) {
   constexpr int Q = DOUT / 4;
@@ -1740,20 +1749,124 @@
   f4 a;
   if (a_init) {
     a = ld4(a_init + off);
-    if (ok) st4(A + off, f4{0.f, 0.f, 0.f, 0.f});
   } else {
-    a = ld4(A + off) + sum_slab4(slab, sp, FJD, off);
-    if (ok) st4(A + off, a);
+    a = (a_load ? ld4(A + off) : f4{0.f, 0.f, 0.f, 0.f}) + sum_slab4(slab, sp, FJD, off);
+    if (ok && a_store) st4(A + off, a);
   }
   const f4 sv = ld4(s + off);
-  const float n2 = qsum<Q>((sv.x * sv.x + sv.y * sv.y) + (sv.z * sv.z + sv.w * sv.w));
-  const float sa = qsum<Q>((sv.x * a.x + sv.y * a.y) + (sv.z * a.z + sv.w * a.w));
+  const float n2 = qsum<Q>(dot4(sv, sv));
+  const float sa = qsum<Q>(dot4(a, sv));
   if (!ok) return;
   const float rs = 1.f / sqrtf(n2 + kSquashEps);
   const float ip = 1.f / (1.f + n2);
   const float gfac = n2 * ip * rs;
   const float dg2 = 2.f * rs * ip * (ip - 0.5f * n2 / (n2 + kSquashEps)) * sa;
-  st4(gs + off, a * gfac + sv * dg2);
+  st4(gs + off, axpby4(a, gfac, sv, dg2));
+}
+
+#ifndef SRF_DR_NORM_FUSED
+#define SRF_DR_NORM_FUSED 1
+#endif
+
+__device__ __forceinline__ void as_stored(f4& v) {
+  asm volatile("" : "+v"(v.x), "+v"(v.y), "+v"(v.z), "+v"(v.w));
+}
+
+struct NormFwdArgs {
+  const float *gamma, *beta;
+  int training;
+  float p;
+  unsigned long long seed;
+  const unsigned long long* seed_src;
+  unsigned stream;
+  float *y, *stat;
+  const float *gamma_o, *beta_o;
+  float *logits, *lens, *v_out;
+  float len_eps;
+};
+
+template <int NPL, int DOUT, bool HEAD>
+__global__ __launch_bounds__(256) void fwd_finish_norm_kernel(const float* __restrict__ slab, SlabSplit sp, size_t FJD,
+                                                              float* __restrict__ s_out, NormFwdArgs na, int rows) {
+  constexpr int n = 64 * NPL, NV = NPL / 4, Q = DOUT / 4;
+  const int w = blockIdx.x * 4 + (threadIdx.x >> 6);
+  if (w >= rows) return;
+  const int lane = threadIdx.x & 63;
+  f4 v[NV];
+#pragma unroll
+  for (int k = 0; k < NV; ++k) {
+    const size_t off = (size_t)w * n + 4 * (k * 64 + lane);
+    const f4 sv = sum_slab4(slab, sp, FJD, off);
+    const float n2 = qsum<Q>(dot4(sv, sv));
+    const float fac = n2 / (1.f + n2) / sqrtf(n2 + kSquashEps);
+    v[k] = sv * fac;
+    as_stored(v[k]);
+    st4(s_out + off, sv);
+    if constexpr (HEAD) st4(na.v_out + off, v[k]);
+  }
+  const bool drop = na.training && na.p > 0.f;
+  const unsigned long long sd = srf_step_seed(na.seed, na.seed_src);
+  if constexpr (HEAD)
+    caps_head_fwd_wave_regs<NPL>(v, na.gamma, na.beta, drop, na.p, sd, na.stream, na.stat, DOUT, na.gamma_o, na.beta_o,
+                                 na.logits, na.lens, na.len_eps, w, lane);
+  else
+    capsnorm_fwd_wave_regs<NPL>(v, na.gamma, na.beta, drop, na.p, sd, na.stream, na.y, na.stat, w, lane);
+}
+
+struct NormBwdArgs {
+  const float *gamma, *stat, *g_y;
+  int training;
+  float p;
+  unsigned long long seed;
+  const unsigned long long* seed_src;
+  unsigned stream;
+  float* gpart;
+};
+
+template <int NPL, int DOUT>
+__global__ __launch_bounds__(256) void norm_bwd_finish_kernel(const float* __restrict__ s, float* __restrict__ gs,
+                                                              NormBwdArgs na, int rows, int rpw,
+                                                              float* __restrict__ zero4, size_t nz4,
+                                                              float* __restrict__ zero1) {
+  constexpr int n = 64 * NPL, NV = NPL / 4, Q = DOUT / 4;
+  const size_t tid = (size_t)blockIdx.x * blockDim.x + threadIdx.x;
+  for (size_t i = tid; i < nz4; i += (size_t)gridDim.x * blockDim.x) st4(zero4 + i * 4, f4{0.f, 0.f, 0.f, 0.f});
+  if (zero1 != nullptr && tid == 0) *zero1 = 0.f;
+  const int w = blockIdx.x * 4 + (threadIdx.x >> 6);
+  const int lane = threadIdx.x & 63;
+  const int r0 = w * rpw;
+  if (r0 >= rows) return;
+  const bool drop = na.training && na.p > 0.f;
+  const unsigned long long sd = srf_step_seed(na.seed, na.seed_src);
+  f4 pgxh[NV], pgg[NV];
+#pragma unroll
+  for (int k = 0; k < NV; ++k) pgxh[k] = pgg[k] = f4{0.f, 0.f, 0.f, 0.f};
+  const int r1 = min(rows, r0 + rpw);
+  for (int f = r0; f < r1; ++f) {
+    f4 sv[NV], v[NV], a[NV];
+    float n2[NV];
+#pragma unroll
+    for (int k = 0; k < NV; ++k) {
+      sv[k] = ld4(s + (size_t)f * n + 4 * (k * 64 + lane));
+      n2[k] = qsum<Q>(dot4(sv[k], sv[k]));
+      const float fac = n2[k] / (1.f + n2[k]) / sqrtf(n2[k] + kSquashEps);
+      v[k] = sv[k] * fac;
+      as_stored(v[k]);
+    }
+    capsnorm_bwd_wave_regs<NPL>([&](int k) { return v[k]; }, na.gamma, drop, na.p, sd, na.stream, na.stat, na.g_y,
+                                [&](int k, const f4& o) { a[k] = o; }, pgxh, pgg, f, lane);
+#pragma unroll
+    for (int k = 0; k < NV; ++k) {
+      as_stored(a[k]);
+      const float sa = qsum<Q>(dot4(a[k], sv[k]));
+      const float rs = 1.f / sqrtf(n2[k] + kSquashEps);
+      const float ip = 1.f / (1.f + n2[k]);
+      const float gfac = n2[k] * ip * rs;
+      const float dg2 = 2.f * rs * ip * (ip - 0.5f * n2[k] / (n2[k] + kSquashEps)) * sa;
+      st4(gs + (size_t)f * n + 4 * (k * 64 + lane), axpby4(a[k], gfac, sv[k], dg2));
+    }
+  }
+  store_gpart<NPL>(na.gpart, (size_t)w, pgxh, pgg, lane);
 }
 
 struct PassCfg {
@@ -1823,13 +1936,59 @@
 
 template <int D>
 void launch_bwd_finish(const DrGeom& g, const float* slab, const SlabSplit& sp, const float* a_init, float* A,
-                       const float* s, float* gs, hipStream_t st, float* zero = nullptr, size_t n_zero = 0,
-                       float* zero1 = nullptr) {
+                       const float* s, float* gs, hipStream_t st, bool a_load = true, bool a_store = true,
+                       float* zero = nullptr, size_t n_zero = 0, float* zero1 = nullptr) {
   const size_t FJD = (size_t)g.F() * g.JD();
   const size_t nz4 = zero ? n_zero / 4 : 0;
   const size_t n = std::max(FJD / 4, nz4);
   hipLaunchKernelGGL((bwd_finish_kernel<D>), dim3((n + 255) / 256), dim3(256), 0, st, slab, sp, FJD, a_init,
-                     A, s, gs, zero, nz4, zero1);
+                     A, a_load ? 1 : 0, a_store ? 1 : 0, s, gs, zero, nz4, zero1);
+}
+
+inline int norm_npl(const DrGeom& g) {
+  const int n = g.JD();
+  return n == 256 ? 4 : n == 512 ? 8 : n == 1024 ? 16 : 0;
+}
+inline bool norm_fused(const DrGeom& g) {
+  return SRF_DR_NORM_FUSED != 0 && g.iters >= 2 && norm_npl(g) != 0 && g.din == g.dout &&
+         (g.dout == 8 || g.dout == 16 || g.dout == 32 || g.dout == 64);
+}
+
+template <int D, bool HEAD>
+void launch_fwd_finish_norm(const DrGeom& g, const float* slab, const SlabSplit& sp, float* s_out,
+                            const NormFwdArgs& na, hipStream_t st) {
+  const size_t FJD = (size_t)g.F() * g.JD();
+  const dim3 grid((g.F() + 3) / 4);
+#define SRF_FIN_NORM(NPL) \
+  hipLaunchKernelGGL((fwd_finish_norm_kernel<NPL, D, HEAD>), grid, dim3(256), 0, st, slab, sp, FJD, s_out, na, g.F())
+  switch (norm_npl(g)) {
+    case 4: SRF_FIN_NORM(4); break;
+    case 8: SRF_FIN_NORM(8); break;
+    default: SRF_FIN_NORM(16); break;
+  }
+#undef SRF_FIN_NORM
+}
+
+struct NormBwd {
+  NormBwdArgs k;
+  float *scratch, *g_gamma, *g_beta;
+};
+
+template <int D>
+void launch_norm_bwd_finish(const DrGeom& g, const float* s, float* gs, const NormBwdArgs& na, hipStream_t st,
+                            float* zero, size_t n_zero, float* zero1) {
+  const int waves = (g.F() + kCnRowsPerWave - 1) / kCnRowsPerWave;
+  const dim3 grid((waves + 3) / 4);
+  const size_t nz4 = zero ? n_zero / 4 : 0;
+#define SRF_NORM_FIN(NPL)                                                                                      \
+  hipLaunchKernelGGL((norm_bwd_finish_kernel<NPL, D>), grid, dim3(256), 0, st, s, gs, na, g.F(), kCnRowsPerWave, \
+                     zero, nz4, zero1)
+  switch (norm_npl(g)) {
+    case 4: SRF_NORM_FIN(4); break;
+    case 8: SRF_NORM_FIN(8); break;
+    default: SRF_NORM_FIN(16); break;
+  }
+#undef SRF_NORM_FIN
 }
 
 constexpr int gu_tw(int d) { return d >= 64 ? 4 : 2; }
@@ -2155,7 +2314,7 @@
 
 template <int D>
 int fwd_impl(const DrPlan& p, const float* emb, const float* W, const float* bias, float* v_out, float* saved,
-             float* couplings, float* slab, hipStream_t st) {
+             float* couplings, float* slab, hipStream_t st, const NormFwdArgs* norm = nullptr, bool head = false) {
   const DrGeom& g = p.g;
   const srf::Fwd32Plan& plan = p.p32;
   const srf::Fwd32Cpl& cl = p.cpl;
@@ -2212,10 +2371,19 @@
     SRF_LAUNCH_CHECK("route_pass(fwd)");
     if (r < nev) SRF_HIP_TRY(hipEventRecord(ev1[r], st));
     const bool last = r == g.iters - 1;
-    launch_fwd_finish<D>(g, p.fwd32 ? srf::fwd32_slab(plan, scratch) : slab,
-                         !p.fwd32 ? uniform_split(p.chunks) : r == 0 ? uniform_split(plan.n_chunks) : pass_split(g, plan),
-                         vc, saved + (size_t)(2 * r) * FJD, last ? nullptr : saved + (size_t)(2 * r + 1) * FJD,
-                         last ? v_out : nullptr, st);
+    const float* fslab = p.fwd32 ? srf::fwd32_slab(plan, scratch) : slab;
+    const SlabSplit fsp =
+        !p.fwd32 ? uniform_split(p.chunks) : r == 0 ? uniform_split(plan.n_chunks) : pass_split(g, plan);
+    if (last && norm) {
+      if (head)
+        launch_fwd_finish_norm<D, true>(g, fslab, fsp, saved + (size_t)(2 * r) * FJD, *norm, st);
+      else
+        launch_fwd_finish_norm<D, false>(g, fslab, fsp, saved + (size_t)(2 * r) * FJD, *norm, st);
+      SRF_LAUNCH_CHECK("fwd_finish_norm");
+      continue;
+    }
+    launch_fwd_finish<D>(g, fslab, fsp, vc, saved + (size_t)(2 * r) * FJD,
+                         last ? nullptr : saved + (size_t)(2 * r + 1) * FJD, last ? v_out : nullptr, st);
     SRF_LAUNCH_CHECK("fwd_finish");
   }
   return SRF_OK;
@@ -2262,7 +2430,7 @@
 template <int D>
 int bwd_impl(const DrPlan& p, const float* emb, const float* W, const float* bias, const float* saved,
              const float* couplings, const float* g_v, float* g_emb, float* g_W, float* g_bias, float* ws,
-             hipStream_t st, bool with_weights) {
+             hipStream_t st, bool with_weights, const NormBwd* norm = nullptr) {
   const DrGeom& g = p.g;
   const BwdWs& w = p.ws;
   const srf::Fwd32Plan& plan = p.p32;
@@ -2272,10 +2440,22 @@
   const bool p32 = p.couplings;
   float* const gsv = ws + w.gs;
   const size_t n_emb = (size_t)g.F() * g.N * g.din;
-  launch_bwd_finish<D>(g, nullptr, uniform_split(1), g_v, ws + w.A, saved + (size_t)(2 * (R - 1)) * FJD,
-                       gsv + (size_t)(R - 1) * FJD, st, p32 ? g_emb : nullptr, n_emb, p32 ? ws + w.gumax : nullptr);
+  if (norm) {
+    launch_norm_bwd_finish<D>(g, saved + (size_t)(2 * (R - 1)) * FJD, gsv + (size_t)(R - 1) * FJD, norm->k, st,
+                              p32 ? g_emb : nullptr, n_emb, p32 ? ws + w.gumax : nullptr);
+    SRF_LAUNCH_CHECK("norm_bwd_finish");
+    const int n = g.JD();
+    if (const int rc = srf::colsum(norm->k.gpart, (g.F() + kCnRowsPerWave - 1) / kCnRowsPerWave, 2 * n, nullptr,
+                                   norm->scratch, st,
+                                   srf::ColSplit{{norm->g_gamma, norm->g_beta, nullptr, nullptr}, {n, n, 0, 0}}))
+      return rc;
+  } else
+    launch_bwd_finish<D>(g, nullptr, uniform_split(1), g_v, ws + w.A, saved + (size_t)(2 * (R - 1)) * FJD,
+                         gsv + (size_t)(R - 1) * FJD, st, false, false, p32 ? g_emb : nullptr, n_emb,
+                         p32 ? ws + w.gumax : nullptr);
   SRF_LAUNCH_CHECK("bwd_finish");
   for (int r = R - 1; r >= 1; --r) {
+    const bool a_load = r != R - 1, a_store = r != 1;
     const float* vc = saved + (size_t)(2 * (r - 1) + 1) * FJD;
     float* stats_r = ws + w.stats + (size_t)(r - 1) * g.F() * g.in_n() * 2;
     if (p32) {
@@ -2287,13 +2467,13 @@
                                      ws + w.gl + (size_t)(r - 1) * blk * JP, st);
       if (rc) return rc;
       launch_bwd_finish<D>(g, srf::fwd32_slab(plan, ws + w.p32), pass_split(g, plan), nullptr, ws + w.A,
-                           saved + (size_t)(2 * (r - 1)) * FJD, gsv + (size_t)(r - 1) * FJD, st);
+                           saved + (size_t)(2 * (r - 1)) * FJD, gsv + (size_t)(r - 1) * FJD, st, a_load, a_store);
     } else {
       dispatch_pass<D, MODE_BWD>(g, p.pc, p.chunks, emb, W, bias, r, vc, gsv + (size_t)r * FJD, ws + w.slab, stats_r, 1,
                                  st);
       SRF_LAUNCH_CHECK("route_pass(bwd)");
       launch_bwd_finish<D>(g, ws + w.slab, uniform_split(p.chunks), nullptr, ws + w.A,
-                           saved + (size_t)(2 * (r - 1)) * FJD, gsv + (size_t)(r - 1) * FJD, st);
+                           saved + (size_t)(2 * (r - 1)) * FJD, gsv + (size_t)(r - 1) * FJD, st, a_load, a_store);
     }
     SRF_LAUNCH_CHECK("bwd_finish");
   }
@@ -2339,6 +2519,59 @@
   return dispatch_din(din, [&](auto D) {
     return bwd_impl<D>(p, emb, W, bias, saved, couplings, g_v, g_emb, g_W, g_bias, static_cast<float*>(workspace),
                        static_cast<hipStream_t>(stream), with_weights);
+  });
+}
+
+int unsupported_norm(const DrGeom& g) {
+  srf::set_error("no fused finish + LayerNorm for J*dout = %d, iters = %d (srf_route_dr_norm_supported)", g.JD(),
+                 g.iters);
+  return SRF_EUNSUPPORTED;
+}
+
+int route_dr_fwd_norm_entry(const float* emb, const float* W, const float* bias, const DrGeom& g, int n_chunks,
+                            float* saved, float* couplings, void* workspace, size_t workspace_bytes,
+                            NormFwdArgs na, int layer, bool head, void* stream) {
+  DrPlan p;
+  const bool ptrs = emb && W && bias && saved && workspace && na.gamma && na.beta && na.stat &&
+                    (head ? na.gamma_o && na.beta_o && na.logits && na.lens && na.v_out : na.y != nullptr);
+  const int rc = enter(p, g, n_chunks, ptrs, couplings != nullptr, true, workspace_bytes);
+  if (rc) return rc;
+  if (!norm_fused(g)) return unsupported_norm(g);
+  na.seed_src = srf::seed_source();
+  na.stream = (unsigned)(kStreamMid0 + layer);
+  return dispatch_din(g.din, [&](auto D) {
+    return fwd_impl<D>(p, emb, W, bias, nullptr, saved, couplings, static_cast<float*>(workspace),
+                       static_cast<hipStream_t>(stream), &na, head);
+  });
+}
+
+int route_dr_bwd_norm_entry(const float* emb, const float* W, const float* bias, const DrGeom& g, int n_chunks,
+                            const float* saved, const float* couplings, NormBwdArgs na, int layer, float* g_emb,
+                            float* g_W, float* g_bias, float* g_gamma, float* g_beta, void* workspace,
+                            size_t workspace_bytes, void* norm_workspace, size_t norm_workspace_bytes, void* stream,
+                            bool with_weights) {
+  DrPlan p;
+  const int rc = enter(p, g, n_chunks,
+                       emb && W && bias && saved && g_emb && g_W && g_bias && workspace && na.g_y && na.gamma &&
+                           na.stat && g_gamma && g_beta && norm_workspace,
+                       couplings != nullptr, false, workspace_bytes);
+  if (rc) return rc;
+  if (!norm_fused(g)) return unsupported_norm(g);
+  const int F = g.F(), n = g.JD();
+  if (norm_workspace_bytes < srf_capsnorm_bwd_workspace(F, n, 0)) {
+    srf::set_error("capsnorm workspace too small");
+    return SRF_EWORKSPACE;
+  }
+  hipStream_t st = static_cast<hipStream_t>(stream);
+  float* part = static_cast<float*>(norm_workspace);
+  float* scratch = part + srf::align_up((size_t)F * 2 * n * 4, 256) / 4 + srf::align_up((size_t)2 * n * 4, 256) / 4;
+  na.gpart = part;
+  na.seed_src = srf::seed_source();
+  na.stream = (unsigned)(kStreamMid0 + layer);
+  const NormBwd nb{na, scratch, g_gamma, g_beta};
+  return dispatch_din(g.din, [&](auto D) {
+    return bwd_impl<D>(p, emb, W, bias, saved, couplings, nullptr, g_emb, g_W, g_bias, static_cast<float*>(workspace),
+                       st, with_weights, &nb);
   });
 }
 
@@ -2481,6 +2714,64 @@
   });
 }
 
+int srf_route_dr_norm_supported(int B, int T, int N, int din, int lpad, int rpad, int J, int dout, int iters) {
+  return norm_fused(DrGeom{B, T, N, din, lpad, rpad, J, dout, iters, 0}) ? 1 : 0;
+}
+
+int srf_route_dr_fwd_norm_ex(const float* emb, const float* W, const float* bias, int B, int T, int N, int din,
+                             int lpad, int rpad, int J, int dout, int iters, int mask_first, int n_chunks,
+                             float* saved, float* couplings, void* workspace, size_t workspace_bytes,
+                             const float* gamma, const float* beta, int training, float p, unsigned long long seed,
+                             int layer, float* y, float* stat, void* stream) {
+  NormFwdArgs na{};
+  na.gamma = gamma, na.beta = beta, na.training = training, na.p = p, na.seed = seed, na.y = y, na.stat = stat;
+  return route_dr_fwd_norm_entry(emb, W, bias, DrGeom{B, T, N, din, lpad, rpad, J, dout, iters, mask_first ? 1 : 0},
+                                 n_chunks, saved, couplings, workspace, workspace_bytes, na, layer, false, stream);
+}
+
+int srf_route_dr_fwd_head_ex(const float* emb, const float* W, const float* bias, int B, int T, int N, int din,
+                             int lpad, int rpad, int J, int dout, int iters, int mask_first, int n_chunks,
+                             float* v_out, float* saved, float* couplings, void* workspace, size_t workspace_bytes,
+                             const float* gamma_mid, const float* beta_mid, const float* gamma_out,
+                             const float* beta_out, int training, float p, unsigned long long seed, int layer,
+                             float length_eps, float* logits, float* stat, float* lens, void* stream) {
+  NormFwdArgs na{};
+  na.gamma = gamma_mid, na.beta = beta_mid, na.training = training, na.p = p, na.seed = seed, na.stat = stat;
+  na.gamma_o = gamma_out, na.beta_o = beta_out, na.logits = logits, na.lens = lens, na.v_out = v_out;
+  na.len_eps = length_eps;
+  return route_dr_fwd_norm_entry(emb, W, bias, DrGeom{B, T, N, din, lpad, rpad, J, dout, iters, mask_first ? 1 : 0},
+                                 n_chunks, saved, couplings, workspace, workspace_bytes, na, layer, true, stream);
+}
+
+int srf_route_dr_bwd_norm_ex(const float* emb, const float* W, const float* bias, int B, int T, int N, int din,
+                             int lpad, int rpad, int J, int dout, int iters, int mask_first, int n_chunks,
+                             const float* saved, const float* couplings, const float* g_y, const float* gamma,
+                             const float* stat, int training, float p, unsigned long long seed, int layer,
+                             float* g_emb, float* g_W, float* g_bias, float* g_gamma, float* g_beta,
+                             void* workspace, size_t workspace_bytes, void* norm_workspace,
+                             size_t norm_workspace_bytes, void* stream) {
+  NormBwdArgs na{};
+  na.gamma = gamma, na.stat = stat, na.g_y = g_y, na.training = training, na.p = p, na.seed = seed;
+  return route_dr_bwd_norm_entry(emb, W, bias, DrGeom{B, T, N, din, lpad, rpad, J, dout, iters, mask_first ? 1 : 0},
+                                 n_chunks, saved, couplings, na, layer, g_emb, g_W, g_bias, g_gamma, g_beta, workspace,
+                                 workspace_bytes, norm_workspace, norm_workspace_bytes, stream, true);
+}
+
+int srf_route_dr_bwd_norm_data_ex(const float* emb, const float* W, const float* bias, int B, int T, int N, int din,
+                                  int lpad, int rpad, int J, int dout, int iters, int mask_first, int n_chunks,
+                                  const float* saved, const float* couplings, const float* g_y, const float* gamma,
+                                  const float* stat, int training, float p, unsigned long long seed, int layer,
+                                  float* g_emb, float* g_gamma, float* g_beta, void* workspace,
+                                  size_t workspace_bytes, void* norm_workspace, size_t norm_workspace_bytes,
+                                  void* stream) {
+  NormBwdArgs na{};
+  na.gamma = gamma, na.stat = stat, na.g_y = g_y, na.training = training, na.p = p, na.seed = seed;
+  float* unused = reinterpret_cast<float*>(workspace);
+  return route_dr_bwd_norm_entry(emb, W, bias, DrGeom{B, T, N, din, lpad, rpad, J, dout, iters, mask_first ? 1 : 0},
+                                 n_chunks, saved, couplings, na, layer, g_emb, unused, unused, g_gamma, g_beta,
+                                 workspace, workspace_bytes, norm_workspace, norm_workspace_bytes, stream, false);
+}
+
 int srf_route_dr_bwd(const float* emb, const float* W, const float* bias, int B, int T, int N, int din, int lpad,
                      int rpad, int J, int dout, int iters, int mask_first, int n_chunks, const float* saved,
                      const float* g_v, float* g_emb, float* g_W, float* g_bias, void* workspace,
diff --git a/srf_amd/ops.py b/srf_amd/ops.py
--- a/srf_amd/ops.py
+++ b/srf_amd/ops.py
@@ -129,31 +129,82 @@
         _dr_state['queued'] = True
 
 
+def _dr_forward_buffers(g, emb, W, bias, need_bwd):
+    _check_dev('emb', emb, (g.B, g.T, g.N, g.din))
+    _check_dev('W', W, (g.in_n, g.J, g.dout, g.din))
+    _check_dev('bias', bias, (g.in_n, g.J, g.dout))
+    L = _lib.lib()
+    dev = emb.device
+    saved = torch.empty(L.srf_route_dr_saved_floats(g.B, g.T, g.J, g.dout, g.iters), device=dev,
+                        dtype=torch.float32)
+    ws_bytes = L.srf_route_dr_fwd_workspace(*g.ws_args())
+    ws = torch.empty(max(ws_bytes, 16), device=dev, dtype=torch.uint8)
+    if g.timing is not None:
+        starts, stops, n = g.timing.pop(0)
+        _lib.check(L.srf_route_dr_set_timing_events(starts, stops, n), 'set_timing_events')
+        if not g.timing:
+            g.timing = None
+    nc = L.srf_route_dr_coupling_floats(g.B, g.T, g.N, g.din, g.lpad, g.rpad, g.J, g.dout, g.iters) \
+        if need_bwd and g.store_couplings else 0
+    cpl = torch.empty(nc, device=dev, dtype=torch.float32) if nc else None
+    return saved, ws, ws_bytes, cpl
+
+
+def _dr_backward(ctx, emb, W, bias, saved, g_v, norm=None):
+    g = ctx.geom
+    L = _lib.lib()
+    g_emb = torch.empty_like(emb)
+    tW, tb = _grad_target(ctx.params[0]), _grad_target(ctx.params[1])
+    g_W, g_b = tW[0], tb[0]
+    ws_bytes = L.srf_route_dr_bwd_workspace(*g.ws_args())
+    ws = torch.empty(ws_bytes, device=emb.device, dtype=torch.uint8)
+    cpl = ctx.couplings
+    ctx.couplings = None
+    cp = _ptr(cpl) if cpl is not None else None
+    if norm is None:
+        head = (_ptr(saved), cp, _ptr(g_v))
+        tail = ()
+        data, full, kind = L.srf_route_dr_bwd_data_ex, L.srf_route_dr_bwd_ex, 'srf_route_dr_bwd'
+        g_norm = ()
+    else:
+        g_y, gamma, stat, tr, p, seed, layer, g_g, g_bt = norm
+        nb = L.srf_capsnorm_bwd_workspace(g.B * g.T, g.J * g.dout, 0)
+        nws = torch.empty(nb, device=emb.device, dtype=torch.uint8)
+        head = (_ptr(saved), cp, _ptr(g_y), _ptr(gamma), _ptr(stat), tr, p, seed, layer)
+        tail = (_ptr(nws), nb)
+        data, full, kind = L.srf_route_dr_bwd_norm_data_ex, L.srf_route_dr_bwd_norm_ex, 'srf_route_dr_bwd_norm'
+        g_norm = (_ptr(g_g), _ptr(g_bt))
+    _dr_issue_pending()
+    if DR_GW_SIDE and cpl is not None and tW[1] and tb[1]:
+        rc = data(_ptr(emb), _ptr(W), _ptr(bias), *g.args(), *head, _ptr(g_emb), *g_norm, _ptr(ws), ws_bytes, *tail,
+                  _stream())
+        _lib.check(rc, kind + '_data_ex')
+        ev = getattr(g, '_gw_event', None)
+        if ev is None:
+            ev = g._gw_event = torch.cuda.Event()
+        ev.record()
+
+        def launch(st, emb=emb, saved=saved, cpl=cpl, g_W=g_W, g_b=g_b, ws=ws):
+            _lib.check(L.srf_route_dr_bwd_weights_ex(_ptr(emb), *g.args(), _ptr(saved), _ptr(cpl), _ptr(g_W),
+                                                     _ptr(g_b), _ptr(ws), ws_bytes, st),
+                       'srf_route_dr_bwd_weights_ex')
+        _defer_side(emb.device, ev, launch, (emb, saved, cpl, ws))
+    else:
+        rc = full(_ptr(emb), _ptr(W), _ptr(bias), *g.args(), *head, _ptr(g_emb), _ptr(g_W), _ptr(g_b), *g_norm,
+                  _ptr(ws), ws_bytes, *tail, _stream())
+        _lib.check(rc, kind + '_ex')
+    return g_emb, tW, tb
+
+
 class DynamicRouting(torch.autograd.Function):
 
     @staticmethod
     def forward(ctx, emb, W, bias, geom, need_bwd=True):
         g = geom
-        _check_dev('emb', emb, (g.B, g.T, g.N, g.din))
-        _check_dev('W', W, (g.in_n, g.J, g.dout, g.din))
-        _check_dev('bias', bias, (g.in_n, g.J, g.dout))
-        L = _lib.lib()
-        dev = emb.device
-        v = torch.empty((g.B, g.T, g.J, g.dout), device=dev, dtype=torch.float32)
-        saved = torch.empty(L.srf_route_dr_saved_floats(g.B, g.T, g.J, g.dout, g.iters), device=dev,
-                            dtype=torch.float32)
-        ws_bytes = L.srf_route_dr_fwd_workspace(*g.ws_args())
-        ws = torch.empty(max(ws_bytes, 16), device=dev, dtype=torch.uint8)
-        if g.timing is not None:
-            starts, stops, n = g.timing.pop(0)
-            _lib.check(L.srf_route_dr_set_timing_events(starts, stops, n), 'set_timing_events')
-            if not g.timing:
-                g.timing = None
-        nc = L.srf_route_dr_coupling_floats(g.B, g.T, g.N, g.din, g.lpad, g.rpad, g.J, g.dout, g.iters) \
-            if need_bwd and g.store_couplings else 0
-        cpl = torch.empty(nc, device=dev, dtype=torch.float32) if nc else None
-        rc = L.srf_route_dr_fwd_ex(_ptr(emb), _ptr(W), _ptr(bias), *g.args(), _ptr(v), _ptr(saved),
-                                   _ptr(cpl) if cpl is not None else None, _ptr(ws), ws_bytes, _stream())
+        saved, ws, ws_bytes, cpl = _dr_forward_buffers(g, emb, W, bias, need_bwd)
+        v = torch.empty((g.B, g.T, g.J, g.dout), device=emb.device, dtype=torch.float32)
+        rc = _lib.lib().srf_route_dr_fwd_ex(_ptr(emb), _ptr(W), _ptr(bias), *g.args(), _ptr(v), _ptr(saved),
+                                            _ptr(cpl) if cpl is not None else None, _ptr(ws), ws_bytes, _stream())
         _lib.check(rc, 'srf_route_dr_fwd_ex')
         ctx.geom = g
         ctx.params = (W, bias)
@@ -164,42 +215,99 @@
     @staticmethod
     def backward(ctx, g_v):
         emb, W, bias, saved = ctx.saved_tensors
-        g = ctx.geom
-        g_v = g_v.contiguous()
-        L = _lib.lib()
-        g_emb = torch.empty_like(emb)
-        tW, tb = _grad_target(ctx.params[0]), _grad_target(ctx.params[1])
-        g_W, g_b = tW[0], tb[0]
-        ws_bytes = L.srf_route_dr_bwd_workspace(*g.ws_args())
-        ws = torch.empty(ws_bytes, device=emb.device, dtype=torch.uint8)
-        cpl = ctx.couplings
-        ctx.couplings = None
-        cp = _ptr(cpl) if cpl is not None else None
-        _dr_issue_pending()
-        if DR_GW_SIDE and cpl is not None and tW[1] and tb[1]:
-            rc = L.srf_route_dr_bwd_data_ex(_ptr(emb), _ptr(W), _ptr(bias), *g.args(), _ptr(saved), cp, _ptr(g_v),
-                                            _ptr(g_emb), _ptr(ws), ws_bytes, _stream())
-            _lib.check(rc, 'srf_route_dr_bwd_data_ex')
-            ev = getattr(g, '_gw_event', None)
-            if ev is None:
-                ev = g._gw_event = torch.cuda.Event()
-            ev.record()
-
-            def launch(st, emb=emb, saved=saved, cpl=cpl, g_W=g_W, g_b=g_b, ws=ws):
-                _lib.check(L.srf_route_dr_bwd_weights_ex(_ptr(emb), *g.args(), _ptr(saved), _ptr(cpl), _ptr(g_W),
-                                                         _ptr(g_b), _ptr(ws), ws_bytes, st),
-                           'srf_route_dr_bwd_weights_ex')
-            _defer_side(emb.device, ev, launch, (emb, saved, cpl, ws))
-        else:
-            rc = L.srf_route_dr_bwd_ex(_ptr(emb), _ptr(W), _ptr(bias), *g.args(), _ptr(saved), cp, _ptr(g_v),
-                                       _ptr(g_emb), _ptr(g_W), _ptr(g_b), _ptr(ws), ws_bytes, _stream())
-            _lib.check(rc, 'srf_route_dr_bwd_ex')
+        g_emb, tW, tb = _dr_backward(ctx, emb, W, bias, saved, g_v.contiguous())
         return (g_emb, *_returned([tW, tb]), None, None)
 
 
 def dynamic_routing(emb, W, bias, geom):
     need_bwd = torch.is_grad_enabled() and (emb.requires_grad or W.requires_grad or bias.requires_grad)
     return DynamicRouting.apply(emb, W, bias, geom, need_bwd)
+
+
+DR_NORM_FUSED = True
+
+
+def dr_norm_supported(geom):
+    g = geom
+    return DR_NORM_FUSED and bool(_lib.lib().srf_route_dr_norm_supported(g.B, g.T, g.N, g.din, g.lpad, g.rpad, g.J,
+                                                                         g.dout, g.iters))
+
+
+class DynamicRoutingNorm(torch.autograd.Function):
+
+    @staticmethod
+    def forward(ctx, emb, W, bias, gamma, beta, geom, training, p, seed, layer, need_bwd=True):
+        g = geom
+        saved, ws, ws_bytes, cpl = _dr_forward_buffers(g, emb, W, bias, need_bwd)
+        y = torch.empty((g.B, g.T, g.J, g.dout), device=emb.device, dtype=torch.float32)
+        stat = torch.empty((g.B * g.T, 4), device=emb.device, dtype=torch.float32)
+        tr = int(bool(training))
+        rc = _lib.lib().srf_route_dr_fwd_norm_ex(_ptr(emb), _ptr(W), _ptr(bias), *g.args(), _ptr(saved),
+                                                 _ptr(cpl) if cpl is not None else None, _ptr(ws), ws_bytes,
+                                                 _ptr(gamma), _ptr(beta), tr, float(p), int(seed), int(layer), _ptr(y),
+                                                 _ptr(stat), _stream())
+        _lib.check(rc, 'srf_route_dr_fwd_norm_ex')
+        ctx.geom = g
+        ctx.params = (W, bias)
+        ctx.norm_params = (gamma, beta)
+        ctx.meta = (tr, float(p), int(seed), int(layer))
+        ctx.couplings = cpl
+        ctx.save_for_backward(emb, W, bias, saved, gamma, stat)
+        return y
+
+    @staticmethod
+    def backward(ctx, g_y):
+        emb, W, bias, saved, gamma, stat = ctx.saved_tensors
+        tg, tbt = (_grad_target(q) for q in ctx.norm_params)
+        g_emb, tW, tb = _dr_backward(ctx, emb, W, bias, saved, None,
+                                     (g_y.contiguous(), gamma, stat, *ctx.meta, tg[0], tbt[0]))
+        return (g_emb, *_returned([tW, tb, tg, tbt]), None, None, None, None, None, None)
+
+
+class DynamicRoutingHead(torch.autograd.Function):
+
+    @staticmethod
+    def forward(ctx, emb, W, bias, gamma_mid, beta_mid, gamma_out, beta_out, geom, training, p, seed, layer,
+                length_eps=1e-7, need_bwd=True):
+        g = geom
+        saved, ws, ws_bytes, cpl = _dr_forward_buffers(g, emb, W, bias, need_bwd)
+        dev = emb.device
+        F = g.B * g.T
+        v = torch.empty((g.B, g.T, g.J, g.dout), device=dev, dtype=torch.float32)
+        logits = torch.empty((g.B, g.T, g.J), device=dev, dtype=torch.float32)
+        stat = torch.empty((F, 4), device=dev, dtype=torch.float32)
+        lens = torch.empty((F, g.J), device=dev, dtype=torch.float32)
+        tr = int(bool(training))
+        rc = _lib.lib().srf_route_dr_fwd_head_ex(_ptr(emb), _ptr(W), _ptr(bias), *g.args(), _ptr(v), _ptr(saved),
+                                                 _ptr(cpl) if cpl is not None else None, _ptr(ws), ws_bytes,
+                                                 _ptr(gamma_mid), _ptr(beta_mid), _ptr(gamma_out), _ptr(beta_out), tr,
+                                                 float(p), int(seed), int(layer), float(length_eps), _ptr(logits),
+                                                 _ptr(stat), _ptr(lens), _stream())
+        _lib.check(rc, 'srf_route_dr_fwd_head_ex')
+        ctx.geom = g
+        ctx.params = (W, bias)
+        ctx.head_params = (gamma_mid, beta_mid, gamma_out, beta_out)
+        ctx.meta = (F, g.J, g.dout, tr, float(p), int(seed), int(layer))
+        ctx.couplings = cpl
+        ctx.save_for_backward(emb, W, bias, saved, v, gamma_mid, beta_mid, gamma_out, beta_out, stat, lens)
+        return logits
+
+    @staticmethod
+    def backward(ctx, g_logits):
+        emb, W, bias, saved, v, gm, bm, go, bo, stat, lens = ctx.saved_tensors
+        F, J, D, tr, p, seed, layer = ctx.meta
+        L = _lib.lib()
+        g_v = torch.empty_like(v)
+        targets = [_grad_target(q) for q in ctx.head_params]
+        g_gm, g_bm, g_go, g_bo = (t for t, _ in targets)
+        wb = L.srf_capsnorm_bwd_workspace(F, J * D, J)
+        ws = torch.empty(wb, device=v.device, dtype=torch.uint8)
+        _lib.check(L.srf_caps_head_bwd(_ptr(v), F, J, D, _ptr(gm), _ptr(bm), _ptr(go), tr, p, seed, layer,
+                                       _ptr(stat), _ptr(lens), _ptr(g_logits.contiguous()), _ptr(g_v), _ptr(g_gm),
+                                       _ptr(g_bm), _ptr(g_go), _ptr(g_bo), _ptr(ws), wb, _stream()),
+                   'srf_caps_head_bwd')
+        g_emb, tW, tb = _dr_backward(ctx, emb, W, bias, saved, g_v)
+        return (g_emb, *_returned([tW, tb] + targets), None, None, None, None, None, None, None)
 
 
 class SequentialRouting(torch.autograd.Function):
diff --git a/srf_amd/sequence_router.py b/srf_amd/sequence_router.py
--- a/srf_amd/sequence_router.py
+++ b/srf_amd/sequence_router.py
@@ -248,9 +248,22 @@
             if l in self._identity and torch.is_grad_enabled():
                 self.P(f'W{l}').grad.zero_()
                 self.P(f'b{l}').grad.zero_()
+            norms = [f'ln_mid{l + 1}_gamma', f'ln_mid{l + 1}_beta']
+            geom = self._geom(l, B, T2)
+            if not self.is_context and ops.dr_norm_supported(geom):
+                last = l == self.enc_num - 1
+                if last:
+                    norms += ['ln_output_gamma', 'ln_output_beta']
+                self._on_grad(emb, [f'W{l}', f'b{l}'] + norms)
+                lnp = [self.P(n) for n in norms]
+                need_bwd = torch.is_grad_enabled() and any(t.requires_grad for t in [emb, W, bias] + lnp)
+                if last:
+                    return ops.DynamicRoutingHead.apply(emb, W, bias, *lnp, geom, training, p_mid, seed, l,
+                                                        self.length_eps, need_bwd)
+                emb = ops.DynamicRoutingNorm.apply(emb, W, bias, *lnp, geom, training, p_mid, seed, l, need_bwd)
+                continue
             self._on_grad(emb, [f'W{l}', f'b{l}'])
-            v = route(emb, W, bias, self._geom(l, B, T2))
-            norms = [f'ln_mid{l + 1}_gamma', f'ln_mid{l + 1}_beta']
+            v = route(emb, W, bias, geom)
             self._on_grad(v, norms if l < self.enc_num - 1 else norms + ['ln_output_gamma', 'ln_output_beta'])
             if l < self.enc_num - 1:
                 emb = ops.CapsNorm.apply(v, self.P(f'ln_mid{l + 1}_gamma'), self.P(f'ln_mid{l + 1}_beta'), training,
```

New measurement: 3.074 million frames/s, median of 6. About the same (+0.8%).
